# vidify/old-audiosync

Hardware: AMD Instinct MI355X
Metric: cross-correlations/sec (N=1440000 float32 pairs) (higher is better)
Workload: dtype f32; 1 GPU; batched xcorr, N=1440000 frames/sample (source 2N), 124 pairs per GPU per step, 48 kHz mono float32, planted delays, SNR 0 dB; sample_len=1440000, pairs_per_gpu=124, group=124, split=600x2400x16, layout=real-column, parallelism=pairs sharded over 1 GPU(s), one process per GPU, RCCL all_gather of results

## Files before the change

### include/audiosync/xcorr_hip.h

```cpp
#ifndef AUDIOSYNC_XCORR_HIP_H
#define AUDIOSYNC_XCORR_HIP_H

#include <stddef.h>
#include <stdint.h>

#ifdef __cplusplus
extern "C" {
#endif

typedef struct asx_plan asx_plan;


int asx_device_count(void);
int asx_current_device(void);
const char *asx_last_error(void);
int asx_abi_version(void);


asx_plan *asx_plan_create(size_t sample_len, size_t max_batch, int device);
asx_plan *asx_plan_create_ex(size_t sample_len, size_t max_batch, int device, const char *split);
int asx_plan_placement(asx_plan *plan, double ms[2], int *kept);
void asx_plan_destroy(asx_plan *plan);

int asx_plan_peak_overflows(asx_plan *plan, uint64_t *count);
int asx_plan_peak_repairs(asx_plan *plan, uint64_t *count);
int asx_plan_set_exact(asx_plan *plan, int on);
size_t asx_plan_peak_capacity(const asx_plan *plan);

int asx_plan_set_lag_window(asx_plan *plan, int64_t lag_min, int64_t lag_max);
int asx_plan_lag_window(const asx_plan *plan, int64_t *lag_min, int64_t *lag_max);

int asx_plan_set_pearson(asx_plan *plan, int spectral);
int asx_plan_pearson_modes(asx_plan *plan, uint64_t counts[3]);

int asx_plan_set_prune(asx_plan *plan, int on);
int asx_plan_prune_stats(asx_plan *plan, uint64_t *tiles_transformed, uint64_t *tiles_total);

size_t asx_plan_sample_len(const asx_plan *plan);
size_t asx_plan_fft_len(const asx_plan *plan);
int asx_plan_split(const asx_plan *plan, int *m1, int *m2, int *tile_cols);
int asx_plan_layout(const asx_plan *plan);
int asx_plan_threads(const asx_plan *plan, int *threads_cols, int *threads_rows);
size_t asx_plan_group(const asx_plan *plan);
size_t asx_plan_workspace_bytes(const asx_plan *plan);


int asx_xcorr_f64(asx_plan *plan, const double *source, const double *sample, long *lag,
                  double *coefficient);
int asx_plan_narrowed_calls(asx_plan *plan, uint64_t *count);

int asx_xcorr_batch_f32(asx_plan *plan, const float *source, const float *sample, size_t batch,
                        int64_t *lag, double *coef, int32_t *ret);

int asx_xcorr_batch_f32_dev(asx_plan *plan, const float *d_source, const float *d_sample,
                            size_t batch, int64_t *d_lag, double *d_coef, int32_t *d_ret,
                            void *stream);

int asx_xcorr_strided_f32_dev(asx_plan *plan, const float *d_source, size_t source_stride,
                              const float *d_sample, size_t sample_stride, size_t batch,
                              int64_t *d_lag, double *d_coef, int32_t *d_ret, void *stream);

int asx_xcorr_windowed_f32_dev(asx_plan *plan, const float *d_source, size_t source_stride,
                               const float *d_sample, size_t sample_stride,
                               const int64_t *d_windows, size_t window_stride,
                               size_t batch, int64_t *d_lag, double *d_coef, int32_t *d_ret,
                               void *stream);

#define ASX_TOPK_MAX 8
int asx_xcorr_topk_f32_dev(asx_plan *plan, const float *d_source, size_t source_stride,
                           const float *d_sample, size_t sample_stride,
                           const int64_t *d_windows, size_t window_stride,
                           size_t batch, int k, int64_t min_separation,
                           int64_t *d_lag, double *d_coef, int32_t *d_ret, void *stream);

int asx_xcorr_phat_f32_dev(asx_plan *plan, const float *d_source, size_t source_stride,
                           const float *d_sample, size_t sample_stride,
                           const int64_t *d_windows, size_t window_stride, size_t batch,
                           int64_t *d_lag, double *d_coef, double *d_peak, int32_t *d_ret, void *stream);

int asx_xcorr_phat_band_f32_dev(asx_plan *plan, const float *d_source, size_t source_stride,
                                const float *d_sample, size_t sample_stride,
                                const int64_t *d_windows, size_t window_stride, size_t batch,
                                int64_t bin_lo, int64_t bin_hi,
                                int64_t *d_lag, double *d_coef, double *d_peak, int32_t *d_ret, void *stream);

int asx_band_bins(size_t sample_len, double sample_rate, double f_lo_hz, double f_hi_hz,
                  int64_t *bin_lo, int64_t *bin_hi);

int asx_xcorr_pool_f32_dev(asx_plan *plan,
                           const float *d_sources, size_t source_stride, size_t nsources,
                           const float *d_samples, size_t sample_stride, size_t nsamples,
                           const int32_t *d_pairs,
                           const int64_t *d_windows, size_t window_stride,
                           size_t batch, int64_t *d_lag, double *d_coef, int32_t *d_ret, void *stream);

int asx_xcorr_pool_topk_f32_dev(asx_plan *plan,
                                const float *d_sources, size_t source_stride, size_t nsources,
                                const float *d_samples, size_t sample_stride, size_t nsamples,
                                const int32_t *d_pairs,
                                const int64_t *d_windows, size_t window_stride,
                                size_t batch, int k, int64_t min_separation,
                                int64_t *d_lag, double *d_coef, int32_t *d_ret, void *stream);

int asx_xcorr_batch_multi(asx_plan *const *plans, int nplans, const float *source, const float *sample,
                          size_t batch, int64_t *lag, double *coef, int32_t *ret);

typedef struct asx_comm asx_comm;
int asx_shard_range(size_t total, int nshards, int shard, size_t *start, size_t *count);
size_t asx_result_bytes(size_t width);
asx_comm *asx_comm_create(asx_plan *const *plans, int nplans);
void asx_comm_destroy(asx_comm *comm);
int asx_xcorr_batch_multi_dev(asx_comm *comm, const float *const *d_source, const float *const *d_sample,
                              const size_t *counts, size_t width, void *const *d_gathered);

int asx_xcorr_debug_r_dev(asx_plan *plan, const float *d_source, const float *d_sample,
                          float *d_r, int64_t *d_lag, double *d_coef, int32_t *d_ret,
                          void *stream);

int asx_xcorr_phat_debug_r_dev(asx_plan *plan, const float *d_source, const float *d_sample, float *d_r,
                               int64_t *d_lag, double *d_coef, double *d_peak, int32_t *d_ret, void *stream);

int asx_xcorr_phat_band_debug_r_dev(asx_plan *plan, const float *d_source, const float *d_sample,
                                    int64_t bin_lo, int64_t bin_hi, float *d_r,
                                    int64_t *d_lag, double *d_coef, double *d_peak, int32_t *d_ret, void *stream);

int asx_pearson_f64(const double *source_seg, const double *sample_seg, size_t n, int device,
                    double *coefficient);


int asx_results_to_ms_dev(const int64_t *d_lag, const double *d_coef, const int32_t *d_ret,
                          size_t batch, double min_confidence, double sample_rate,
                          int64_t *d_lag_ms, int32_t *d_accept, void *stream);

int asx_topk_best_dev(const int64_t *d_lag, const double *d_coef, const int32_t *d_ret,
                      size_t batch, int k,
                      int64_t *d_best_lag, double *d_best_coef, int32_t *d_best_ret, int32_t *d_best_entry,
                      void *stream);


typedef struct asx_stream asx_stream;

asx_stream *asx_stream_create(size_t max_sample_len, int device);
void asx_stream_destroy(asx_stream *stream);
int asx_stream_append_f64(asx_stream *stream, const double *source_frames, size_t n_source,
                          const double *sample_frames, size_t n_sample);
int asx_stream_lengths(const asx_stream *stream, size_t *n_source, size_t *n_sample);
int asx_stream_reset(asx_stream *stream);
int asx_stream_xcorr(asx_stream *stream, size_t sample_len, long *lag, double *coefficient);
int asx_stream_set_lag_window(asx_stream *stream, int64_t lag_min, int64_t lag_max);


int asx_synth_pairs_dev(uint64_t seed, uint64_t first_pair, size_t count, size_t sample_len,
                        int noise_shift, float *d_source, float *d_sample, int64_t *d_true_lag,
                        void *stream);

int asx_plan_set_profiling(asx_plan *plan, int depth);
int asx_plan_timings_ms(asx_plan *plan, int calls_back, float out[6]);
int asx_plan_last_timings_ms(asx_plan *plan, float out[6]);

void *asx_device_malloc(size_t bytes, int device);
int asx_device_free(void *ptr);
void *asx_host_malloc(size_t bytes);
int asx_host_free(void *ptr);
int asx_memcpy_h2d(void *dst_dev, const void *src_host, size_t bytes);
int asx_memcpy_d2h(void *dst_host, const void *src_dev, size_t bytes);
int asx_stream_sync(asx_plan *plan, void *stream);

#ifdef __cplusplus
}
#endif
#endif
```

### old-audiosync_amd/csrc/asx_api.hip

```cpp
#include "audiosync/xcorr_hip.h"

#include "asx_internal.h"
#include "dev_mem.h"
#include "plan_math.h"
#include "shard_driver.h"
#include "host_narrow.h"

#include <algorithm>
#include <cassert>
#include <cmath>
#include <cstdarg>
#include <cstdio>
#include <cstdlib>
#include <cstring>
#include <dlfcn.h>
#include <mutex>
#include <string>
#include <thread>
#include <type_traits>
#include <vector>

static thread_local std::string g_err;

static int fail(const char *fmt, ...)
{
    char buf[512];
    va_list ap;
    va_start(ap, fmt);
    vsnprintf(buf, sizeof(buf), fmt, ap);
    va_end(ap);
    g_err = buf;
    fprintf(stderr, "audiosync: %s\n", buf);
    return -1;
}

#define HIP_TRY(expr)                                                                         \
    do {                                                                                      \
        hipError_t e_ = (expr);                                                               \
        if (e_ != hipSuccess)                                                                 \
            return fail("%s failed: %s (%s:%d)", #expr, hipGetErrorString(e_), __FILE__, __LINE__); \
    } while (0)

#define HIP_TRY_NULL(expr)                                                                    \
    do {                                                                                      \
        hipError_t e_ = (expr);                                                               \
        if (e_ != hipSuccess) {                                                               \
            fail("%s failed: %s (%s:%d)", #expr, hipGetErrorString(e_), __FILE__, __LINE__);  \
            return nullptr;                                                                   \
        }                                                                                     \
    } while (0)

extern "C" const char *asx_last_error(void) { return g_err.c_str(); }
extern "C" int asx_abi_version(void) { return 2; }

extern "C" int asx_device_count(void)
{
    int n = 0;
    if (hipGetDeviceCount(&n) != hipSuccess) return 0;
    return n;
}

struct EventPair {
    hipEvent_t e0 = nullptr, e1 = nullptr;
    ~EventPair() { for (hipEvent_t e : { e0, e1 }) if (e) (void)hipEventDestroy(e); }
};

struct DevGuard {
    int prev = -1;
    bool ok = false;
    explicit DevGuard(int dev)
    {
        if (hipGetDevice(&prev) == hipSuccess && hipSetDevice(dev) == hipSuccess) ok = true;
    }
    ~DevGuard() { if (prev >= 0) (void)hipSetDevice(prev); }
};

static bool stream_capturing(hipStream_t s)
{
    hipStreamCaptureStatus cap = hipStreamCaptureStatusNone;
    if (hipStreamIsCapturing(s, &cap) != hipSuccess) (void)hipGetLastError();
    return cap != hipStreamCaptureStatusNone;
}

extern "C" int asx_current_device(void)
{
    int d = -1;
    if (hipGetDevice(&d) != hipSuccess) return -1;
    return d;
}

static thread_local hipError_t g_take_err = hipSuccess;
static const AsxMemOps hip_mem = {
    [](void **out, size_t bytes) { return (g_take_err = hipMalloc(out, bytes)) == hipSuccess ? 0 : ((void)hipGetLastError(), -1); },
    [](void *ptr) { (void)hipFree(ptr); }
};

struct asx_plan {
    int device = 0;
    AsxHostPlan host;
    AsxDev dev{};
    size_t group = 1;
    size_t stamp_blocks = 0;
    hipStream_t stream = nullptr;
    std::mutex lock;

    AsxMemSet mem{ hip_mem }, cxy0{ hip_mem };
    struct Lane {
        hipStream_t stream = nullptr;
        hipEvent_t done = nullptr;
        float2 *zxa = nullptr, *zya = nullptr, *ga = nullptr;
        AsxPeakWs pk{};
        AsxSeg *seg = nullptr;
        double *psums = nullptr;
        AsxSpecWs spec{};
        AsxTopkWs tk{};
        AsxPrune prune{};
        AsxPoolPair *pool = nullptr;
    } lanes[2];
    int nlanes = 1;
    hipEvent_t fork = nullptr;
    struct BigPeak {
        AsxCand *cand = nullptr;
        uint32_t *refine_idx = nullptr, *cand_n = nullptr, *refine_n = nullptr;
        double *refine_val = nullptr;
        unsigned long long *overflows = nullptr;
        float *src_dc = nullptr;
        double *stats = nullptr;
        size_t cap = 0;
    } big;
    AsxSpectra bslot{};
    struct Bank {
        AsxSpectra c{};
        AsxMemSet mem{ hip_mem };
        size_t nsrc = 0, nsmp = 0;
        unsigned long long fills = 0;
    } bank;
    uint32_t *over_list = nullptr, *over_n = nullptr;
    volatile uint32_t *h_over_n = nullptr;
    size_t over_cap = 0;
    std::vector<uint32_t> h_over;
    unsigned long long repaired = 0;
    bool exact = true;
    int64_t win_lo = 0, win_hi = 0;
    bool spectral = false;
    unsigned long long *mode_count = nullptr;
    bool prunable = false;
    bool prune = false;
    unsigned long long *prune_stats = nullptr;
    bool tune_placement = false, placement_done = false;
    double placement_ms[2] = { 0.0, 0.0 };
    int placement_kept = -1;
    struct Staging {
        float *src = nullptr, *smp = nullptr;
        int64_t *lag = nullptr; double *coef = nullptr; int32_t *ret = nullptr;
    } st;
    struct Staging64 { double *src = nullptr, *smp = nullptr; } st64;
    float *pin32 = nullptr;
    unsigned long long narrowed = 0;

    bool profiling = false;
    size_t prof_depth = 1, prof_calls = 0, prof_ring = 0;
    std::vector<std::vector<hipEvent_t>> evr;
    std::vector<size_t> prof_groups;
    size_t ev_groups = 0;
};

struct PlanCall {
    std::unique_lock<std::mutex> guard;
    DevGuard dg;
    hipStream_t s;
    explicit PlanCall(asx_plan *p, void *stream = nullptr, bool lock = true)
        : guard(lock ? std::unique_lock<std::mutex>(p->lock) : std::unique_lock<std::mutex>()), dg(p->device),
          s(stream ? (hipStream_t)stream : p->stream) {}
};

template <typename T> static int dev_alloc(AsxMemSet &m, T **out, size_t count)
{
    return m.take(out, count) ? fail("hipMalloc(&ptr, bytes) failed: %s (%s:%d)", hipGetErrorString(g_take_err), __FILE__, __LINE__) : 0;
}

template <typename T> static int dev_upload(AsxMemSet &m, const T **out, const std::vector<T> &v)
{
    T *d = nullptr;
    if (dev_alloc(m, &d, v.size()) != 0) return -1;
    HIP_TRY(hipMemcpy(d, v.data(), v.size() * sizeof(T), hipMemcpyHostToDevice));
    *out = d;
    return 0;
}

static int take_spectra(const AsxDev &P, AsxMemSet &m, AsxSpectra &c, size_t nsrc, size_t nsmp)
{
    const size_t pitch = asx_spectrum_len(P), na = std::max(nsrc, nsmp), nt = P.ntiles, nb = nt * (size_t)P.nbands;
    return m.take(&c.cx, nsrc * pitch) || m.take(&c.cy, nsmp * pitch) || m.take(&c.nrm, na * 2 * nt) || (nb && m.take(&c.band, na * 2 * nb)) ? -1 : 0;
}

static int plan_init(asx_plan *p, size_t N, size_t max_batch, const char *split)
{
    std::string err = asx_host_plan_build(N, split, &p->host);
    if (!err.empty()) return fail("plan for sample_len=%zu: %s", N, err.c_str());
    const AsxHostPlan &h = p->host;
    AsxDev &d = p->dev;
    AsxMemSet &m = p->mem;
    d.N = (uint32_t)N;
    d.F = h.F; d.M = h.M; d.M1 = h.M1; d.M2 = h.M2; d.T = h.T; d.logT = h.logT; d.ntiles = h.ntiles;
    d.src_valid = h.src_valid;
    d.src_period = (uint32_t)(2 * N);
    d.nout = (uint32_t)(2 * N);
    d.bound_scale = 2.0f * ASX_BOUND_C * 5.9604645e-8f * log2f((float)h.F) * (float)h.F;
    d.st1 = h.st1; d.st2 = h.st2;
    const AsxKernelChoice &k = h.kernels;
    if (k.rlayout && (k.cols < 0 || k.rows < 0 || !h.rlayout)) return fail("internal: a real-column plan without its kernels");
    d.threads_cols = k.threads_cols; d.threads_rows = k.threads_rows;
    d.rlayout = k.rlayout ? 1 : 0;
    d.kcols = k.cols; d.krows = k.rows;
    d.band_rows = k.band_rows;
    d.nbands = k.band_rows ? 2 * h.M1 / k.band_rows : 0;
    p->prunable = k.prunable;
    if (dev_upload(m, &d.tw1, h.tw1) || dev_upload(m, &d.tw2, h.tw2) || dev_upload(m, &d.tw2s, h.tw2s) || dev_upload(m, &d.tw_lo, h.tw_lo) ||
        dev_upload(m, &d.tw_hi, h.tw_hi) ||
        dev_upload(m, &d.k1_of_pos1, h.k1_of_pos1) || dev_upload(m, &d.pos1_of_k1, h.pos1_of_k1) ||
        dev_upload(m, &d.pos2_of_k2, h.pos2_of_k2) || dev_upload(m, &d.row_tasks, h.row_tasks))
        return -1;

    d.col_pairs = nullptr;
    d.col_tw = nullptr;
    if (k.rlayout && (dev_upload(m, &d.col_pairs, h.col_pairs) || dev_upload(m, &d.col_tw, h.col_tw))) return -1;
    size_t ws_mb = 4096;
    if (const char *e = getenv("ASX_WS_MB")) ws_mb = (size_t)atol(e) > 0 ? (size_t)atol(e) : ws_mb;
    size_t per_pair = (size_t)3 * h.M * sizeof(float2);
    size_t g = (ws_mb << 20) / per_pair / (getenv("ASX_LANES") && atoi(getenv("ASX_LANES")) == 2 ? 2 : 1);
    if (g < 1) g = 1;
    if (g > 65535) g = 65535;
    if (max_batch < 1) max_batch = 1;
    if (g > max_batch) g = max_batch;
    p->group = g;
    if (const char *e = getenv("ASX_LANES")) p->nlanes = atoi(e) == 2 ? 2 : 1;
    size_t cap = std::min<size_t>(std::max<size_t>(N / 64, ASX_CAND_MIN), ASX_CAND_MAX);
    cap = std::min<size_t>(cap, 2 * N);
    for (int l = 0; l < p->nlanes; l++) {
        asx_plan::Lane &ln = p->lanes[l];
        ln.pk.cap = (uint32_t)cap;
        const size_t mz = asx_spectrum_len(d);
        AsxMemSet &cxy = l == 0 ? p->cxy0 : m;
        if (dev_alloc(cxy, &ln.zxa, g * mz) || dev_alloc(cxy, &ln.zya, g * mz) || dev_alloc(m, &ln.ga, g * mz) ||
            dev_alloc(m, &ln.pk.nrm_part, g * 2 * (size_t)h.ntiles) || dev_alloc(m, &ln.pk.bound2, g) ||
            dev_alloc(m, &ln.pk.pairmax, g) || dev_alloc(m, &ln.pk.cand_n, g) ||
            dev_alloc(m, &ln.pk.cand, g * cap) || dev_alloc(m, &ln.pk.refine_n, g) ||
            dev_alloc(m, &ln.pk.refine_idx, g * cap) || dev_alloc(m, &ln.pk.refine_val, g * cap) ||
            dev_alloc(m, &ln.pk.overflows, 1) ||
            dev_alloc(m, &ln.seg, g) || dev_alloc(m, &ln.psums, g * (size_t)asx_pearson_blocks((uint32_t)N) * 6) ||
            dev_alloc(m, &ln.tk.pairs, g) || dev_alloc(m, &ln.tk.lag, g) || dev_alloc(m, &ln.tk.coef, g) || dev_alloc(m, &ln.tk.ret, g) ||
            dev_alloc(m, &ln.tk.sink, 1) || dev_alloc(m, &ln.pool, g))
            return -1;
        HIP_TRY(hipMemset(ln.pk.overflows, 0, sizeof(unsigned long long)));
        ln.pk.band = nullptr; ln.pk.tile_peak = nullptr;
        if (d.rlayout) {
            const size_t nbands = (size_t)d.nbands;
            if (!p->mode_count) {
                if (dev_alloc(m, &p->mode_count, ASX_PM_NMODES)) return -1;
                HIP_TRY(hipMemset(p->mode_count, 0, ASX_PM_NMODES * sizeof(unsigned long long)));
            }
            if (dev_alloc(m, &ln.pk.band, g * 2 * nbands * (size_t)h.ntiles) || dev_alloc(m, &ln.pk.tile_peak, g * (size_t)(h.M2 / h.T)) ||
                dev_alloc(m, &ln.spec.part, g * ASX_PREP_BLOCKS_MAX * 4) || dev_alloc(m, &ln.spec.hdr, g * ASX_SPEC_HDR))
                return -1;
            ln.spec.mode_count = p->mode_count;
            ln.spec.tol = 1e-5;
        }
        if (p->prunable) {
            if (!p->prune_stats) {
                if (dev_alloc(m, &p->prune_stats, 2)) return -1;
                HIP_TRY(hipMemset(p->prune_stats, 0, 2 * sizeof(unsigned long long)));
            }
            if (dev_alloc(m, &ln.prune.eng, g * ((size_t)h.M1 + 1) * (size_t)h.ntiles) || dev_alloc(m, &ln.prune.ub, g * (size_t)h.ntiles) ||
                dev_alloc(m, &ln.prune.best, g) || dev_alloc(m, &ln.prune.skip, g * (size_t)h.ntiles) ||
                dev_alloc(m, &ln.prune.part, g * 1024) || dev_alloc(m, &ln.prune.ticket, g))
                return -1;
            HIP_TRY(hipMemset(ln.prune.part, 0, g * 1024 * sizeof(double)));
            HIP_TRY(hipMemset(ln.prune.ticket, 0, g * sizeof(unsigned)));
            ln.prune.stats = p->prune_stats;
        }
        HIP_TRY(hipStreamCreateWithFlags(&ln.stream, hipStreamNonBlocking));
        HIP_TRY(hipEventCreateWithFlags(&ln.done, hipEventDisableTiming));
    }
    p->over_cap = std::max<size_t>(g * (size_t)p->nlanes, 1024);
    if (dev_alloc(m, &p->over_list, p->over_cap) || dev_alloc(m, &p->over_n, 1)) return -1;
    HIP_TRY(hipMemset(p->over_n, 0, sizeof(uint32_t)));
    uint32_t *d_over_host = nullptr;
    {
        void *h = nullptr, *dptr = nullptr;
        HIP_TRY(hipHostMalloc(&h, sizeof(uint32_t), hipHostMallocMapped));
        p->h_over_n = (volatile uint32_t *)h;
        *p->h_over_n = 0;
        HIP_TRY(hipHostGetDevicePointer(&dptr, h, 0));
        d_over_host = (uint32_t *)dptr;
    }
    for (int l = 0; l < p->nlanes; l++) {
        p->lanes[l].pk.over_list = p->over_list;
        p->lanes[l].pk.over_n = p->over_n;
        p->lanes[l].pk.over_host = d_over_host;
        p->lanes[l].pk.over_cap = (uint32_t)p->over_cap;
    }
    p->spectral = d.rlayout != 0;
    if (const char *e = getenv("ASX_PEARSON")) p->spectral = p->spectral && strcmp(e, "direct") != 0;
    p->prune = p->prunable;
    if (const char *e = getenv("ASX_PRUNE")) p->prune = p->prune && atoi(e) != 0;
    if (const char *e = getenv("ASX_EXACT")) p->exact = atoi(e) != 0;
    p->win_lo = -(int64_t)p->host.N;
    p->win_hi = (int64_t)p->host.N - 1;
    HIP_TRY(hipEventCreateWithFlags(&p->fork, hipEventDisableTiming));
    d.stamps = nullptr;
    d.stamp_kernel = 0;
    if (const char *e = getenv("ASX_STAMPS")) {
        unsigned long long *st = nullptr;
        p->stamp_blocks = g * (size_t)std::max(h.M1 + 1, 2 * h.ntiles);
        if (dev_alloc(m, &st, p->stamp_blocks * 8)) return -1;
        HIP_TRY(hipMemset(st, 0, p->stamp_blocks * 8 * sizeof(unsigned long long)));
        d.stamps = st;
        d.stamp_kernel = !strcmp(e, "fwd") ? 1 : !strcmp(e, "inv") ? 2 : 0;
    }
    {
        AsxDev *dcopy = nullptr;
        if (dev_alloc(m, &dcopy, 1)) return -1;
        d.self_dev = dcopy;
        HIP_TRY(hipMemcpy(dcopy, &d, sizeof(AsxDev), hipMemcpyHostToDevice));
    }
    HIP_TRY(hipStreamCreate(&p->stream));
    HIP_TRY(hipDeviceSynchronize());
    return 0;
}

static std::string measure_best_split(size_t N, size_t max_batch, int device)
{
    std::vector<std::string> cands = asx_host_plan_candidates(N, 16);
    {
        AsxHostPlan h;
        if (asx_host_plan_build(N, "", &h).empty()) {
            char buf[64];
            snprintf(buf, sizeof buf, "%dx%dx%d", h.M1, h.M2, h.T);
            if (std::find(cands.begin(), cands.end(), std::string(buf)) == cands.end()) cands.insert(cands.begin(), buf);
        }
    }
    if (cands.empty()) return "";
    size_t probe = ((size_t)512 << 20) / (12 * N);
    probe = std::max<size_t>(probe, 4);
    probe = std::min<size_t>(probe, 1024);
    probe = std::max<size_t>(1, std::min(probe, max_batch));
    AsxMemSet m(hip_mem);
    asx_plan::Staging d;
    std::string best;
    float best_ms = 0.f;
    EventPair ev;
    if (!m.take(&d.src, probe * 2 * N) && !m.take(&d.smp, probe * N) && !m.take(&d.lag, probe) && !m.take(&d.coef, probe) &&
        !m.take(&d.ret, probe) && hipEventCreate(&ev.e0) == hipSuccess && hipEventCreate(&ev.e1) == hipSuccess &&
        asx_synth_pairs_dev(12345, 0, probe, N, 1, d.src, d.smp, nullptr, nullptr) == 0 && hipDeviceSynchronize() == hipSuccess) {
        for (const std::string &c : cands) {
            asx_plan *p = asx_plan_create_ex(N, probe, device, c.c_str());
            if (!p) continue;
            bool ok = asx_xcorr_batch_f32_dev(p, d.src, d.smp, probe, d.lag, d.coef, d.ret, nullptr) == 0;
            float ms = 0.f;
            if (ok) {
                ok = hipEventRecord(ev.e0, p->stream) == hipSuccess;
                for (int r = 0; r < 2 && ok; r++) ok = asx_xcorr_batch_f32_dev(p, d.src, d.smp, probe, d.lag, d.coef, d.ret, nullptr) == 0;
                ok = ok && hipEventRecord(ev.e1, p->stream) == hipSuccess && hipEventSynchronize(ev.e1) == hipSuccess &&
                     hipEventElapsedTime(&ms, ev.e0, ev.e1) == hipSuccess;
            }
            asx_plan_destroy(p);
            if (ok && (best.empty() || ms < best_ms)) { best = c; best_ms = ms; }
        }
    }
    (void)hipGetLastError();
    return best;
}

extern "C" asx_plan *asx_plan_create_ex(size_t sample_len, size_t max_batch, int device, const char *split)
{
    if (!split || !*split) split = getenv("ASX_SPLIT");
    if (split && !strcmp(split, "measure")) {
        int prev = 0, ndev0 = 0;
        if (hipGetDeviceCount(&ndev0) != hipSuccess || ndev0 == 0) {
            fail("no usable HIP device; this library has no CPU fallback");
            return nullptr;
        }
        HIP_TRY_NULL(hipGetDevice(&prev));
        const int dev = device < 0 ? prev : device;
        if (dev >= ndev0) { fail("device %d out of range (%d devices)", dev, ndev0); return nullptr; }
        HIP_TRY_NULL(hipSetDevice(dev));
        const std::string best = measure_best_split(sample_len, max_batch ? max_batch : 1, dev);
        (void)hipSetDevice(prev);
        asx_plan *mp = asx_plan_create_ex(sample_len, max_batch, device, best.empty() ? "auto" : best.c_str());
        if (mp) mp->tune_placement = true;
        return mp;
    }
    if (split && !strcmp(split, "auto")) split = "";
    int ndev = 0;
    hipError_t e = hipGetDeviceCount(&ndev);
    if (e != hipSuccess || ndev == 0) {
        fail("no usable HIP device (%s); this library has no CPU fallback",
             e == hipSuccess ? "device count is 0" : hipGetErrorString(e));
        return nullptr;
    }
    if (device < 0) HIP_TRY_NULL(hipGetDevice(&device));
    if (device >= ndev) {
        fail("device %d out of range (%d devices)", device, ndev);
        return nullptr;
    }
    int prev = 0;
    HIP_TRY_NULL(hipGetDevice(&prev));
    HIP_TRY_NULL(hipSetDevice(device));
    asx_plan *p = new asx_plan();
    p->device = device;
    int rc = plan_init(p, sample_len, max_batch, split);
    (void)hipSetDevice(prev);
    if (rc != 0) {
        asx_plan_destroy(p);
        return nullptr;
    }
    return p;
}

extern "C" asx_plan *asx_plan_create(size_t sample_len, size_t max_batch, int device)
{
    return asx_plan_create_ex(sample_len, max_batch, device, nullptr);
}

extern "C" void asx_plan_destroy(asx_plan *p)
{
    if (!p) return;
    DevGuard dg(p->device);
    if (p->stream) { (void)hipStreamSynchronize(p->stream); (void)hipStreamDestroy(p->stream); }
    for (auto &ln : p->lanes) {
        if (ln.stream) { (void)hipStreamSynchronize(ln.stream); (void)hipStreamDestroy(ln.stream); }
        if (ln.done) (void)hipEventDestroy(ln.done);
    }
    if (p->fork) (void)hipEventDestroy(p->fork);
    for (auto &ring : p->evr)
        for (hipEvent_t ev : ring) (void)hipEventDestroy(ev);
    if (p->pin32) (void)hipHostFree(p->pin32);
    if (p->h_over_n) (void)hipHostFree((void *)p->h_over_n);
    delete p;
}

extern "C" size_t asx_plan_sample_len(const asx_plan *p) { return p ? p->host.N : 0; }
extern "C" size_t asx_plan_fft_len(const asx_plan *p) { return p ? p->host.F : 0; }
extern "C" size_t asx_plan_group(const asx_plan *p) { return p ? p->group : 0; }
extern "C" size_t asx_plan_workspace_bytes(const asx_plan *p) { return p ? p->mem.bytes() + p->cxy0.bytes() : 0; }
extern "C" long asx_plan_debug_stamps(asx_plan *p, unsigned long long *out, size_t cap)
{
    if (!p || !p->dev.stamps) return -1;
    size_t n = p->stamp_blocks * 8;
    if (n > cap) n = cap;
    if (hipMemcpy(out, p->dev.stamps, n * sizeof(unsigned long long), hipMemcpyDeviceToHost) != hipSuccess) return -1;
    return (long)n;
}

extern "C" int asx_plan_peak_overflows(asx_plan *p, uint64_t *count)
{
    if (!p || !count) return fail("asx_plan_peak_overflows: null argument");
    PlanCall c(p);
    if (!c.dg.ok) return fail("cannot select device %d", p->device);
    unsigned long long total = 0;
    for (int l = 0; l < p->nlanes; l++) {
        unsigned long long v = 0;
        HIP_TRY(hipStreamSynchronize(p->lanes[l].stream));
        HIP_TRY(hipStreamSynchronize(p->stream));
        HIP_TRY(hipMemcpy(&v, p->lanes[l].pk.overflows, sizeof(v), hipMemcpyDeviceToHost));
        total += v;
    }
    *count = total;
    return 0;
}

extern "C" int asx_plan_set_exact(asx_plan *p, int on)
{
    if (!p) return fail("asx_plan_set_exact: null argument");
    PlanCall c(p);
    if (!c.dg.ok) return fail("cannot select device %d", p->device);
    HIP_TRY(hipDeviceSynchronize());
    HIP_TRY(hipMemset(p->over_n, 0, sizeof(uint32_t)));
    *p->h_over_n = 0;
    p->exact = on != 0;
    return 0;
}

extern "C" int asx_plan_set_pearson(asx_plan *p, int spectral)
{
    if (!p) return fail("asx_plan_set_pearson: null argument");
    std::lock_guard<std::mutex> guard(p->lock);
    if (spectral && !p->dev.rlayout) return fail("asx_plan_set_pearson: the spectral form needs a real-column plan (the reference's six lengths)");
    p->spectral = spectral != 0;
    return 0;
}

extern "C" int asx_plan_pearson_modes(asx_plan *p, uint64_t counts[3])
{
    if (!p || !counts) return fail("asx_plan_pearson_modes: null argument");
    PlanCall c(p);
    if (!c.dg.ok) return fail("cannot select device %d", p->device);
    counts[0] = counts[1] = counts[2] = 0;
    if (!p->mode_count) return 0;
    HIP_TRY(hipDeviceSynchronize());
    unsigned long long v[ASX_PM_NMODES];
    HIP_TRY(hipMemcpy(v, p->mode_count, sizeof v, hipMemcpyDeviceToHost));
    for (int i = 0; i < 3; i++) counts[i] = v[i];
    return 0;
}

extern "C" int asx_plan_set_prune(asx_plan *p, int on)
{
    if (!p) return fail("asx_plan_set_prune: null argument");
    std::lock_guard<std::mutex> guard(p->lock);
    if (on && !p->prunable)
        return fail("asx_plan_set_prune: the pruned inverse pass needs a real-column plan (the reference's six lengths)");
    p->prune = on != 0;
    return 0;
}

extern "C" int asx_plan_prune_stats(asx_plan *p, uint64_t *tiles_transformed, uint64_t *tiles_total)
{
    if (!p || !tiles_transformed || !tiles_total) return fail("asx_plan_prune_stats: null argument");
    PlanCall c(p);
    if (!c.dg.ok) return fail("cannot select device %d", p->device);
    *tiles_transformed = *tiles_total = 0;
    if (!p->prune_stats) return 0;
    HIP_TRY(hipDeviceSynchronize());
    unsigned long long v[2];
    HIP_TRY(hipMemcpy(v, p->prune_stats, sizeof v, hipMemcpyDeviceToHost));
    *tiles_transformed = v[0];
    *tiles_total = v[1];
    return 0;
}

extern "C" int asx_plan_peak_repairs(asx_plan *p, uint64_t *count)
{
    if (!p || !count) return fail("asx_plan_peak_repairs: null argument");
    std::lock_guard<std::mutex> guard(p->lock);
    *count = p->repaired;
    return 0;
}

extern "C" int asx_plan_debug_peak(asx_plan *p, size_t pair, float *bound2, uint32_t *cand_n, uint32_t *refine_n,
                                   unsigned long long *pairmax, double *vals, uint32_t *idxs, size_t cap)
{
    if (!p || pair >= p->group) return -1;
    PlanCall c(p, nullptr, false);
    const AsxPeakWs &W = p->lanes[0].pk;
    (void)hipDeviceSynchronize();
    if (hipMemcpy(bound2, W.bound2 + pair, 4, hipMemcpyDeviceToHost) != hipSuccess) return -1;
    if (hipMemcpy(cand_n, W.cand_n + pair, 4, hipMemcpyDeviceToHost) != hipSuccess) return -1;
    if (hipMemcpy(refine_n, W.refine_n + pair, 4, hipMemcpyDeviceToHost) != hipSuccess) return -1;
    if (hipMemcpy(pairmax, W.pairmax + pair, 8, hipMemcpyDeviceToHost) != hipSuccess) return -1;
    size_t n = std::min<size_t>(cap, W.cap);
    if (vals && hipMemcpy(vals, W.refine_val + pair * (size_t)W.cap, n * 8, hipMemcpyDeviceToHost) != hipSuccess) return -1;
    if (idxs && hipMemcpy(idxs, W.refine_idx + pair * (size_t)W.cap, n * 4, hipMemcpyDeviceToHost) != hipSuccess) return -1;
    return 0;
}

extern "C" int asx_plan_debug_spectral(asx_plan *p, size_t pair, int *dims, float *band, size_t band_cap, double *hdr,
                                       long long *seg, double *pick)
{
    if (!p || pair >= p->group || !dims || !hdr || !seg || !pick) return -1;
    const asx_plan::Lane &W = p->lanes[0];
    if (!p->dev.rlayout || !W.pk.band || !W.spec.hdr) return -1;
    PlanCall c(p, nullptr, false);
    if (!c.dg.ok || hipDeviceSynchronize() != hipSuccess) return -1;
    const AsxDev &P = p->dev;
    const size_t cells = (size_t)P.ntiles * (size_t)P.nbands;
    if (band) {
        if (band_cap < 4 * cells) return -1;
        if (hipMemcpy(band, W.pk.band + pair * 2 * cells, 2 * cells * sizeof(float2), hipMemcpyDeviceToHost) != hipSuccess) return -1;
    }
    AsxSeg sg;
    if (hipMemcpy(hdr, W.spec.hdr + pair * ASX_SPEC_HDR, ASX_SPEC_HDR * sizeof(double), hipMemcpyDeviceToHost) != hipSuccess ||
        hipMemcpy(&sg, W.seg + pair, sizeof sg, hipMemcpyDeviceToHost) != hipSuccess)
        return -1;
    seg[0] = sg.lag; seg[1] = sg.src_off; seg[2] = sg.smp_off; seg[3] = sg.len; seg[4] = sg.peak; seg[5] = sg.flags;
    AsxMemSet tmp(hip_mem);
    double *d_pick = nullptr;
    if (tmp.take(&d_pick, 8)) return -1;
    const int nb = asx_launch_debug_spec_pick(P, W.spec, W.seg, pair, d_pick, p->stream);
    if (hipGetLastError() != hipSuccess || hipStreamSynchronize(p->stream) != hipSuccess ||
        hipMemcpy(pick, d_pick, 8 * sizeof(double), hipMemcpyDeviceToHost) != hipSuccess)
        return -1;
    dims[0] = P.ntiles; dims[1] = P.nbands; dims[2] = P.band_rows; dims[3] = nb;
    return 0;
}

extern "C" int asx_plan_debug_prune(asx_plan *p, size_t pair, float *ub, int *best, size_t n)
{
    if (!p || pair >= p->group || !p->lanes[0].prune.ub || n > (size_t)p->host.ntiles) return -1;
    PlanCall c(p, nullptr, false);
    if (!c.dg.ok || hipDeviceSynchronize() != hipSuccess) return -1;
    const AsxPrune &U = p->lanes[0].prune;
    if (ub && hipMemcpy(ub, U.ub + pair * (size_t)p->host.ntiles, n * sizeof(float), hipMemcpyDeviceToHost) != hipSuccess) return -1;
    if (best && hipMemcpy(best, U.best + pair, sizeof(int), hipMemcpyDeviceToHost) != hipSuccess) return -1;
    return 0;
}

extern "C" int asx_plan_debug_over_list(asx_plan *p, uint32_t *dev_n, uint32_t *host_n)
{
    if (!p || !dev_n || !host_n) return -1;
    PlanCall c(p, nullptr, false);
    if (!c.dg.ok || hipDeviceSynchronize() != hipSuccess) return -1;
    if (hipMemcpy(dev_n, p->over_n, sizeof(uint32_t), hipMemcpyDeviceToHost) != hipSuccess) return -1;
    *host_n = *p->h_over_n;
    return 0;
}

extern "C" size_t asx_plan_peak_capacity(const asx_plan *p) { return p ? p->lanes[0].pk.cap : 0; }

extern "C" int asx_plan_set_lag_window(asx_plan *p, int64_t lag_min, int64_t lag_max)
{
    if (!p) return fail("asx_plan_set_lag_window: null plan");
    const int64_t N = (int64_t)p->host.N;
    if (lag_min < -N || lag_max > N - 1 || lag_min > lag_max)
        return fail("asx_plan_set_lag_window: [%lld, %lld] is not a window inside [%lld, %lld] with lag_min <= lag_max",
                    (long long)lag_min, (long long)lag_max, (long long)-N, (long long)(N - 1));
    std::lock_guard<std::mutex> guard(p->lock);
    p->win_lo = lag_min;
    p->win_hi = lag_max;
    return 0;
}

extern "C" int asx_plan_lag_window(const asx_plan *p, int64_t *lag_min, int64_t *lag_max)
{
    if (!p || !lag_min || !lag_max) return fail("asx_plan_lag_window: null argument");
    std::lock_guard<std::mutex> guard(const_cast<asx_plan *>(p)->lock);
    *lag_min = p->win_lo;
    *lag_max = p->win_hi;
    return 0;
}

extern "C" int asx_plan_threads(const asx_plan *p, int *cols, int *rows)
{
    if (!p) return -1;
    if (cols) *cols = p->dev.threads_cols;
    if (rows) *rows = p->dev.threads_rows;
    return 0;
}

extern "C" int asx_plan_layout(const asx_plan *p) { return p ? p->dev.rlayout : -1; }

extern "C" int asx_plan_narrowed_calls(asx_plan *p, uint64_t *count)
{
    if (!p || !count) return fail("asx_plan_narrowed_calls: null argument");
    std::lock_guard<std::mutex> guard(p->lock);
    *count = p->narrowed;
    return 0;
}

extern "C" int asx_plan_split(const asx_plan *p, int *m1, int *m2, int *tile_cols)
{
    if (!p) return -1;
    if (m1) *m1 = p->host.M1;
    if (m2) *m2 = p->host.M2;
    if (tile_cols) *tile_cols = p->host.T;
    return 0;
}

static void prof_begin_call(asx_plan *p)
{
    p->ev_groups = 0;
    if (!p->profiling) return;
    p->prof_ring = p->prof_calls % p->prof_depth;
    if (p->prof_groups.size() < p->prof_depth) p->prof_groups.resize(p->prof_depth, 0);
    if (p->evr.size() < p->prof_depth) p->evr.resize(p->prof_depth);
    p->prof_groups[p->prof_ring] = 0;
}
static void prof_end_call(asx_plan *p, size_t groups)
{
    if (!p->profiling) return;
    p->ev_groups = groups;
    p->prof_groups[p->prof_ring] = groups;
    p->prof_calls++;
}

static int prof_mark(asx_plan *p, hipStream_t s, size_t slot)
{
    if (!p->profiling) return 0;
    std::vector<hipEvent_t> &ev = p->evr[p->prof_ring];
    while (ev.size() <= slot) {
        hipEvent_t e;
        HIP_TRY(hipEventCreate(&e));
        ev.push_back(e);
    }
    HIP_TRY(hipEventRecord(ev[slot], s));
    return 0;
}

struct PoolCall {
    const int32_t *rows;
    size_t nsrc, nsmp;
};
template <typename TIn> struct Pairs {
    const float *src, *smp;
    const TIn *tsrc, *tsmp;
    size_t src_step, smp_step;
    int bc;
    const int64_t *win = nullptr;
    size_t win_step = 0;
    const PoolCall *pool = nullptr;
    size_t first = 0;
    static Pairs staged(const float *src, const float *smp, const TIn *tsrc, const TIn *tsmp, size_t N, const int64_t *win = nullptr,
                        size_t win_step = 0)
    {
        return { .src = src, .smp = smp, .tsrc = tsrc, .tsmp = tsmp, .src_step = 2 * N, .smp_step = N, .bc = 0, .win = win, .win_step = win_step };
    }
    static Pairs contiguous(const float *src, const float *smp, size_t N) { return staged(src, smp, src, smp, N); }
    static Pairs strided(const float *src, size_t src_step, const float *smp, size_t smp_step, int bc, const int64_t *win, size_t win_step)
    {
        return { .src = src, .smp = smp, .tsrc = src, .tsmp = smp, .src_step = src_step, .smp_step = smp_step, .bc = bc, .win = win, .win_step = win_step };
    }
    static Pairs pooled(const PoolCall *pool, const float *srcs, size_t src_stride, const float *smps, size_t smp_stride, const int64_t *win,
                        size_t win_step)
    {
        Pairs x = strided(srcs, src_stride, smps, smp_stride, 0, win, win_step);
        x.pool = pool;
        return x;
    }
    Pairs pool_pair(size_t a, size_t b, size_t N) const
    {
        return staged(src + a * src_step, smp + b * smp_step, tsrc + a * src_step, tsmp + b * smp_step, N, win, win_step);
    }
    Pairs at(size_t k) const
    {
        Pairs x = *this;
        if (win) x.win += 2 * k * win_step;
        if (pool) { x.first += k; return x; }
        x.src += k * src_step; x.smp += k * smp_step; x.tsrc += k * src_step; x.tsmp += k * smp_step;
        return x;
    }
    AsxInputs<TIn> inputs(const AsxPoolPair *pl) const { return { tsrc, tsmp, src_step, smp_step, pl }; }
};

struct Results {
    int64_t *lag;
    double *coef;
    int32_t *ret;
    size_t step = 1;
    double *peak = nullptr;
    Results at(size_t k) const
    {
        return { lag ? lag + k * step : nullptr, coef + k * step, ret ? ret + k * step : nullptr, step, peak ? peak + k : nullptr };
    }
};

struct Topk {
    int k = 1;
    int64_t sep = 0;
};

struct GroupOpts {
    static constexpr size_t no_marks = SIZE_MAX;
    size_t prof_group = 0;
    int lane = 0;
    uint32_t pair_base = 0;
    bool listed = true;
    bool spectral = true;
    float *r_out = nullptr;
    int dot_blocks = 0;
    const AsxPeakWs *pk = nullptr;
    Topk topk{};
    AsxWeight weight = ASX_W_NONE;
    AsxBand fband{};
};

template <typename TIn>
static int run_group(asx_plan *p, const Pairs<TIn> &x, size_t g, const Results &y, hipStream_t s, const GroupOpts &o = {})
{
    const AsxDev &P = p->dev;
    asx_plan::Lane &W = p->lanes[o.lane];
    const AsxPeakWs &pk = o.pk ? *o.pk : W.pk;
    auto mark = [&](size_t k) { return o.prof_group != GroupOpts::no_marks && prof_mark(p, s, o.prof_group * 6 + k); };
    AsxPeakWs fin = pk;
    const bool phat = o.weight != ASX_W_NONE;
    if (!o.listed || phat) { fin.over_list = nullptr; fin.over_n = nullptr; fin.over_host = nullptr; fin.over_cap = 0; }
    const bool spectral = std::is_same<TIn, float>::value && p->spectral && o.spectral && pk.band && !phat;
    AsxPeakWs tk = pk;
    if (!spectral) { tk.band = nullptr; tk.tile_peak = nullptr; }
    const bool f32_entry = std::is_same<TIn, float>::value && o.spectral;
    const AsxSearch call = AsxSearch::of(p->win_lo, p->win_hi, P.N, x.win, x.win_step, W.tk, 0);
    const bool prune = p->prune && !phat && f32_entry && !x.pool && x.bc == 0 && !o.r_out && !o.pk && o.topk.k == 1 && call.kind == AsxSearch::ALL;
    const AsxPoolPair *pl = x.pool ? W.pool : nullptr;
    const AsxSpectra &from = pl ? p->bank.c : p->bslot;
    const AsxSpectra C{ (pl || (x.bc & 1)) ? from.cx : W.zxa, (pl || (x.bc & 2)) ? from.cy : W.zya, pk.nrm_part, tk.band, x.bc, pl,
                        prune ? &W.prune : nullptr, o.weight, o.fband };
    if (mark(0)) return -1;
    if (pl) {
        const AsxPoolArgs A{ x.pool->rows, (uint64_t)x.first, (uint64_t)x.pool->nsrc, (uint64_t)x.pool->nsmp, (uint64_t)x.src_step,
                             (uint64_t)x.smp_step, from.nrm, from.band };
        asx_launch_pool_resolve(P, A, W.pool, C.nrm, C.band, (int)g, s);
    } else if (P.rlayout) {
        asx_launch_fwd_cols_r(P, (x.bc & 1) ? nullptr : x.src, x.src_step, (x.bc & 2) ? nullptr : x.smp, x.smp_step, 0, (int)g, C, false, s);
        for (unsigned which = 0; which < 2; which++)
            if (x.bc & (1 << which)) asx_launch_bcast_aux(P, from.nrm, from.band, C.nrm, C.band, (int)g, which, s);
    } else if (x.src_step == 2 * (size_t)P.N && x.smp_step == P.N) {
        asx_launch_fwd_cols(P, x.src, x.smp, W.zxa, W.zya, tk, (int)g, s);
    } else {
        for (size_t k = 0; k < g; k++) {
            AsxPeakWs one = tk;
            one.nrm_part = pk.nrm_part + k * 2 * (size_t)P.ntiles;
            asx_launch_fwd_cols(P, x.at(k).src, x.at(k).smp, W.zxa + k * (size_t)P.M, W.zya + k * (size_t)P.M, one, 1, s);
        }
    }
    if (mark(1)) return -1;
    float2 *q = W.ga;
    if (!P.rlayout) asx_launch_rows(P, W.zxa, W.zya, q, tk, (int)g, s);
    else asx_launch_rows_r(P, C, q, tk, (int)g, s);
    if (mark(2)) return -1;
    const int K = o.topk.k;
    const Results out = K > 1 ? Results{ W.tk.lag, W.tk.coef, W.tk.ret } : y;
    const AsxInputs<TIn> in = x.inputs(pl);
    const int dot_blocks = o.dot_blocks ? o.dot_blocks : (int)std::min<size_t>(ASX_DOT_BLOCKS, std::max<size_t>(8, 16384 / g));
    auto search = [&](int j) { return AsxSearch::of(p->win_lo, p->win_hi, P.N, x.win, x.win_step, W.tk, j); };
    auto pass = [&](const AsxSearch &find, bool first) -> int {
        float *const r_out = first ? o.r_out : nullptr;
        if (!P.rlayout) asx_launch_inv_cols(P, q, tk, r_out, (int)g, s, find);
        else asx_launch_inv_cols_r(P, q, tk, r_out, (int)g, s, find, C.prune);
        if (first && mark(3)) return -1;
        if (phat) {
            asx_launch_phat_finalize(P, fin, W.seg, y.peak, o.weight == ASX_W_PHAT_BAND ? o.fband.votes(P.N) : (double)P.F, (int)g, s, find);
            if (first && mark(4)) return -1;
            asx_launch_pearson(in, P.N, W.seg, W.psums, out.lag, out.coef, out.ret, (int)g, s);
            return 0;
        }
        asx_launch_finalize(P, fin, W.seg, (int)g, s, o.pair_base, find);
        asx_launch_refine(P, in, pk, W.seg, (int)g, s, dot_blocks, !spectral, find);
        if (first && mark(4)) return -1;
        if (!spectral)
            asx_launch_pearson(in, P.N, W.seg, W.psums, out.lag, out.coef, out.ret, (int)g, s);
        else if constexpr (std::is_same<TIn, float>::value)
            asx_launch_pearson_spectral_f32(P, in, find, tk, W.spec, W.seg, W.psums, out.lag, out.coef, out.ret, (int)g, s);
        return 0;
    };
    if (pass(call, true)) return -1;
    if (call.kind == AsxSearch::ROWS && K == 1) asx_launch_invalid_rows(call.rows, P.N, y.lag, y.coef, y.ret, (int)g, s);
    if (pl && K == 1) asx_launch_invalid_pairs(pl, y.lag, y.coef, y.ret, (int)g, s);
    for (int j = 0; K > 1 && j < K; j++) {
        if (j > 0 && pass(search(j), false)) return -1;
        asx_launch_topk_step(W.tk, W.seg, pk, call, P.N, (int)g, j, K, o.topk.sep, y.lag, y.coef, y.ret, s);
    }
    if (pl && K > 1) asx_launch_invalid_pairs_k(pl, K, y.lag, y.coef, y.ret, (int)g, s);
    if (mark(5)) return -1;
    HIP_TRY(hipGetLastError());
    return 0;
}

template <typename TIn>
static int second_look(asx_plan *p, const Pairs<TIn> &xi, const Results &yi, hipStream_t s, const Topk &topk)
{
    const AsxDev &P = p->dev;
    const size_t N = p->host.N;
    asx_plan::BigPeak &B = p->big;
    if (!B.cand && asx_mem_whole(p->mem, B, [&](AsxMemSet &m, asx_plan::BigPeak &T) {
            T.cap = 2 * N;
            if (dev_alloc(m, &T.cand, T.cap) || dev_alloc(m, &T.refine_idx, T.cap) || dev_alloc(m, &T.refine_val, T.cap) ||
                dev_alloc(m, &T.cand_n, 1) || dev_alloc(m, &T.refine_n, 1) || dev_alloc(m, &T.overflows, 1) ||
                dev_alloc(m, &T.src_dc, 2 * N) || dev_alloc(m, &T.stats, ASX_DC_STATS_DOUBLES))
                return -1;
            HIP_TRY(hipMemsetAsync(T.overflows, 0, sizeof(unsigned long long), s));
            return 0;
        }))
        return -1;
    AsxPeakWs K = p->lanes[0].pk;
    K.cand_n = B.cand_n; K.cand = B.cand;
    K.refine_n = B.refine_n; K.refine_idx = B.refine_idx; K.refine_val = B.refine_val;
    K.overflows = B.overflows;
    K.over_list = nullptr; K.over_n = nullptr; K.over_host = nullptr; K.over_cap = 0;
    K.band = nullptr; K.tile_peak = nullptr;
    K.cap = (uint32_t)B.cap;
    HIP_TRY(hipMemsetAsync(B.cand_n, 0, sizeof(uint32_t), s));
    asx_launch_dc_remove(xi.tsrc, xi.tsmp, P.N, (double)P.F, B.stats, B.src_dc, s);
    K.shift = B.stats + 2;
    if (run_group(p, Pairs<TIn>::staged(B.src_dc, xi.smp, xi.tsrc, xi.tsmp, N, xi.win, xi.win_step), 1, yi, s,
                  { .prof_group = GroupOpts::no_marks, .listed = false, .spectral = false, .dot_blocks = 2048, .pk = &K, .topk = topk }))
        return -1;
    p->repaired++;
    return 0;
}

template <typename TIn>
static int resolve_overflows(asx_plan *p, const Pairs<TIn> &x, const Results &y, hipStream_t s, const Topk &topk = {})
{
    HIP_TRY(hipStreamSynchronize(s));
    if (p->lanes[0].pk.cap >= 2 * p->host.N) return 0;
    const uint32_t n = *p->h_over_n;
    if (n == 0) return 0;
    if (n > p->over_cap) {
        (void)hipMemsetAsync(p->over_n, 0, sizeof(uint32_t), s);
        (void)hipStreamSynchronize(s);
        *p->h_over_n = 0;
        return fail("internal: %u overflowed pairs in a window of %zu", n, p->over_cap);
    }
    p->h_over.resize(n);
    HIP_TRY(hipMemcpyAsync(p->h_over.data(), p->over_list, n * sizeof(uint32_t), hipMemcpyDeviceToHost, s));
    HIP_TRY(hipMemsetAsync(p->over_n, 0, sizeof(uint32_t), s));
    std::vector<int32_t> ab;
    if (x.pool) {
        ab.resize(2 * (size_t)n);
        for (uint32_t k = 0; k < n; k++) {
            const size_t pi = x.first + p->h_over[k];
            if (x.pool->rows)
                HIP_TRY(hipMemcpyAsync(&ab[2 * k], x.pool->rows + 2 * pi, 2 * sizeof(int32_t), hipMemcpyDeviceToHost, s));
            else { ab[2 * k] = (int32_t)(pi / x.pool->nsmp); ab[2 * k + 1] = (int32_t)(pi % x.pool->nsmp); }
        }
    }
    HIP_TRY(hipStreamSynchronize(s));
    *p->h_over_n = 0;
    for (uint32_t k = 0; k < n; k++) {
        const uint32_t i = p->h_over[k];
        Pairs<TIn> xi = x.at(i);
        if (x.pool) {
            const int64_t a = ab[2 * k], b = ab[2 * k + 1];
            if (a < 0 || (size_t)a >= x.pool->nsrc || b < 0 || (size_t)b >= x.pool->nsmp) continue;
            xi = xi.pool_pair((size_t)a, (size_t)b, p->host.N);
        }
        if (second_look(p, xi, y.at(i), s, topk)) return -1;
    }
    return (int)n;
}

template <typename TIn>
static int fetch_results(asx_plan *p, const Pairs<TIn> &x, size_t g, const Results &d, const Results &h, hipStream_t s)
{
    for (int pass = 0; pass < 2; pass++) {
        HIP_TRY(hipMemcpyAsync(h.lag, d.lag, g * sizeof(int64_t), hipMemcpyDeviceToHost, s));
        HIP_TRY(hipMemcpyAsync(h.coef, d.coef, g * sizeof(double), hipMemcpyDeviceToHost, s));
        HIP_TRY(hipMemcpyAsync(h.ret, d.ret, g * sizeof(int32_t), hipMemcpyDeviceToHost, s));
        if (pass == 1) { HIP_TRY(hipStreamSynchronize(s)); break; }
        const int looked = resolve_overflows(p, x, d, s);
        if (looked < 0) return -1;
        if (looked == 0) break;
    }
    return 0;
}

static int tune_placement(asx_plan *p, const float *d_src, const float *d_smp, size_t g, hipStream_t s)
{
    if (stream_capturing(s)) return 0;
    p->placement_done = true;
    const AsxDev &P = p->dev;
    asx_plan::Lane &W = p->lanes[0];
    const size_t mz = asx_spectrum_len(P) * p->group;
    AsxMemSet second(hip_mem);
    float2 *set[2][2] = { { W.zxa, W.zya }, { nullptr, nullptr } };
    if (second.take(&set[1][0], mz) || second.take(&set[1][1], mz)) return 0;
    EventPair ev;
    HIP_TRY(hipEventCreate(&ev.e0));
    HIP_TRY(hipEventCreate(&ev.e1));
    AsxPeakWs tk = W.pk;
    tk.band = nullptr; tk.tile_peak = nullptr;
    for (int k = 0; k < 2; k++) {
        float best = 0.f;
        for (int r = 0; r < 4; r++) {
            HIP_TRY(hipEventRecord(ev.e0, s));
            if (P.rlayout) asx_launch_fwd_cols_r(P, d_src, 2 * (size_t)P.N, d_smp, P.N, 0, (int)g, { set[k][0], set[k][1], tk.nrm_part, tk.band }, false, s);
            else asx_launch_fwd_cols(P, d_src, d_smp, set[k][0], set[k][1], tk, (int)g, s);
            HIP_TRY(hipEventRecord(ev.e1, s));
            HIP_TRY(hipEventSynchronize(ev.e1));
            float ms = 0.f;
            HIP_TRY(hipEventElapsedTime(&ms, ev.e0, ev.e1));
            if (r >= 1 && (best == 0.f || ms < best)) best = ms;
        }
        p->placement_ms[k] = best;
    }
    const int keep = p->placement_ms[1] < 0.995 * p->placement_ms[0] ? 1 : 0;
    p->placement_kept = keep;
    if (keep == 1) p->cxy0.swap(second);
    W.zxa = set[keep][0];
    W.zya = set[keep][1];
    return 0;
}

extern "C" int asx_plan_placement(asx_plan *p, double ms[2], int *kept)
{
    if (!p || !ms || !kept) return fail("asx_plan_placement: null argument");
    std::lock_guard<std::mutex> guard(p->lock);
    ms[0] = p->placement_ms[0]; ms[1] = p->placement_ms[1];
    *kept = p->placement_kept;
    return 0;
}

static int run_batch(asx_plan *p, const Pairs<float> &x, size_t batch, const Results &y, hipStream_t s, const Topk &topk = {},
                     AsxWeight weight = ASX_W_NONE, const AsxBand &band = {})
{
    prof_begin_call(p);
    const bool exact = p->exact && weight == ASX_W_NONE;
    const bool overlap = (p->nlanes == 2) && !p->profiling && batch >= 8;
    size_t chunk = p->group;
    if (overlap && batch < 2 * chunk) chunk = (batch + 1) / 2;
    const size_t window = exact ? std::max<size_t>(chunk, p->over_cap / chunk * chunk) : batch;
    size_t gi = 0;
    for (size_t w0 = 0; w0 < batch; w0 += window) {
        const size_t wn = std::min(window, batch - w0);
        if (overlap) {
            HIP_TRY(hipEventRecord(p->fork, s));
            for (int l = 0; l < 2; l++) HIP_TRY(hipStreamWaitEvent(p->lanes[l].stream, p->fork, 0));
        }
        for (size_t done = w0; done < w0 + wn; done += chunk, gi++) {
            const size_t g = std::min(chunk, w0 + wn - done);
            const int lane = overlap ? (int)(gi & 1) : 0;
            hipStream_t ls = overlap ? p->lanes[lane].stream : s;
            if (run_group(p, x.at(done), g, y.at(done), ls,
                          { .prof_group = gi, .lane = lane, .pair_base = (uint32_t)(done - w0), .listed = exact, .topk = topk,
                            .weight = weight, .fband = band }))
                return -1;
        }
        if (overlap) {
            for (int l = 0; l < 2; l++) {
                HIP_TRY(hipEventRecord(p->lanes[l].done, p->lanes[l].stream));
                HIP_TRY(hipStreamWaitEvent(s, p->lanes[l].done, 0));
            }
        }
        if (exact && resolve_overflows(p, x.at(w0), y.at(w0), s, topk) < 0) return -1;
    }
    prof_end_call(p, gi);
    return 0;
}

extern "C" int asx_xcorr_batch_f32_dev(asx_plan *p, const float *d_source, const float *d_sample,
                                       size_t batch, int64_t *d_lag, double *d_coef, int32_t *d_ret,
                                       void *stream)
{
    if (!p || !d_source || !d_sample || !d_coef) return fail("asx_xcorr_batch_f32_dev: null argument");
    PlanCall c(p, stream);
    if (!c.dg.ok) return fail("cannot select device %d", p->device);
    const size_t N = p->host.N;
    if (p->tune_placement && !p->placement_done && batch >= std::min<size_t>(p->group, 8) &&
        tune_placement(p, d_source, d_sample, std::min(batch, p->group), c.s))
        return -1;
    return run_batch(p, Pairs<float>::contiguous(d_source, d_sample, N), batch, { d_lag, d_coef, d_ret }, c.s);
}

static int strided_batch(asx_plan *p, const char *fn, const float *d_source, size_t source_stride, const float *d_sample,
                         size_t sample_stride, const int64_t *d_windows, size_t window_stride, size_t batch, const Results &y, void *stream,
                         const Topk &topk = {}, AsxWeight weight = ASX_W_NONE, const AsxBand &band = {})
{
    PlanCall c(p, stream);
    if (!c.dg.ok) return fail("cannot select device %d", p->device);
    hipStream_t s = c.s;
    const AsxDev &P = p->dev;
    if (weight != ASX_W_NONE && P.rlayout != 1) return fail("%s: PHAT calls need a real-column plan (asx_plan_layout() == 1)", fn);
    if (P.rlayout) {
        if (((uintptr_t)d_source & 15u) || ((uintptr_t)d_sample & 15u))
            return fail("%s: real-column plans need 16-byte aligned inputs (source %p, sample %p)",
                        fn, (const void *)d_source, (const void *)d_sample);
        if ((source_stride & 3u) || (sample_stride & 3u))
            return fail("%s: real-column plans need strides that are multiples of 4 floats "
                        "(source_stride %zu, sample_stride %zu)", fn, source_stride, sample_stride);
    }
    if (batch == 0) return 0;
    const int bc = P.rlayout ? (source_stride == 0 ? 1 : 0) | (sample_stride == 0 ? 2 : 0) : 0;
    if (bc) {
        AsxSpectra &B = p->bslot;
        if (!B.cx) {
            if (stream_capturing(s))
                return fail("%s: the plan's broadcast workspace does not exist yet and cannot be allocated "
                            "during a stream capture; make one call with a stride of 0 outside the capture first", fn);
            if (asx_mem_whole(p->mem, B, [&](AsxMemSet &m, AsxSpectra &T) { return take_spectra(P, m, T, 1, 1); }))
                return fail("hipMalloc(&ptr, bytes) failed: %s (%s:%d)", hipGetErrorString(g_take_err), __FILE__, __LINE__);
        }
        asx_launch_fwd_cols_r(P, (bc & 1) ? d_source : nullptr, 0, (bc & 2) ? d_sample : nullptr, 0, 0, 1, B, true, s);
    }
    return run_batch(p, Pairs<float>::strided(d_source, source_stride, d_sample, sample_stride, bc, d_windows, window_stride), batch, y, s,
                     topk, weight, band);
}

extern "C" int asx_xcorr_strided_f32_dev(asx_plan *p, const float *d_source, size_t source_stride, const float *d_sample,
                                         size_t sample_stride, size_t batch, int64_t *d_lag, double *d_coef, int32_t *d_ret,
                                         void *stream)
{
    if (!p || !d_source || !d_sample || !d_coef) return fail("asx_xcorr_strided_f32_dev: null argument");
// ... 924 lines not shown
```

### old-audiosync_amd/csrc/asx_internal.h

```cpp
#pragma once

#include <hip/hip_runtime.h>
#include <stdint.h>
#include <type_traits>

#define ASX_MAX_STAGES 12
#define ASX_TW_LOG 11
#define ASX_TW_LO (1u << ASX_TW_LOG)
#define ASX_THREADS 256
#define ASX_FFT_THREADS_MAX 512
#define ASX_COL_LOADS 10
#define ASX_ROW_STEPS 5
#define ASX_PEARSON_BLOCKS_MAX 512
#define ASX_DC_STATS_DOUBLES (4 + 2 * 128)
#define ASX_BOUND_C 4.0f
#define ASX_PRUNE_DELTA 6.103515625e-5f
#define ASX_PRUNE_FLOOR_PER_TERM 3.944304526105059e-31
#define ASX_PRUNE_T 16
#define ASX_CAND_MAX 16384
#define ASX_CAND_MIN 2048
#define ASX_DOT_BLOCKS 128

struct AsxStages {
    int n;
    int nstages;
    int radix[ASX_MAX_STAGES];
    int ns[ASX_MAX_STAGES];
    int q[ASX_MAX_STAGES];
    int nbf[ASX_MAX_STAGES];
    int twmul[ASX_MAX_STAGES];
    float inv_q[ASX_MAX_STAGES];
    float inv_nbf[ASX_MAX_STAGES];
};

struct AsxDev;
struct AsxDev {
    uint32_t N;
    uint32_t F, M;
    int M1, M2;
    int T, logT;
    int ntiles;
    int threads_cols, threads_rows;
    uint32_t src_valid;
    uint32_t src_period;
    uint32_t nout;
    float bound_scale;
    AsxStages st1, st2;
    const float2 *tw1;
    const float2 *tw2;
    const float2 *tw2s;
    const float2 *tw_lo;
    const float2 *tw_hi;
    const int *k1_of_pos1;
    const int *pos1_of_k1;
    const int *pos2_of_k2;
    const int4 *row_tasks;
    int band_rows, nbands;
    int rlayout;
    const int4 *col_pairs;
    const float2 *col_tw;
    const AsxDev *self_dev;
    unsigned long long *stamps;
    int stamp_kernel;
    int kcols, krows;
};

typedef unsigned long long asx_peak_t;

struct AsxSeg {
    long long lag;
    uint32_t src_off;
    uint32_t smp_off;
    uint32_t len;
    uint32_t peak;
    uint32_t flags;
};
#define ASX_SEG_INEXACT 1u

struct AsxWin {
    uint32_t a, w, seed, n;
    static constexpr bool masks = true;
    __device__ __forceinline__ AsxWin window_of(size_t, uint32_t) const { return *this; }
};
__host__ __device__ inline bool asx_win_has(const AsxWin &z, uint32_t idx)
{
    if (idx >= z.n) return false;
    const uint32_t d = idx >= z.a ? idx - z.a : idx + (z.n - z.a);
    return d <= z.w;
}
__host__ __device__ inline AsxWin asx_win_of(int64_t lo, int64_t hi, uint32_t N)
{
    AsxWin z;
    z.n = 2u * N;
    z.a = (uint32_t)(lo >= 0 ? lo : (int64_t)z.n + lo);
    z.w = (uint32_t)(hi - lo);
    z.seed = (lo < 0 && hi >= 0) ? 0u : z.a;
    return z;
}

struct AsxWinRows;
__device__ inline bool asx_win_row(const AsxWinRows &R, size_t pair, uint32_t N, AsxWin &z);
struct AsxWinRows {
    const int64_t *rows;
    size_t step;
    static constexpr bool masks = true;
    __device__ __forceinline__ AsxWin window_of(size_t pair, uint32_t N) const
    {
        AsxWin z;
        (void)asx_win_row(*this, pair, N, z);
        return z;
    }
    __device__ __forceinline__ uint32_t seed_of(size_t pair, uint32_t N) const { return window_of(pair, N).seed; }
};
__device__ inline bool asx_win_row(const AsxWinRows &R, size_t pair, uint32_t N, AsxWin &z)
{
    const int64_t *row = R.rows + 2 * pair * R.step;
    const int64_t lo = row[0], hi = row[1], n = (int64_t)N;
    const bool ok = -n <= lo && lo <= hi && hi <= n - 1;
    if (ok) z = asx_win_of(lo, hi, N);
    else z.a = z.w = z.seed = z.n = 0u;
    return ok;
}

#define ASX_TOPK_MAX 8
#define ASX_TK_EMPTY 1u
#define ASX_TK_INVALID 2u
#define ASX_TK_INEXACT 4u
struct AsxTopkPair {
    AsxWin z;
    int32_t lo[ASX_TOPK_MAX - 1];
    uint32_t wd[ASX_TOPK_MAX - 1];
    uint32_t nz;
    uint32_t flags;
    int32_t wlo, whi;
};
template <int ZC> struct AsxWinX {
    uint32_t a, w, seed, n;
    uint32_t zo[ZC];
    uint32_t wd[ZC];
};
template <int ZC> __host__ __device__ inline bool asx_win_has(const AsxWinX<ZC> &z, uint32_t idx)
{
    if (idx >= z.n) return false;
    const uint32_t d = idx >= z.a ? idx - z.a : idx + (z.n - z.a);
    bool in = d <= z.w;
#pragma unroll
    for (int i = 0; i < ZC; i++) in = in && d - z.zo[i] > z.wd[i];
    return in;
}
template <int ZC> __host__ __device__ inline AsxWinX<ZC> asx_win_x(const AsxTopkPair *X, size_t pair)
{
    const AsxTopkPair &t = X[pair];
    AsxWinX<ZC> z;
    z.a = t.z.a; z.w = t.z.w; z.seed = t.z.seed; z.n = t.z.n;
#pragma unroll
    for (int i = 0; i < ZC; i++) {
        const bool used = (uint32_t)i < t.nz;
        z.zo[i] = used ? (uint32_t)(t.lo[i] - t.wlo) : ~0u;
        z.wd[i] = used ? t.wd[i] : 0u;
    }
    return z;
}
struct AsxTopkWs {
    AsxTopkPair *pairs;
    int64_t *lag;
    double *coef;
    int32_t *ret;
    unsigned long long *sink;
};

struct AsxSearch {
    enum Kind { ALL, WINDOW, ROWS, TOPK } kind;
    int64_t lo, hi;
    AsxWin win;
    AsxWinRows rows;
    const AsxTopkPair *tk;
    int tk_zones;
    unsigned long long *tk_sink;
    uint32_t seed() const { return kind == WINDOW ? win.seed : 0u; }
    static AsxSearch of(int64_t lo, int64_t hi, uint32_t N, const int64_t *rows, size_t rows_step, const AsxTopkWs &T, int pass)
    {
        AsxSearch q{ ALL, lo, hi, asx_win_of(lo, hi, N), { rows, rows_step }, nullptr, 0, nullptr };
        if (pass > 0) { q.kind = TOPK; q.tk = T.pairs; q.tk_zones = pass; q.tk_sink = T.sink; }
        else if (rows) q.kind = ROWS;
        else if (lo != -(int64_t)N || hi != (int64_t)N - 1) q.kind = WINDOW;
        return q;
    }
};

#define ASX_POOL_INVALID 1u
struct AsxPoolPair {
    uint32_t sx, sy;
    uint32_t flags, pad;
    uint64_t src_off;
    uint64_t smp_off;
};
struct AsxPoolArgs {
    const int32_t *rows;
    uint64_t first;
    uint64_t nsrc, nsmp, src_stride, smp_stride;
    const float *nrm;
    const float2 *band;
};

template <typename TIn> struct AsxInputs {
    const TIn *src, *smp;
    size_t src_pitch, smp_pitch;
    const AsxPoolPair *pl;
};
struct AsxAtPitch {
    size_t src_pitch, smp_pitch;
    __device__ __forceinline__ size_t src_off(size_t pair) const { return pair * src_pitch; }
    __device__ __forceinline__ size_t smp_off(size_t pair) const { return pair * smp_pitch; }
};
struct AsxAtList {
    const AsxPoolPair *__restrict__ pl;
    __device__ __forceinline__ size_t src_off(size_t pair) const { return pl[pair].src_off; }
    __device__ __forceinline__ size_t smp_off(size_t pair) const { return pl[pair].smp_off; }
};
template <typename TIn, class F> void asx_with_inputs(const AsxInputs<TIn> &in, F go)
{
    if constexpr (std::is_same<TIn, float>::value) {
        if (in.pl) return go(AsxAtList{ in.pl });
    }
    go(AsxAtPitch{ in.src_pitch, in.smp_pitch });
}

struct AsxCand {
    uint32_t idx;
    float key;
};

struct AsxPeakWs {
    float *nrm_part;
    float *bound2;
    asx_peak_t *pairmax;
    uint32_t *cand_n;
    AsxCand *cand;
    uint32_t *refine_n;
    uint32_t *refine_idx;
    double *refine_val;
    unsigned long long *overflows;
    uint32_t *over_list;
    uint32_t *over_n;
    uint32_t *over_host;
    uint32_t over_cap;
    const double *shift;
    uint32_t cap;
    float2 *band;
    float *tile_peak;
};

struct AsxPrune {
    float *eng;
    float *ub;
    int *best;
    double *part;
    unsigned *ticket;
    unsigned char *skip;
    unsigned long long *stats;
};

struct AsxSelAll {
    static constexpr bool masks = false;
    __device__ __forceinline__ AsxWin window_of(size_t, uint32_t) const { return AsxWin{}; }
};
template <int ZC> struct AsxSelTopk {
    const AsxTopkPair *__restrict__ X;
    static constexpr bool masks = true;
    __device__ __forceinline__ AsxWinX<ZC> window_of(size_t pair, uint32_t) const { return asx_win_x<ZC>(X, pair); }
};
struct AsxSelSeed {
    uint32_t seed;
    __device__ __forceinline__ uint32_t seed_of(size_t, uint32_t) const { return seed; }
};
struct AsxSelTopkSeed {
    const AsxTopkPair *__restrict__ X;
    __device__ __forceinline__ uint32_t seed_of(size_t pair, uint32_t) const { return X[pair].z.seed; }
};
template <bool FIRST> struct AsxSelPrune {
    const int *__restrict__ best;
    const unsigned char *__restrict__ skip;
    static constexpr bool masks = false;
    __device__ __forceinline__ AsxWin window_of(size_t, uint32_t) const { return AsxWin{}; }
};
template <class Sel> __device__ __forceinline__ bool asx_sel_takes(const Sel &, int, int, int) { return true; }
template <class Sel> __device__ __forceinline__ int asx_sel_tile(const Sel &, int grid_tile) { return grid_tile; }
template <bool FIRST> __device__ __forceinline__ bool asx_sel_takes(const AsxSelPrune<FIRST> &q, int grid_tile, int M2, int T)
{
    if constexpr (FIRST) {
        const int bt = q.best[blockIdx.x];
        return blockIdx.y == 0 || bt != 0;
    } else {
        return grid_tile * T < M2 && !q.skip[(size_t)blockIdx.x * (size_t)(M2 / T) + grid_tile];
    }
}
template <bool FIRST> __device__ __forceinline__ int asx_sel_tile(const AsxSelPrune<FIRST> &q, int grid_tile)
{
    if constexpr (FIRST) return blockIdx.y == 0 ? q.best[blockIdx.x] : 0;
    else return grid_tile;
}
template <int... ZC, class F> void asx_with_selection(const AsxSearch &q, F go)
{
    if constexpr (sizeof...(ZC) == 0) {
        if (q.kind == AsxSearch::TOPK) go(AsxSelTopkSeed{ q.tk });
        else if (q.kind == AsxSearch::ROWS) go(q.rows);
        else go(AsxSelSeed{ q.seed() });
    } else {
        if (q.kind == AsxSearch::TOPK) (void)((q.tk_zones <= ZC && (go(AsxSelTopk<ZC>{ q.tk }), true)) || ...);
        else if (q.kind == AsxSearch::ROWS) go(q.rows);
        else if (q.kind == AsxSearch::WINDOW) go(q.win);
        else go(AsxSelAll{});
    }
}

enum AsxWeight { ASX_W_NONE = 0, ASX_W_PHAT = 1, ASX_W_PHAT_BAND = 2 };
struct AsxBand {
    uint32_t lo = 0, span = 0;
    double votes(uint32_t N) const { return 2.0 * ((double)span + 1.0) - (lo == 0) - (lo + span == N); }
};
struct AsxSpectra {
    float2 *cx, *cy;
    float *nrm;
    float2 *band;
    int bc = 0;
    const AsxPoolPair *pl = nullptr;
    const AsxPrune *prune = nullptr;
    AsxWeight weight = ASX_W_NONE;
    AsxBand fband{};
};
inline size_t asx_spectrum_len(const AsxDev &P) { return ((size_t)P.M1 + 1) * (size_t)P.M2; }

#define ASX_PM_FAST 0
#define ASX_PM_CORR 1
#define ASX_PM_DIRECT 2
#define ASX_PM_NMODES 3
#ifndef ASX_PREP_BLOCKS
#define ASX_PREP_BLOCKS 4
#endif
#define ASX_PREP_BLOCKS_MAX 16
#define ASX_SPEC_HDR 4
struct AsxSpecWs {
    double *part;
    double *hdr;
    unsigned long long *mode_count;
    double tol;
    int nb;
    uint32_t N;
};

void asx_launch_fwd_cols(const AsxDev &P, const float *src, const float *smp, float2 *zxa,
                         float2 *zya, const AsxPeakWs &W, int npairs, hipStream_t s);
void asx_launch_rows(const AsxDev &P, float2 *zxa, float2 *zya, float2 *ga,
                     const AsxPeakWs &W, int npairs, hipStream_t s);
void asx_launch_inv_cols(const AsxDev &P, const float2 *ga, const AsxPeakWs &W, float *r_out, int npairs, hipStream_t s,
                         const AsxSearch &q);
void asx_launch_fwd_cols_r(const AsxDev &P, const float *src, size_t src_stride, const float *smp, size_t smp_stride, size_t first,
                           int count, const AsxSpectra &dst, bool temporal, hipStream_t s);
void asx_launch_rows_r(const AsxDev &P, const AsxSpectra &C, float2 *q, const AsxPeakWs &W, int npairs, hipStream_t s);
void asx_launch_inv_cols_r(const AsxDev &P, const float2 *q, const AsxPeakWs &W, float *r_out, int npairs, hipStream_t s,
                           const AsxSearch &search, const AsxPrune *U);
void asx_launch_phat_finalize(const AsxDev &P, const AsxPeakWs &W, AsxSeg *seg, double *peak, double f, int npairs, hipStream_t s,
                              const AsxSearch &q);
void asx_launch_bcast_aux(const AsxDev &P, const float *snrm, const float2 *sband, float *nrm, float2 *band, int npairs,
                          unsigned which, hipStream_t s);
void asx_launch_pool_resolve(const AsxDev &P, const AsxPoolArgs &A, AsxPoolPair *out, float *nrm, float2 *band, int npairs,
                             hipStream_t s);
void asx_launch_invalid_pairs(const AsxPoolPair *pl, int64_t *lag, double *coef, int32_t *ret, int npairs, hipStream_t s);
void asx_launch_invalid_pairs_k(const AsxPoolPair *pl, int k, int64_t *lag, double *coef, int32_t *ret, int npairs, hipStream_t s);
void asx_launch_finalize(const AsxDev &P, const AsxPeakWs &W, AsxSeg *seg, int npairs, hipStream_t s, uint32_t pair_base,
                         const AsxSearch &q);
void asx_launch_topk_step(AsxTopkWs T, const AsxSeg *seg, const AsxPeakWs &W, const AsxSearch &call, uint32_t N, int npairs, int j,
                          int k, int64_t sep, int64_t *lag, double *coef, int32_t *ret, hipStream_t s);
void asx_launch_invalid_rows(const AsxWinRows &rows, uint32_t N, int64_t *lag, double *coef, int32_t *ret, int npairs, hipStream_t s);
template <typename TIn>
void asx_launch_refine(const AsxDev &P, const AsxInputs<TIn> &in, const AsxPeakWs &W, AsxSeg *seg, int npairs, hipStream_t s,
                       int dot_blocks, bool pick, const AsxSearch &q);
template <typename TIn>
void asx_launch_pearson(const AsxInputs<TIn> &in, uint32_t basis_len, const AsxSeg *seg, double *psums, int64_t *lag, double *coef,
                        int32_t *ret, int npairs, hipStream_t s);
void asx_launch_pearson_partial_spec_f32(const AsxInputs<float> &in, uint32_t basis_len, const AsxSeg *seg, const AsxSpecWs &S,
                                         double *psums, int npairs, hipStream_t s);
void asx_launch_pearson_spectral_f32(const AsxDev &P, const AsxInputs<float> &in, const AsxSearch &q, const AsxPeakWs &W,
                                     const AsxSpecWs &S, AsxSeg *seg, double *psums, int64_t *lag, double *coef, int32_t *ret,
                                     int npairs, hipStream_t s);
int asx_launch_debug_spec_pick(const AsxDev &P, const AsxSpecWs &S, const AsxSeg *seg, size_t pair, double *out, hipStream_t s);
void asx_launch_results_to_ms(const int64_t *lag, const double *coef, const int32_t *ret, size_t batch,
                              double min_confidence, double sample_rate, int64_t *lag_ms, int32_t *accept,
                              hipStream_t s);
void asx_launch_topk_best(const int64_t *lag, const double *coef, const int32_t *ret, size_t batch, int k, int64_t *best_lag,
                          double *best_coef, int32_t *best_ret, int32_t *best_entry, hipStream_t s);
void asx_launch_cvt_f64_f32(const double *in, float *out, size_t n, hipStream_t s);
unsigned asx_pearson_blocks(uint32_t basis_len);
template <typename TIn>
void asx_launch_dc_remove(const TIn *src, const TIn *smp, uint32_t N, double scale, double *stats, float *out, hipStream_t s);
void asx_launch_synth(uint64_t seed, uint64_t first_pair, size_t count, uint32_t N,
                      int noise_shift, float *src, float *smp, int64_t *true_lag, hipStream_t s);
```

### old-audiosync_amd/csrc/rlayout.hip

```cpp
#include "asx_internal.h"
#include "lds_fft.h"
#include "xcorr_dev.h"
#include "kernel_table.h"

#include <algorithm>
#include <map>
#include <mutex>
#include <utility>
#include <stdlib.h>

extern __shared__ __attribute__((aligned(16))) float2 asx_lds_r[];

#ifdef ASX_STAMPS
#define RSTAMP(kernel, block, slot)                                                                  \
    do {                                                                                             \
        if (P.stamps && P.stamp_kernel == (kernel) && threadIdx.x == 0)                              \
            P.stamps[(size_t)(block) * 8 + (slot)] = clock64();                                      \
    } while (0)
#else
#define RSTAMP(kernel, block, slot) do {} while (0)
#endif

struct RArgs {
    const float2 *tw1, *tw2, *tw_lo, *tw_hi;
    uint32_t N, nout;
    int M1, M2, ntiles;
    float bound_scale;
    unsigned long long *stamps;
    int stamp_kernel;
};
static RArgs rargs_of(const AsxDev &P)
{
    RArgs a;
    a.tw1 = P.tw1; a.tw2 = P.tw2; a.tw_lo = P.tw_lo; a.tw_hi = P.tw_hi;
    a.N = P.N; a.nout = P.nout; a.M1 = P.M1; a.M2 = P.M2; a.ntiles = P.ntiles; a.bound_scale = P.bound_scale;
    a.stamps = P.stamps; a.stamp_kernel = P.stamp_kernel;
    return a;
}
__device__ __forceinline__ float2 tw_F(const RArgs &P, uint32_t p)
{
    const float2 lo = P.tw_lo[p & (ASX_TW_LO - 1u)];
    const float2 hi = P.tw_hi[p >> ASX_TW_LOG];
    return cmul(lo, hi);
}

__device__ __forceinline__ Cx1 lds_get1(const float4 *p)
{
    const float2 x = *reinterpret_cast<const float2 *>(p);
    return Cx1{ x.x, x.y };
}
__device__ __forceinline__ void lds_put1(float4 *p, Cx1 v) { *reinterpret_cast<float2 *>(p) = make_float2(v.re, v.im); }

__device__ __forceinline__ void wave_lds_sync()
{
    asm volatile("s_waitcnt lgkmcnt(0)" ::: "memory");
    __builtin_amdgcn_fence(__ATOMIC_RELEASE, "wavefront");
    __builtin_amdgcn_wave_barrier();
    __builtin_amdgcn_fence(__ATOMIC_ACQUIRE, "wavefront");
}

__device__ __forceinline__ float quad_sum(float v)
{
    v += __int_as_float(__builtin_amdgcn_mov_dpp(__float_as_int(v), 0xB1, 0xF, 0xF, true));
    v += __int_as_float(__builtin_amdgcn_mov_dpp(__float_as_int(v), 0x4E, 0xF, 0xF, true));
    return v;
}
__device__ __forceinline__ float row16_sum(float v)
{
    v = quad_sum(v);
    v += __int_as_float(__builtin_amdgcn_mov_dpp(__float_as_int(v), 0x141, 0xF, 0xF, true));
    v += __int_as_float(__builtin_amdgcn_mov_dpp(__float_as_int(v), 0x140, 0xF, 0xF, true));
    return v;
}
template <int N> __device__ __forceinline__ float tree_sum(const float (&p)[N])
{
    if constexpr (N == 1) return p[0];
    else {
        float q[(N + 1) / 2];
        static_for<0, N / 2>([&](auto I) __attribute__((always_inline)) { q[I] = p[2 * decltype(I)::value] + p[2 * decltype(I)::value + 1]; });
        if constexpr (N & 1) q[N / 2] = p[N - 1];
        return tree_sum<(N + 1) / 2>(q);
    }
}

#ifdef ASX_EXP_PAIRMOD
#define RWS_PAIR(pair) ((pair) % (ASX_EXP_PAIRMOD))
#else
#define RWS_PAIR(pair) (pair)
#endif
#ifndef ASX_RNT
#define ASX_RNT 15
#endif
typedef float asx_f4v __attribute__((ext_vector_type(4)));
__device__ __forceinline__ float4 ld_f4(const void *p, bool nt)
{
    if (nt) { const asx_f4v v = __builtin_nontemporal_load(reinterpret_cast<const asx_f4v *>(p)); return make_float4(v.x, v.y, v.z, v.w); }
    return *reinterpret_cast<const float4 *>(p);
}
__device__ __forceinline__ void st_f4(void *p, float4 v, bool nt)
{
    if (nt) { asx_f4v w; w.x = v.x; w.y = v.y; w.z = v.z; w.w = v.w; __builtin_nontemporal_store(w, reinterpret_cast<asx_f4v *>(p)); }
    else *reinterpret_cast<float4 *>(p) = v;
}
typedef float asx_f2v __attribute__((ext_vector_type(2)));
__device__ __forceinline__ void st_f2(float2 *p, float2 v, bool nt)
{
    if (nt) { asx_f2v w; w.x = v.x; w.y = v.y; __builtin_nontemporal_store(w, reinterpret_cast<asx_f2v *>(p)); }
    else *p = v;
}

#ifndef ASX_ROWS_EARLY
#define ASX_ROWS_EARLY 14
#endif
#ifndef ASX_ROWSR_WAVES
#define ASX_ROWSR_WAVES 4
#endif

__device__ __forceinline__ Cx1 phat_unit(Cx1 q)
{
    const float m = fmaxf(fabsf(q.re), fabsf(q.im));
    const int e = __builtin_amdgcn_frexp_expf(m);
    const float a = ldexpf(q.re, -e), b = ldexpf(q.im, -e);
    const float n2 = fmaf(a, a, b * b);
    float y = __builtin_amdgcn_rsqf(n2);
    y = fmaf(y, fmaf(-0.5f * n2 * y, y, 0.5f), y);
    return m == 0.f ? Cx1{ 0.f, 0.f } : Cx1{ a * y, b * y };
}

template <class S, int NT, bool TWO, int BC, bool ENG = false, bool PHAT = false, bool BAND = false>
__device__ __forceinline__ void rows_r_body(const RArgs P, const float2 *__restrict__ cx, const float2 *__restrict__ cy,
                                            float2 *__restrict__ qo, int nrows, size_t pitch_x, size_t pitch_y, size_t pitch_q,
                                            AsxPeakWs W, const AsxPoolPair *__restrict__ L = nullptr, float *__restrict__ eng = nullptr,
                                            const AsxBand band = {})
{
    static_assert(S::nstages == 3, "three-stage row schedules only");
    static_assert(!BAND || PHAT, "a band is a band of the phase transform");
    constexpr int NS = S::n;
    constexpr int M2 = TWO ? 2 * NS : NS;
    constexpr int TWS = TWO ? 2 : 1;
    constexpr int NTB = TWO ? 2 * NT : NT;
    constexpr StageK K0 = S::stage(0), K1 = S::stage(1), K2 = S::stage(2);
    constexpr int R0 = K0.R, R1 = K1.R, R2 = K2.R;
    constexpr int Q0 = K0.q;
    constexpr int UN = K1.ns;
    static_assert(UN == R1 * R2 && Q0 == UN && K2.q == 1, "unit = R1 x R2");
    static_assert((NS & 1) == 0, "rows move as 16 bytes per lane");
    constexpr int HALF = NS / 2, WSTEPS = (HALF + NTB - 1) / NTB;
    constexpr int LPU = R1 > R2 ? R1 : R2, UPW = 64 / LPU, NW = NT / 64;
    static_assert(NT % 64 == 0 && UPW >= 1, "whole waves");
    constexpr bool XNT = (BC & 1) == 0, YNT = (BC & 2) == 0;

#ifdef ASX_STAMPS
    const long long t_entry = clock64(), w_entry = wall_clock64();
#endif
    const int task = blockIdx.x, tid = threadIdx.x;
    const int half = TWO ? tid / NT : 0, lt = tid - half * NT;
    float4 *A4 = reinterpret_cast<float4 *>(asx_lds_r) + half * NS;
    __shared__ float2 tw_step[WSTEPS];
    __shared__ float2 leg[R0];

    const int pair = task / nrows;
    const uint32_t k1 = (uint32_t)(task - pair * nrows);
    const size_t row = (size_t)RWS_PAIR(pair) * pitch_q + (size_t)k1 * M2;
    size_t rowx, rowy;
    if constexpr ((BC & 4) != 0) {
        rowx = (size_t)L[pair].sx * pitch_x + (size_t)k1 * M2;
        rowy = (size_t)L[pair].sy * pitch_y + (size_t)k1 * M2;
    } else {
        rowx = (size_t)RWS_PAIR(pair) * pitch_x + (size_t)k1 * M2;
        rowy = (size_t)RWS_PAIR(pair) * pitch_y + (size_t)k1 * M2;
    }
    if (k1 == 0 && tid < 64) {
        const float *np = W.nrm_part + (size_t)pair * 2 * P.ntiles;
        float sx = 0.f, sy = 0.f;
        for (int t = tid; t < P.ntiles; t += 64) { sx += np[t]; sy += np[P.ntiles + t]; }
        sx = wave_sum_f32(sx); sy = wave_sum_f32(sy);
        if (tid == 0) {
            if constexpr (PHAT) W.bound2[pair] = (sx != 0.f && sy != 0.f) ? 1.17549435e-38f : 0.f;
            else W.bound2[pair] = P.bound_scale * sqrtf(sx) * sqrtf(sy);
            W.pairmax[pair] = 0;
            W.cand_n[pair] = 0;
        }
    }
    constexpr bool LOOKUPS_FIRST = (ASX_ROWS_EARLY & 8) != 0 && (TWO || NS != 1200);
    const bool is_step = tid < WSTEPS, is_leg = tid >= NTB - R0;
    static_assert(WSTEPS <= NTB - R0, "the threads that fill tw_step and leg are different threads");
    float2 pre_lo = make_float2(1.f, 0.f), pre_hi = pre_lo;
    if ((LOOKUPS_FIRST || (ASX_ROWS_EARLY & 1)) && (is_step || is_leg)) {
        const uint32_t p = is_step ? k1 * (uint32_t)(2 * NTB * tid) : k1 * (uint32_t)(Q0 * (tid - (NTB - R0)));
        pre_lo = P.tw_lo[p & (ASX_TW_LO - 1u)];
        pre_hi = P.tw_hi[p >> ASX_TW_LOG];
    }
    float2 tail_w2 = make_float2(1.f, 0.f), tail_lo = tail_w2, tail_hi = tail_w2;
    if (TWO && (ASX_ROWS_EARLY & 2) && tid < Q0) {
        const uint32_t p = k1 * (uint32_t)tid;
        tail_w2 = P.tw2[tid];
        tail_lo = P.tw_lo[p & (ASX_TW_LO - 1u)];
        tail_hi = P.tw_hi[p >> ASX_TW_LOG];
    }
    float4 w2pre[TWO ? WSTEPS : 1];
    if constexpr (TWO && (ASX_ROWS_EARLY & 4) != 0) {
        static_for<0, WSTEPS>([&](auto I) __attribute__((always_inline)) {
            constexpr int i = decltype(I)::value;
            const int q = tid + i * NTB;
            w2pre[I] = make_float4(1.f, 0.f, 1.f, 0.f);
            if ((i + 1) * NTB <= HALF || q < HALF) w2pre[I] = *reinterpret_cast<const float4 *>(P.tw2 + 2 * q);
        });
    }
    float4 lx[WSTEPS], ly[WSTEPS], lx2[TWO ? WSTEPS : 1], ly2[TWO ? WSTEPS : 1];
    auto issue_row_loads = [&]() __attribute__((always_inline)) {
        const float2 *gx = cx + rowx, *gy = cy + rowy;
        static_for<0, WSTEPS>([&](auto I) __attribute__((always_inline)) {
            const int q = tid + decltype(I)::value * NTB;
            if (((ASX_ROWS_EARLY & 4) && (decltype(I)::value + 1) * NTB <= HALF) || q < HALF) {
                lx[I] = ld_f4(gx + 2 * q, XNT && (ASX_RNT & 4));
                ly[I] = ld_f4(gy + 2 * q, YNT && (ASX_RNT & 4));
                if constexpr (TWO) {
                    lx2[I] = ld_f4(gx + NS + 2 * q, XNT && (ASX_RNT & 4));
                    ly2[I] = ld_f4(gy + NS + 2 * q, YNT && (ASX_RNT & 4));
                }
            }
        });
    };
    if constexpr (!LOOKUPS_FIRST) issue_row_loads();
    auto publish_step_and_leg = [&]() __attribute__((always_inline)) {
        if (is_step) {
            const float2 t = (LOOKUPS_FIRST || (ASX_ROWS_EARLY & 1)) ? cmul(pre_lo, pre_hi) : tw_F(P, k1 * (uint32_t)(2 * NTB * tid));
            tw_step[tid] = make_float2(0.5f * t.x, 0.5f * t.y);
        }
        if (is_leg) { const int t = tid - (NTB - R0); leg[t] = (LOOKUPS_FIRST || (ASX_ROWS_EARLY & 1)) ? cmul(pre_lo, pre_hi) : tw_F(P, k1 * (uint32_t)(Q0 * t)); }
    };
    if constexpr (!LOOKUPS_FIRST) publish_step_and_leg();
    const float2 twa = tw_F(P, k1 * (uint32_t)(2 * tid < NS ? 2 * tid : 0));
    const float2 wk1 = tw_F(P, k1);
    const float2 wh = TWO ? tw_F(P, k1 * (uint32_t)NS) : make_float2(1.f, 0.f);
    const int j0 = lt < Q0 ? lt : 0;
    const float2 s0w1 = P.tw2[TWS * j0], s0w4 = P.tw2[TWS * 4 * j0];
    const float2 tw0base = TWO ? make_float2(1.f, 0.f) : tw_F(P, k1 * (uint32_t)j0);
    const int lane = tid & 63, wave = lt >> 6;
    const int ul = lane / LPU, jl = lane - ul * LPU;
    const int j1c = jl < R2 ? jl : 0;
    const float2 s1w1 = P.tw2[TWS * K1.twmul * j1c], s1w4 = P.tw2[TWS * (R1 > 4 ? 4 : 1) * K1.twmul * j1c];
    if constexpr (LOOKUPS_FIRST) { issue_row_loads(); publish_step_and_leg(); }
    RSTAMP(0, task, 0);
#ifdef ASX_STAMPS
    if (P.stamps && P.stamp_kernel == 0 && threadIdx.x == 0) { P.stamps[(size_t)task * 8 + 6] = t_entry; P.stamps[(size_t)task * 8 + 7] = w_entry; }
#endif
    __syncthreads();
    static_for<0, WSTEPS>([&](auto I) __attribute__((always_inline)) {
        constexpr int i = decltype(I)::value;
        const int q = tid + i * NTB;
        if (((ASX_ROWS_EARLY & 4) && (i + 1) * NTB <= HALF) || q < HALF) {
            const float2 wa0 = cmul(twa, tw_step[i]), wa1 = cmul(wa0, wk1);
            const Cx2 c0 = mulw(Cx2{ v2f{ lx[I].x, ly[I].x }, v2f{ lx[I].y, ly[I].y } }, wa0);
            const Cx2 c1 = mulw(Cx2{ v2f{ lx[I].z, ly[I].z }, v2f{ lx[I].w, ly[I].w } }, wa1);
            if constexpr (!TWO) {
                lds_put(A4 + 2 * q, c0);
                lds_put(A4 + 2 * q + 1, c1);
            } else {
                float4 *base = reinterpret_cast<float4 *>(asx_lds_r);
                const float2 wb0 = cmul(wa0, wh), wb1 = cmul(wa1, wh);
                const Cx2 d0 = mulw(Cx2{ v2f{ lx2[I].x, ly2[I].x }, v2f{ lx2[I].y, ly2[I].y } }, wb0);
                const Cx2 d1 = mulw(Cx2{ v2f{ lx2[I].z, ly2[I].z }, v2f{ lx2[I].w, ly2[I].w } }, wb1);
                const float4 w2 = (ASX_ROWS_EARLY & 4) ? w2pre[I] : *reinterpret_cast<const float4 *>(P.tw2 + 2 * q);
                lds_put(base + 2 * q, c0 + d0);
                lds_put(base + 2 * q + 1, c1 + d1);
                lds_put(base + NS + 2 * q, mulw(c0 - d0, make_float2(w2.x, w2.y)));
                lds_put(base + NS + 2 * q + 1, mulw(c1 - d1, make_float2(w2.z, w2.w)));
            }
        }
    });
    __syncthreads();
    RSTAMP(0, task, 1);

    for (int j = lt; j < Q0; j += NT) {
        float4 *p = A4 + j;
        Cx2 v[R0];
        static_for<0, R0>([&](auto T) __attribute__((always_inline)) { v[T] = lds_get(p + decltype(T)::value * Q0); });
        float2 w1 = s0w1, w4 = s0w4;
        if (j != lt) { w1 = P.tw2[TWS * j]; w4 = P.tw2[TWS * 4 * j]; }
        float2 tww[R0];
        stage_twiddles_from<R0>(w1, w4, tww);
        Bfly<R0, false>::run(v);
        static_for<1, R0>([&](auto U) __attribute__((always_inline)) { v[U] = mulw(v[U], tww[U]); });
        static_for<0, R0>([&](auto T) __attribute__((always_inline)) { lds_put(p + decltype(T)::value * Q0, v[T]); });
    }
    __syncthreads();
    RSTAMP(0, task, 2);

    for (int u0 = wave * UPW; u0 < R0; u0 += NW * UPW) {
        const int unit = u0 + ul;
        const bool on = (ul < UPW) && (unit < R0);
        float4 *base = A4 + (on ? unit : 0) * UN;
        float2 tw1[R1];
        stage_twiddles_from<R1>(s1w1, s1w4, tw1);
        if (on && jl < R2) {
            float4 *p = base + jl;
            Cx2 v[R1];
            static_for<0, R1>([&](auto T) __attribute__((always_inline)) { v[T] = lds_get(p + decltype(T)::value * R2); });
            Bfly<R1, false>::run(v);
            static_for<1, R1>([&](auto U) __attribute__((always_inline)) { v[U] = mulw(v[U], tw1[U]); });
            static_for<0, R1>([&](auto T) __attribute__((always_inline)) { lds_put(p + decltype(T)::value * R2, v[T]); });
        }
        wave_lds_sync();
        if (on && jl < R1) {
            float4 *p = base + jl * R2;
            Cx2 v[R2];
            static_for<0, R2>([&](auto T) __attribute__((always_inline)) { v[T] = lds_get(p + decltype(T)::value); });
            Bfly<R2, false>::run(v);
            Cx1 pr[R2];
            static_for<0, R2>([&](auto T) __attribute__((always_inline)) {
                pr[T] = Cx1{ v[T].re.x * v[T].re.y + v[T].im.x * v[T].im.y, v[T].im.x * v[T].re.y - v[T].re.x * v[T].im.y };
            });
            if constexpr (PHAT) static_for<0, R2>([&](auto T) __attribute__((always_inline)) { pr[T] = phat_unit(pr[T]); });
            if constexpr (BAND) {
                constexpr uint32_t HS = TWO ? 2u : 1u;
                const uint32_t F = 2u * P.N, m2 = 2u * (uint32_t)P.M1;
                const uint32_t k0 = k1 + m2 * (HS * (uint32_t)(unit + R0 * jl) + (uint32_t)half), kstep = m2 * (HS * R0 * R1);
                static_for<0, R2>([&](auto T) __attribute__((always_inline)) {
                    const uint32_t k = k0 + (uint32_t) decltype(T)::value * kstep;
                    const bool in = (k - band.lo <= band.span) || (F - k - band.lo <= band.span);
                    pr[T] = in ? pr[T] : Cx1{ 0.f, 0.f };
                });
            }
            Bfly<R2, true>::run(pr);
            static_for<0, R2>([&](auto T) __attribute__((always_inline)) { lds_put1(p + decltype(T)::value, pr[T]); });
        }
        wave_lds_sync();
        if (on && jl < R2) {
            float4 *p = base + jl;
            Cx1 v[R1];
            static_for<0, R1>([&](auto T) __attribute__((always_inline)) { v[T] = lds_get1(p + decltype(T)::value * R2); });
            static_for<1, R1>([&](auto U) __attribute__((always_inline)) { v[U] = mulwc(v[U], tw1[U]); });
            Bfly<R1, true>::run(v);
            static_for<0, R1>([&](auto T) __attribute__((always_inline)) { lds_put1(p + decltype(T)::value * R2, v[T]); });
        }
    }
    __syncthreads();
    RSTAMP(0, task, 3);

    float2 *go = qo + row;
    static_assert(!ENG || (ASX_PRUNE_T == 16 && M2 % ASX_PRUNE_T == 0 && NTB % ASX_PRUNE_T == 0 && 16 * M2 < 65536),
                  "tile energies: tiles of sixteen columns, a tile per row of sixteen lanes");
    auto eng_base = [](int j) __attribute__((always_inline)) { return reinterpret_cast<float *>(asx_lds_r) + 4 * j + 2; };
    auto eng_put = [](float *ej, int c0, Cx1 y) __attribute__((always_inline)) { ej[4 * c0] = fmaf(y.re, y.re, y.im * y.im); };
    if constexpr (!TWO) {
        for (int j = lt; j < Q0; j += NT) {
            [[maybe_unused]] float *const ej = eng_base(j);
            const float4 *p = A4 + j;
            Cx1 v[R0];
            static_for<0, R0>([&](auto T) __attribute__((always_inline)) { v[T] = lds_get1(p + decltype(T)::value * Q0); });
            float2 w1 = s0w1, w4 = s0w4, fb = tw0base;
            if (j != lt) { w1 = P.tw2[j]; w4 = P.tw2[4 * j]; fb = tw_F(P, k1 * (uint32_t)j); }
            float2 tww[R0];
            stage_twiddles_from<R0>(w1, w4, tww);
            static_for<1, R0>([&](auto U) __attribute__((always_inline)) { v[U] = mulwc(v[U], tww[U]); });
            Bfly<R0, true>::run(v);
            static_for<0, R0>([&](auto T) __attribute__((always_inline)) {
                constexpr int t = decltype(T)::value;
                const Cx1 y = mulwc(v[t], t == 0 ? fb : cmul(fb, leg[t]));
                st_f2(go + j + t * Q0, make_float2(y.re, y.im), ASX_RNT & 8);
                if constexpr (ENG) eng_put(ej, t * Q0, y);
            });
        }
    } else {
        const float4 *base = reinterpret_cast<const float4 *>(asx_lds_r);
        static_assert(Q0 <= NT, "one butterfly per thread of the first half");
        for (int j = tid; j < Q0; j += NTB) {
            [[maybe_unused]] float *const ej = eng_base(j);
            Cx2 v[R0];
            static_for<0, R0>([&](auto T) __attribute__((always_inline)) {
                const Cx1 a = lds_get1(base + j + decltype(T)::value * Q0), b = lds_get1(base + NS + j + decltype(T)::value * Q0);
                v[T] = Cx2{ v2f{ a.re, b.re }, v2f{ a.im, b.im } };
            });
            float2 tww[R0];
            if constexpr (ASX_ROWS_EARLY & 2) stage_twiddles_from<R0>(s0w1, s0w4, tww);
            else stage_twiddles_from<R0>(P.tw2[TWS * j], P.tw2[TWS * 4 * j], tww);
            static_for<1, R0>([&](auto U) __attribute__((always_inline)) { v[U] = mulwc(v[U], tww[U]); });
            Bfly<R0, true>::run(v);
            const float2 w2 = (ASX_ROWS_EARLY & 2) ? tail_w2 : P.tw2[j];
            const float2 fa = (ASX_ROWS_EARLY & 2) ? cmul(tail_lo, tail_hi) : tw_F(P, k1 * (uint32_t)j);
            const float2 fbh = cmul(fa, wh);
            static_for<0, R0>([&](auto T) __attribute__((always_inline)) {
                constexpr int t = decltype(T)::value;
                const Cx1 A = Cx1{ v[t].re.x, v[t].im.x };
                const Cx1 Bw = mul_root<2 * R0, t, true>(mulwc(Cx1{ v[t].re.y, v[t].im.y }, w2));
                const float2 lg = leg[t];
                const Cx1 y = mulwc(A + Bw, t == 0 ? fa : cmul(fa, lg));
                const Cx1 z = mulwc(A - Bw, t == 0 ? fbh : cmul(fbh, lg));
                st_f2(go + j + t * Q0, make_float2(y.re, y.im), ASX_RNT & 8);
                st_f2(go + NS + j + t * Q0, make_float2(z.re, z.im), ASX_RNT & 8);
                if constexpr (ENG) { eng_put(ej, t * Q0, y); eng_put(ej, NS + t * Q0, z); }
            });
        }
    }
    if constexpr (ENG) {
        __syncthreads();
        constexpr int NTILE = M2 / ASX_PRUNE_T, ESTEPS = (M2 + NTB - 1) / NTB;
        const float *er = eng_base(tid);
        float *eo = eng + ((size_t)pair * nrows + k1) * NTILE + (tid >> 4);
        float v[ESTEPS];
        static_for<0, ESTEPS>([&](auto I) __attribute__((always_inline)) {
            constexpr int i = decltype(I)::value;
            v[I] = ((i + 1) * NTB <= M2 || tid + i * NTB < M2) ? er[4 * NTB * i] : 0.f;
        });
        static_for<0, ESTEPS>([&](auto I) __attribute__((always_inline)) { v[I] = row16_sum(v[I]); });
        if ((tid & 15) == 0)
            static_for<0, ESTEPS>([&](auto I) __attribute__((always_inline)) {
                constexpr int i = decltype(I)::value;
                if ((i + 1) * NTB <= M2 || tid + i * NTB < M2) eo[(NTB / 16) * i] = v[I];
            });
    }
    RSTAMP(0, task, 4);
#ifdef ASX_STAMPS
    if (P.stamps && P.stamp_kernel == 0 && threadIdx.x == 0) P.stamps[(size_t)task * 8 + 5] = wall_clock64();
#endif
}

template <class S, int NT, bool TWO, int BC>
__global__ __launch_bounds__(TWO ? 2 * NT : NT, ASX_ROWSR_WAVES) void k_rows_r(const RArgs P, const float2 *__restrict__ cx,
                                                                                const float2 *__restrict__ cy, float2 *__restrict__ qo,
                                                                                int nrows, size_t pair_pitch, AsxPeakWs W)
{
    rows_r_body<S, NT, TWO, BC>(P, cx, cy, qo, nrows, (BC & 1) ? 0 : pair_pitch, (BC & 2) ? 0 : pair_pitch, pair_pitch, W);
}

template <class S, int NT, bool TWO>
__global__ __launch_bounds__(TWO ? 2 * NT : NT, ASX_ROWSR_WAVES) void k_rows_re(const RArgs P, const float2 *__restrict__ cx,
                                                                                 const float2 *__restrict__ cy, float2 *__restrict__ qo,
                                                                                 int nrows, size_t pair_pitch, AsxPeakWs W,
                                                                                 float *__restrict__ eng)
{
    rows_r_body<S, NT, TWO, 0, true>(P, cx, cy, qo, nrows, pair_pitch, pair_pitch, pair_pitch, W, nullptr, eng);
}

template <class S, int NT, bool TWO, int BC>
__global__ __launch_bounds__(TWO ? 2 * NT : NT, ASX_ROWSR_WAVES) void k_rows_rp(const RArgs P, const float2 *__restrict__ cx,
                                                                                 const float2 *__restrict__ cy, float2 *__restrict__ qo,
                                                                                 int nrows, size_t pair_pitch, AsxPeakWs W)
{
    rows_r_body<S, NT, TWO, BC, false, true>(P, cx, cy, qo, nrows, (BC & 1) ? 0 : pair_pitch, (BC & 2) ? 0 : pair_pitch, pair_pitch, W);
}

template <class S, int NT, bool TWO, int BC>
__global__ __launch_bounds__(TWO ? 2 * NT : NT, ASX_ROWSR_WAVES) void k_rows_rb(const RArgs P, const float2 *__restrict__ cx,
                                                                                 const float2 *__restrict__ cy, float2 *__restrict__ qo,
                                                                                 int nrows, size_t pair_pitch, AsxPeakWs W,
                                                                                 const AsxBand band)
{
    rows_r_body<S, NT, TWO, BC, false, true, true>(P, cx, cy, qo, nrows, (BC & 1) ? 0 : pair_pitch, (BC & 2) ? 0 : pair_pitch, pair_pitch, W,
                                                   nullptr, nullptr, band);
}

template <class S, int NT, bool TWO>
__global__ __launch_bounds__(TWO ? 2 * NT : NT, ASX_ROWSR_WAVES) void k_rows_rl(const RArgs P, const float2 *__restrict__ cx,
                                                                                 const float2 *__restrict__ cy, float2 *__restrict__ qo,
                                                                                 int nrows, size_t pair_pitch, AsxPeakWs W,
                                                                                 const AsxPoolPair *__restrict__ L)
{
    const int pair = blockIdx.x / nrows;
    if (L[pair].flags & ASX_POOL_INVALID) {
        constexpr int M2 = TWO ? 2 * S::n : S::n, NTB = TWO ? 2 * NT : NT;
        const int k1 = blockIdx.x - pair * nrows;
        float2 *go = qo + (size_t)pair * pair_pitch + (size_t)k1 * M2;
        for (int j = threadIdx.x; j < M2; j += NTB) go[j] = make_float2(NAN, NAN);
        if (k1 == 0 && threadIdx.x == 0) {
            W.bound2[pair] = 0.f;
            W.pairmax[pair] = 0;
            W.cand_n[pair] = 0;
        }
        return;
    }
    rows_r_body<S, NT, TWO, 7>(P, cx, cy, qo, nrows, pair_pitch, pair_pitch, pair_pitch, W, L);
}

__device__ __host__ constexpr int rcol_line_log(int logT) { return logT >= 5 ? 0 : 5 - logT; }
__device__ __forceinline__ int rcol_tile_of_block(int b, int logT)
{
    const int ll = rcol_line_log(logT);
    const int grp = 8 << ll;
    return (b & ~(grp - 1)) + ((b & 7) << ll) + ((b >> 3) & ((1 << ll) - 1));
}
static inline unsigned rcol_grid_x(int ntiles, int logT)
{
    const unsigned grp = 8u << rcol_line_log(logT);
    return ((unsigned)ntiles + grp - 1) / grp * grp;
}

#ifndef ASX_SPECIAL_LAST
#define ASX_SPECIAL_LAST 1
#endif
template <int NITEMS, int H, int NT> __device__ __forceinline__ int rcol_item_of_thread(int t)
{
    constexpr bool own_wave = NITEMS - H <= NT - 64;
    if (!ASX_SPECIAL_LAST || !own_wave) return t < NITEMS ? t : -1;
    return t < NITEMS - H ? t + H : t >= NT - H ? t - (NT - H) : -1;
}
#ifndef ASX_INV_WU
#define ASX_INV_WU 1
#endif
#ifndef ASX_RCOL_LOADS
#define ASX_RCOL_LOADS 5
#endif

template <class S1, int TC, int NT, bool NTS>
__global__ __launch_bounds__(NT, 4) void k_fwd_cols_r(const RArgs P, const float *__restrict__ src, const float *__restrict__ smp,
                                                       size_t src_stride, size_t smp_stride, float2 *__restrict__ cx,
                                                       float2 *__restrict__ cy, float *__restrict__ nrm_part, size_t pair_pitch,
                                                       float2 *__restrict__ band, unsigned op0)
{
    constexpr int M1 = S1::n, T = TC, logT = asx_ilog2(TC), H = T / 2, logH = logT - 1, Q4 = T / 4, logQ4 = logT - 2;
    static_assert(T >= 4 && (M1 & 1) == 0, "four real columns per 16-byte load, an even number of packed rows");
    __shared__ float nrm_red[NT / 64];
    const unsigned which = op0 + blockIdx.y;
    const bool is_smp = which != 0;
    const size_t pair = blockIdx.z;
    const int tile = rcol_tile_of_block(blockIdx.x, logT);
    if (tile >= P.ntiles) return;
    const int M2 = P.M2, c0 = tile * T;
    const float *in = is_smp ? smp + pair * smp_stride : src + pair * src_stride;
    const int data_m = is_smp ? M1 / 2 : M1;
    float2 *out = (is_smp ? cy : cx) + RWS_PAIR(pair) * pair_pitch;
    float4 *lds4 = reinterpret_cast<float4 *>(asx_lds_r);
    const LdsLayout Lc = col_layout(T, logT, NT);
    const TwPre pre = tw_prefetch_first<S1, false, true>(Lc, P.tw1);

    constexpr int QN = NT / Q4, RPQ = rcol_rows_per_group(M1, NT, T);
    static_assert(Q4 == 4, "sixteen real columns: four lanes per row pair (the quad reductions below)");
    static_assert(M1 % RPQ == 0 && (M1 / 2) % RPQ == 0 && RPQ <= ASX_RCOL_LOADS && RPQ * QN >= M1, "whole bands in both tracks");
    const int grp = threadIdx.x >> logQ4, h = threadIdx.x & (Q4 - 1), m0 = grp * RPQ;
    float ss = 0.f, q1 = 0.f;
    {
        float4 a[RPQ], b[RPQ];
        float sq[RPQ];
        static_for<0, RPQ>([&](auto I) __attribute__((always_inline)) {
            const int m = m0 + decltype(I)::value;
            a[I] = b[I] = make_float4(0.f, 0.f, 0.f, 0.f);
            if (m < data_m) {
                const float *p = in + (size_t)(2 * m) * M2 + c0 + 4 * h;
                a[I] = *reinterpret_cast<const float4 *>(p);
                b[I] = *reinterpret_cast<const float4 *>(p + M2);
            }
        });
        static_for<0, RPQ>([&](auto I) __attribute__((always_inline)) {
            const int m = m0 + decltype(I)::value;
            if (m < M1) {
                float4 *o = lds4 + (m << logH) + 2 * h;
                o[0] = make_float4(a[I].x, b[I].x, a[I].y, b[I].y);
                o[1] = make_float4(a[I].z, b[I].z, a[I].w, b[I].w);
            }
            sq[I] = fmaf(a[I].x, a[I].x, fmaf(a[I].y, a[I].y, fmaf(a[I].z, a[I].z, a[I].w * a[I].w)));
            sq[I] = fmaf(b[I].x, b[I].x, fmaf(b[I].y, b[I].y, fmaf(b[I].z, b[I].z, fmaf(b[I].w, b[I].w, sq[I]))));
            if (band) q1 += ((a[I].x + a[I].y) + (a[I].z + a[I].w)) + ((b[I].x + b[I].y) + (b[I].z + b[I].w));
        });
        ss = tree_sum<RPQ>(sq);
    }
    if (band) {
        const float r1 = quad_sum(q1), r2 = quad_sum(ss);
        if (h == 0 && m0 < data_m)
            band[(((size_t)pair * 2 + which) * (size_t)P.ntiles + tile) * (size_t)(M1 / RPQ) + grp] = make_float2(r1, r2);
    }
    ss = wave_sum_f32(ss);
    if ((threadIdx.x & 63) == 0) nrm_red[threadIdx.x >> 6] = ss;
    __syncthreads();
    (void)lds_fft_static_head<S1, false, true>(lds4, Lc, P.tw1, pre);
    if (threadIdx.x == NT - H - 1) {
        float t = nrm_red[0];
        for (int w = 1; w < NT / 64; w++) t += nrm_red[w];
        nrm_part[(pair * 2 + which) * (size_t)P.ntiles + tile] = t;
    }
    static_assert(S1::nstages == 3, "three-stage column schedules");
    constexpr int RL = S1::stage(2).R, R0c = S1::stage(0).R, R1c = S1::stage(1).R, MB = M1 / RL;
    static_assert(S1::stage(2).q == 1 && MB == R0c * R1c && MB % 2 == 0, "innermost stage of consecutive slots");
    constexpr int NBPAIRS = (MB / 2) * H;
    static_assert(NBPAIRS <= NT - 1, "one work item per thread at most, none for thread NT - H - 1 (the block's norm)");
    if (const int e = rcol_item_of_thread<NBPAIRS, H, NT>(threadIdx.x); e >= 0) {
        const int g = e & (H - 1), v = e >> logH;
        const int ub = v, ubp = v == 0 ? MB / 2 : MB - v;
        const int d1 = ub / R0c, d0 = ub - d1 * R0c, e1 = ubp / R0c, e0 = ubp - e1 * R0c;
        const float4 *pa = lds4 + (((d0 * R1c + d1) * RL) << logH) + g, *pb = lds4 + (((e0 * R1c + e1) * RL) << logH) + g;
        Cx2 za[RL], zb[RL];
        static_for<0, RL>([&](auto TT) __attribute__((always_inline)) {
            za[TT] = lds_get(pa + (decltype(TT)::value << logH));
            zb[TT] = lds_get(pb + (decltype(TT)::value << logH));
        });
        Bfly<RL, false>::run(za);
// ... 214 lines not shown
        float best_m = -INFINITY;
        last_stage([&](auto RC, auto &v, int g, int pos0, int q) __attribute__((always_inline)) {
            static_for<0, decltype(RC)::value>([&](auto TT) __attribute__((always_inline)) {
                constexpr int t = decltype(TT)::value;
                if constexpr (WIN) {
                    const uint32_t i0 = (uint32_t)(2 * (pos0 + t * q)) * uM2 + (uint32_t)(c0 + 2 * g);
                    const float a0 = inw(i0) ? fabsf(v[t].re.x) : NAN, a1 = inw(i0 + uM2) ? fabsf(v[t].im.x) : NAN;
                    const float a2 = inw(i0 + 1) ? fabsf(v[t].re.y) : NAN, a3 = inw(i0 + uM2 + 1) ? fabsf(v[t].im.y) : NAN;
                    best_m = fmaxf(fmaxf(best_m, fmaxf(a0, a1)), fmaxf(a2, a3));
                } else {
                    best_m = fmaxf(fmaxf(best_m, fmaxf(fabsf(v[t].re.x), fabsf(v[t].im.x))), fmaxf(fabsf(v[t].re.y), fabsf(v[t].im.y)));
                }
            });
        });
        RSTAMP(2, sblock, 4);
        const float wmax = wave_max_nonneg(fmaxf(best_m, 0.f));
        float *redf = reinterpret_cast<float *>(red);
        if ((threadIdx.x & 63) == 0) redf[threadIdx.x >> 6] = wmax;
        __syncthreads();
        float bm = redf[0];
        for (int w = 1; w < NT / 64; w++) bm = fmaxf(bm, redf[w]);
        if (bm < near_max_threshold(peak_key(run0), b2)) return;
        RSTAMP(2, sblock, 5);
        const float thr = near_max_threshold(fmaxf(bm, peak_key(run0)), b2);
        uint32_t my_idx = 0xFFFFFFFFu;
        float my_val = 0.f;
        if (best_m >= thr || best_m == bm) {
            last_stage([&](auto RC, auto &v, int g, int pos0, int q) __attribute__((always_inline)) {
                static_for<0, decltype(RC)::value>([&](auto TT) __attribute__((always_inline)) {
                    constexpr int t = decltype(TT)::value;
                    const float val[4] = { v[t].re.x, v[t].re.y, v[t].im.x, v[t].im.y };
                    const uint32_t i0 = (uint32_t)(2 * (pos0 + t * q)) * uM2 + (uint32_t)(c0 + 2 * g);
#pragma unroll
                    for (int h = 0; h < 4; h++) {
                        const uint32_t idx = i0 + (uint32_t)(h >> 1) * uM2 + (uint32_t)(h & 1);
                        const float a = inw(idx) ? fabsf(val[h]) : NAN;
                        if (a == bm && idx < my_idx) { my_idx = idx; my_val = val[h]; }
                        if (a >= thr) cand_append(W, pair, idx, a);
                    }
                });
            });
        }
        __syncthreads();
        const asx_peak_t mine = my_idx == 0xFFFFFFFFu ? 0 : peak_pack_key(bm, my_idx);
        const asx_peak_t tb = block_peak_max(mine, red);
        if (threadIdx.x == 0) { atomicMax(&W.pairmax[pair], tb); red[0] = tb; }
        __syncthreads();
        if (W.tile_peak && mine != 0 && mine == red[0]) W.tile_peak[pair * (size_t)(P.M2 / T) + tile] = my_val;
    } else {
        float best_key = -INFINITY, best_val = 0.f;
        uint32_t best_idx = 0xFFFFFFFFu;
        last_stage([&](auto RC, auto &v, int g, int pos0, int q) __attribute__((always_inline)) {
            static_for<0, decltype(RC)::value>([&](auto TT) __attribute__((always_inline)) {
                constexpr int t = decltype(TT)::value;
                const float val[4] = { v[t].re.x, v[t].im.x, v[t].re.y, v[t].im.y };
                const uint32_t i0 = (uint32_t)(2 * (pos0 + t * q)) * uM2 + (uint32_t)(c0 + 2 * g);
#pragma unroll
                for (int h = 0; h < 4; h++) {
                    const uint32_t idx = i0 + (uint32_t)(h & 1) * uM2 + (uint32_t)(h >> 1);
                    const float key = shift == 0.0 ? peak_key_of(val[h], idx, seed) : peak_key_shifted(val[h], idx, shift, seed);
                    if (inw(idx) && (key > best_key || (key == best_key && idx < best_idx) || best_idx == 0xFFFFFFFFu)) { best_key = key; best_idx = idx; best_val = val[h]; }
                    if (r_out) r_out[pair * (size_t)P.nout + idx] = val[h];
                }
            });
        });
        const asx_peak_t mine = best_idx == 0xFFFFFFFFu ? 0 : peak_pack_key(best_key, best_idx);
        asx_peak_t best = block_peak_max(mine, red);
        if (threadIdx.x == 0) { atomicMax(&W.pairmax[pair], best); red[0] = best; }
        __syncthreads();
        if (W.tile_peak && mine != 0 && mine == red[0]) W.tile_peak[pair * (size_t)(P.M2 / T) + tile] = best_val;
        const float thr = near_max_threshold(peak_key(peak_max(red[0], run0)), b2);
        again = best_key >= thr;
        thr_again = thr;
    }
    if (again) examine_again(thr_again);
    RSTAMP(2, sblock, 3);
}

#if defined(HIP_VERSION_MAJOR) && HIP_VERSION_MAJOR == 7 && HIP_VERSION_MINOR == 2
constexpr int BOUNDS_TICKET_ORDER = __ATOMIC_RELAXED;
#else
constexpr int BOUNDS_TICKET_ORDER = __ATOMIC_RELEASE;
#endif
constexpr int BOUNDS_ROWS_IN_FLIGHT = 16, BOUNDS_SLICES_IN_FLIGHT = 8;

template <int DEPTH, class Load>
__device__ __forceinline__ double sum_in_order(int n, Load load)
{
    double sum = 0.0;
    for (int i0 = 0; i0 < n; i0 += DEPTH) {
        double v[DEPTH];
#pragma unroll
        for (int i = 0; i < DEPTH; i++) v[i] = load(i0 + i < n ? i0 + i : n - 1);
#pragma unroll
        for (int i = 0; i < DEPTH; i++) sum += i0 + i < n ? v[i] : 0.0;
    }
    return sum;
}

__global__ __launch_bounds__(1024) void k_tile_bounds(const float *__restrict__ eng, float *__restrict__ ub, int *__restrict__ best,
                                                       double *part, unsigned *__restrict__ ticket, int nrows, int ntiles,
                                                       double scale, double floor)
{
    __shared__ unsigned long long tops[16];
    __shared__ int last;
    const size_t pair = blockIdx.x;
    const int tile = threadIdx.x, tp = (ntiles + 31) & ~31, sl = blockIdx.y, nsl = gridDim.y;
    unsigned long long *pp = reinterpret_cast<unsigned long long *>(part + pair * 1024);
    if (tile < ntiles) {
        const float *e = eng + pair * (size_t)nrows * ntiles + (size_t)sl * ntiles + tile;
        const size_t step = (size_t)nsl * ntiles;
        const double sum = sum_in_order<BOUNDS_ROWS_IN_FLIGHT>((nrows - sl + nsl - 1) / nsl,
                                                               [=](int i) { return (double)e[(size_t)i * step]; });
        __hip_atomic_store(pp + sl * tp + tile, (unsigned long long)__double_as_longlong(sum), __ATOMIC_RELAXED,
                           __HIP_MEMORY_SCOPE_AGENT);
    }
    asm volatile("s_waitcnt vmcnt(0)" ::: "memory");
    __syncthreads();
    if (threadIdx.x == 0) {
        const unsigned drawn = __hip_atomic_fetch_add(ticket + pair, 1u, BOUNDS_TICKET_ORDER, __HIP_MEMORY_SCOPE_AGENT);
        last = drawn == (unsigned)nsl - 1u;
        if (last) {
            __hip_atomic_store(ticket + pair, 0u, __ATOMIC_RELAXED, __HIP_MEMORY_SCOPE_AGENT);
            __builtin_amdgcn_fence(__ATOMIC_ACQUIRE, "agent");
            asm volatile("s_waitcnt vmcnt(0)" ::: "memory");
        }
    }
    __syncthreads();
    if (!last) return;
    unsigned long long top = 0;
    if (tile < ntiles) {
        const double s = sum_in_order<BOUNDS_SLICES_IN_FLIGHT>(nsl, [=](int i) {
            return __longlong_as_double((long long)__hip_atomic_load(pp + i * tp + tile, __ATOMIC_RELAXED, __HIP_MEMORY_SCOPE_AGENT));
        });
        const float b = s < floor ? INFINITY : __double2float_ru(sqrt(scale * s) * (1.0 + (double)ASX_PRUNE_DELTA));
        ub[pair * ntiles + tile] = b;
        top = b == b ? ((unsigned long long)__float_as_uint(b) << 32) | (0xFFFFFFFFu - (unsigned)tile) : 0ull;
    }
#pragma unroll
    for (int off = 32; off > 0; off >>= 1) {
        const unsigned hi = __shfl_xor((unsigned)(top >> 32), off, 64), lo = __shfl_xor((unsigned)top, off, 64);
        const unsigned long long o = ((unsigned long long)hi << 32) | lo;
        top = o > top ? o : top;
    }
    if ((threadIdx.x & 63) == 0) tops[threadIdx.x >> 6] = top;
    __syncthreads();
    if (threadIdx.x != 0) return;
    for (int w = 1; w < (int)blockDim.x / 64; w++) top = tops[w] > top ? tops[w] : top;
    best[pair] = top ? (int)(0xFFFFFFFFu - (unsigned)top) : 0;
}

__global__ __launch_bounds__(256) void k_prune_select(const float *__restrict__ ub, const int *__restrict__ best,
                                                       unsigned char *__restrict__ skip, AsxPeakWs W, int ntiles,
                                                       unsigned long long *__restrict__ stats)
{
    __shared__ unsigned kept;
    const size_t pair = blockIdx.x;
    if (threadIdx.x == 0) kept = 0;
    __syncthreads();
    const asx_peak_t pm = W.pairmax[pair];
    const float thr = near_max_threshold(peak_key(pm), W.bound2[pair]);
    const int bt = best[pair];
    unsigned n = 0;
    for (int t = threadIdx.x; t < ntiles; t += 256) {
        const bool sk = t == bt || t == 0 || (pm != 0 && ub[pair * ntiles + t] < thr);
        skip[pair * ntiles + t] = sk ? 1 : 0;
        n += sk ? 0u : 1u;
    }
    if (n) atomicAdd(&kept, n);
    __syncthreads();
    if (threadIdx.x == 0) {
        atomicAdd(&stats[0], (unsigned long long)(kept + (bt == 0 ? 1u : 2u)));
        atomicAdd(&stats[1], (unsigned long long)ntiles);
    }
}

template <class Sel>
__global__ __launch_bounds__(256) void k_phat_finalize(AsxPeakWs W, AsxSeg *__restrict__ seg, double *__restrict__ peak, uint32_t N,
                                                        double f, int npairs, Sel sel)
{
    const int pair = blockIdx.x * 256 + threadIdx.x;
    if (pair >= npairs) return;
    const asx_peak_t best = W.pairmax[pair];
    seg[pair] = make_seg(best ? peak_index(best) : sel.seed_of((size_t)pair, N), N);
    W.refine_n[pair] = 0u;
    if (!peak) return;
    const float key = best ? peak_key(best) : 0.f;
    double v = key == -INFINITY ? (double)NAN : fabs((double)key) / f;
    if constexpr (std::is_same<Sel, AsxWinRows>::value) {
        AsxWin z;
        if (!asx_win_row(sel, (size_t)pair, N, z)) v = (double)NAN;
    }
    peak[pair] = v;
}

template <class K, class... X>
static void launch_rows_r(K kernel, const AsxDev &P, int nt, const AsxSpectra &C, float2 *q, const AsxPeakWs &W, int npairs,
                          hipStream_t s, X... extra)
{
    const int nrows = P.M1 + 1;
    hipLaunchKernelGGL(kernel, dim3((unsigned)nrows * (unsigned)npairs), dim3(nt), (size_t)P.M2 * sizeof(float4), s, rargs_of(P),
                       (const float2 *)C.cx, (const float2 *)C.cy, q, nrows, (size_t)nrows * (size_t)P.M2, W, extra...);
}

void asx_launch_rows_r(const AsxDev &P, const AsxSpectra &C, float2 *q, const AsxPeakWs &W, int npairs, hipStream_t s)
{
    asx_with_entry(AsxRRows{}, P.krows, [&](auto e) {
        using S = typename decltype(e)::sched;
        constexpr int NT = e.nt, nt = e.two ? 2 * NT : NT;
        constexpr bool TWO = e.two;
        if (C.weight == ASX_W_PHAT_BAND)
            switch (C.bc) {
            case 0: launch_rows_r(k_rows_rb<S, NT, TWO, 0>, P, nt, C, q, W, npairs, s, C.fband); break;
            case 1: launch_rows_r(k_rows_rb<S, NT, TWO, 1>, P, nt, C, q, W, npairs, s, C.fband); break;
            case 2: launch_rows_r(k_rows_rb<S, NT, TWO, 2>, P, nt, C, q, W, npairs, s, C.fband); break;
            default: launch_rows_r(k_rows_rb<S, NT, TWO, 3>, P, nt, C, q, W, npairs, s, C.fband); break;
            }
        else if (C.weight == ASX_W_PHAT)
            switch (C.bc) {
            case 0: launch_rows_r(k_rows_rp<S, NT, TWO, 0>, P, nt, C, q, W, npairs, s); break;
            case 1: launch_rows_r(k_rows_rp<S, NT, TWO, 1>, P, nt, C, q, W, npairs, s); break;
            case 2: launch_rows_r(k_rows_rp<S, NT, TWO, 2>, P, nt, C, q, W, npairs, s); break;
            default: launch_rows_r(k_rows_rp<S, NT, TWO, 3>, P, nt, C, q, W, npairs, s); break;
            }
        else if (C.prune) launch_rows_r(k_rows_re<S, NT, TWO>, P, nt, C, q, W, npairs, s, C.prune->eng);
        else if (C.pl) launch_rows_r(k_rows_rl<S, NT, TWO>, P, nt, C, q, W, npairs, s, C.pl);
        else
            switch (C.bc) {
            case 0: launch_rows_r(k_rows_r<S, NT, TWO, 0>, P, nt, C, q, W, npairs, s); break;
            case 1: launch_rows_r(k_rows_r<S, NT, TWO, 1>, P, nt, C, q, W, npairs, s); break;
            case 2: launch_rows_r(k_rows_r<S, NT, TWO, 2>, P, nt, C, q, W, npairs, s); break;
            default: launch_rows_r(k_rows_r<S, NT, TWO, 3>, P, nt, C, q, W, npairs, s); break;
            }
    });
}

void asx_launch_phat_finalize(const AsxDev &P, const AsxPeakWs &W, AsxSeg *seg, double *peak, double f, int npairs, hipStream_t s,
                              const AsxSearch &q)
{
    asx_with_selection(q, [&](auto sel) {
        if constexpr (!std::is_same<decltype(sel), AsxSelTopkSeed>::value)
            hipLaunchKernelGGL(k_phat_finalize<decltype(sel)>, dim3((unsigned)(npairs + 255) / 256), dim3(256), 0, s, W, seg, peak, P.N,
                               f, npairs, sel);
    });
}

static unsigned resident_blocks(const void *fn, int nthreads, size_t lds)
{
    static std::mutex mu;
    static std::map<std::pair<const void *, int>, unsigned> known;
    int dev = 0;
    (void)hipGetDevice(&dev);
    std::lock_guard<std::mutex> lock(mu);
    auto it = known.find({ fn, dev });
    if (it != known.end()) return it->second;
    int per_cu = 0, cus = 0;
    unsigned n = 512;
    if (hipDeviceGetAttribute(&cus, hipDeviceAttributeMultiprocessorCount, dev) == hipSuccess &&
        hipOccupancyMaxActiveBlocksPerMultiprocessor(&per_cu, fn, nthreads, lds) == hipSuccess && per_cu > 0 && cus > 0)
        n = (unsigned)per_cu * (unsigned)cus;
    known[{ fn, dev }] = n;
    return n;
}

void asx_launch_fwd_cols_r(const AsxDev &P, const float *src, size_t src_stride, const float *smp, size_t smp_stride, size_t first,
                           int count, const AsxSpectra &dst, bool temporal, hipStream_t s)
{
    const unsigned op0 = src ? 0 : 1, nops = (src ? 1 : 0) + (smp ? 1 : 0);
    if (nops == 0) return;
    const size_t pitch = asx_spectrum_len(P), lds = (size_t)P.M1 * P.T * sizeof(float2);
    const size_t per = 2 * (size_t)P.ntiles;
    if (src) src += first * src_stride;
    if (smp) smp += first * smp_stride;
    float2 *cx = dst.cx + first * pitch, *cy = dst.cy + first * pitch;
    float2 *band = dst.band ? dst.band + first * per * (size_t)P.nbands : nullptr;
    float *nrm = dst.nrm + first * per;
    const dim3 grid(rcol_grid_x(P.ntiles, P.logT), nops, count);
    auto launch = [&](auto kernel, int nt) {
        allow_big_lds((const void *)kernel, lds);
        hipLaunchKernelGGL(kernel, grid, dim3(nt), lds, s, rargs_of(P), src, smp, src_stride, smp_stride, cx, cy, nrm, pitch, band, op0);
    };
    asx_with_entry(AsxRCols{}, P.kcols, [&](auto e) {
        using S = typename decltype(e)::sched;
        if (temporal) launch(k_fwd_cols_r<S, e.t, e.nt, false>, e.nt);
        else launch(k_fwd_cols_r<S, e.t, e.nt, true>, e.nt);
    });
}

void asx_launch_pool_resolve(const AsxDev &P, const AsxPoolArgs &A, AsxPoolPair *out, float *nrm, float2 *band, int npairs,
                             hipStream_t s)
{
    const int per = std::max(P.ntiles, band ? P.ntiles * P.nbands : 0);
    hipLaunchKernelGGL(k_pool_resolve, dim3((unsigned)(per + 255) / 256, (unsigned)npairs), dim3(256), 0, s, A, out, nrm, band, P.ntiles,
                       P.nbands);
}

void asx_launch_bcast_aux(const AsxDev &P, const float *snrm, const float2 *sband, float *nrm, float2 *band, int npairs,
                          unsigned which, hipStream_t s)
{
    const int per = std::max(P.ntiles, band ? P.ntiles * P.nbands : 0);
    hipLaunchKernelGGL(k_bcast_aux, dim3((unsigned)(per + 255) / 256, (unsigned)npairs), dim3(256), 0, s, snrm, sband, nrm, band,
                       P.ntiles, P.nbands, which);
}

template <class K, class Sel>
static void launch_inv_r(K kernel, const AsxDev &P, dim3 grid, int nt, size_t lds, hipStream_t s, const float2 *q, const AsxPeakWs &W,
                         float *r_out, Sel sel)
{
    const void *fn = (const void *)kernel;
    allow_big_lds(fn, lds);
    hipLaunchKernelGGL(kernel, grid, dim3(nt), lds, s, rargs_of(P), q, asx_spectrum_len(P), W, r_out,
                       resident_blocks(fn, nt, lds), sel);
}

template <class S1, int TC, int NT>
static void launch_inv_rq(const AsxDev &P, const float2 *q, const AsxPeakWs &W, const AsxPrune &U, int npairs, hipStream_t s)
{
    const size_t pitch = asx_spectrum_len(P), lds = (size_t)S1::n * TC * sizeof(float2);
    auto k1 = k_inv_cols_r<S1, TC, NT, AsxSelPrune<true>>;
    auto k2 = k_inv_cols_r<S1, TC, NT, AsxSelPrune<false>>;
    allow_big_lds((const void *)k1, lds);
    allow_big_lds((const void *)k2, lds);
    const int tp = (P.ntiles + 31) & ~31;
    hipLaunchKernelGGL(k_tile_bounds, dim3(npairs, 1024 / tp), dim3((tp + 63) & ~63), 0, s, U.eng, U.ub, U.best, U.part, U.ticket, P.M1 + 1, P.ntiles,
                       4.0 * (double)P.M1, ASX_PRUNE_FLOOR_PER_TERM * (double)ASX_PRUNE_T * (double)(P.M1 + 1));
    hipLaunchKernelGGL(k1, dim3(npairs, 2), dim3(NT), lds, s, rargs_of(P), q, pitch, W, resident_blocks((const void *)k1, NT, lds),
                       AsxSelPrune<true>{ U.best, U.skip });
    hipLaunchKernelGGL(k_prune_select, dim3(npairs), dim3(256), 0, s, U.ub, U.best, U.skip, W, P.ntiles, U.stats);
    hipLaunchKernelGGL(k2, dim3(npairs, rcol_grid_x(P.ntiles, asx_ilog2(TC))), dim3(NT), lds, s, rargs_of(P), q, pitch, W,
                       resident_blocks((const void *)k2, NT, lds), AsxSelPrune<false>{ U.best, U.skip });
}

void asx_launch_inv_cols_r(const AsxDev &P, const float2 *q, const AsxPeakWs &W, float *r_out, int npairs, hipStream_t s,
                           const AsxSearch &search, const AsxPrune *U)
{
    asx_with_entry(AsxRCols{}, P.kcols, [&](auto e) {
        using S = typename decltype(e)::sched;
        constexpr int T = e.t, NT = e.nt;
        const size_t lds = (size_t)S::n * T * sizeof(float2);
        const dim3 grid(npairs, rcol_grid_x(P.M2 / T, asx_ilog2(T)));
        if (U)
            launch_inv_rq<S, T, NT>(P, q, W, *U, npairs, s);
        else
            asx_with_selection<1, 3, ASX_TOPK_MAX - 1>(search, [&](auto sel) {
                launch_inv_r(k_inv_cols_r<S, T, NT, decltype(sel), float>, P, grid, NT, lds, s, q, W, r_out, sel);
            });
    });
}
```

### old-audiosync_amd/hipxcorr.py

```python
import ctypes
import os
import sys

import numpy as np

_HERE = os.path.dirname(os.path.abspath(__file__))
LIB_PATH = os.path.join(_HERE, "libaudiosync_hip.so")
_lib = None

c_f32p = ctypes.POINTER(ctypes.c_float)
c_f64p = ctypes.POINTER(ctypes.c_double)
c_i64p = ctypes.POINTER(ctypes.c_int64)
c_i32p = ctypes.POINTER(ctypes.c_int32)
c_intp = ctypes.POINTER(ctypes.c_int)

_vp, _sz, _int, _i64, _u64, _dbl, _str = (ctypes.c_void_p, ctypes.c_size_t, ctypes.c_int, ctypes.c_int64, ctypes.c_uint64,
                                          ctypes.c_double, ctypes.c_char_p)
_vpp, _szp, _longp = ctypes.POINTER(_vp), ctypes.POINTER(_sz), ctypes.POINTER(ctypes.c_long)
_u32p, _u64p = ctypes.POINTER(ctypes.c_uint32), ctypes.POINTER(ctypes.c_uint64)

_HEADER_SIGNATURES = {
    "asx_device_count": (_int, []),
    "asx_current_device": (_int, []),
    "asx_last_error": (_str, []),
    "asx_abi_version": (_int, []),
    "asx_plan_create": (_vp, [_sz, _sz, _int]),
    "asx_plan_create_ex": (_vp, [_sz, _sz, _int, _str]),
    "asx_plan_destroy": (None, [_vp]),
    "asx_plan_sample_len": (_sz, [_vp]),
    "asx_plan_fft_len": (_sz, [_vp]),
    "asx_plan_group": (_sz, [_vp]),
    "asx_plan_workspace_bytes": (_sz, [_vp]),
    "asx_plan_peak_capacity": (_sz, [_vp]),
    "asx_plan_threads": (_int, [_vp, c_intp, c_intp]),
    "asx_plan_split": (_int, [_vp, c_intp, c_intp, c_intp]),
    "asx_plan_layout": (_int, [_vp]),
    "asx_plan_peak_overflows": (_int, [_vp, _u64p]),
    "asx_plan_peak_repairs": (_int, [_vp, _u64p]),
    "asx_plan_narrowed_calls": (_int, [_vp, _u64p]),
    "asx_plan_set_exact": (_int, [_vp, _int]),
    "asx_plan_set_lag_window": (_int, [_vp, _i64, _i64]),
    "asx_plan_lag_window": (_int, [_vp, c_i64p, c_i64p]),
    "asx_stream_set_lag_window": (_int, [_vp, _i64, _i64]),
    "asx_plan_placement": (_int, [_vp, c_f64p, c_intp]),
    "asx_plan_set_pearson": (_int, [_vp, _int]),
    "asx_plan_pearson_modes": (_int, [_vp, _u64p]),
    "asx_plan_set_prune": (_int, [_vp, _int]),
    "asx_plan_prune_stats": (_int, [_vp, _u64p, _u64p]),
    "asx_plan_set_profiling": (_int, [_vp, _int]),
    "asx_plan_last_timings_ms": (_int, [_vp, c_f32p]),
    "asx_plan_timings_ms": (_int, [_vp, _int, c_f32p]),
    "asx_xcorr_f64": (_int, [_vp, c_f64p, c_f64p, _longp, c_f64p]),
    "asx_xcorr_batch_f32": (_int, [_vp, c_f32p, c_f32p, _sz, c_i64p, c_f64p, c_i32p]),
    "asx_xcorr_batch_multi": (_int, [_vpp, _int, c_f32p, c_f32p, _sz, c_i64p, c_f64p, c_i32p]),
    "asx_xcorr_batch_f32_dev": (_int, [_vp, _vp, _vp, _sz, _vp, _vp, _vp, _vp]),
    "asx_xcorr_strided_f32_dev": (_int, [_vp, _vp, _sz, _vp, _sz, _sz, _vp, _vp, _vp, _vp]),
    "asx_xcorr_windowed_f32_dev": (_int, [_vp, _vp, _sz, _vp, _sz, _vp, _sz, _sz, _vp, _vp, _vp, _vp]),
    "asx_xcorr_topk_f32_dev": (_int, [_vp, _vp, _sz, _vp, _sz, _vp, _sz, _sz, _int, _i64, _vp, _vp, _vp, _vp]),
    "asx_xcorr_phat_f32_dev": (_int, [_vp, _vp, _sz, _vp, _sz, _vp, _sz, _sz, _vp, _vp, _vp, _vp, _vp]),
    "asx_xcorr_phat_band_f32_dev": (_int, [_vp, _vp, _sz, _vp, _sz, _vp, _sz, _sz, _i64, _i64, _vp, _vp, _vp, _vp, _vp]),
    "asx_xcorr_pool_f32_dev": (_int, [_vp, _vp, _sz, _sz, _vp, _sz, _sz, _vp, _vp, _sz, _sz, _vp, _vp, _vp, _vp]),
    "asx_xcorr_pool_topk_f32_dev": (_int, [_vp, _vp, _sz, _sz, _vp, _sz, _sz, _vp, _vp, _sz, _sz, _int, _i64, _vp, _vp, _vp, _vp]),
    "asx_xcorr_debug_r_dev": (_int, [_vp, _vp, _vp, _vp, _vp, _vp, _vp, _vp]),
    "asx_xcorr_phat_debug_r_dev": (_int, [_vp, _vp, _vp, _vp, _vp, _vp, _vp, _vp, _vp]),
    "asx_xcorr_phat_band_debug_r_dev": (_int, [_vp, _vp, _vp, _i64, _i64, _vp, _vp, _vp, _vp, _vp, _vp]),
    "asx_band_bins": (_int, [_sz, _dbl, _dbl, _dbl, c_i64p, c_i64p]),
    "asx_pearson_f64": (_int, [c_f64p, c_f64p, _sz, _int, c_f64p]),
    "asx_results_to_ms_dev": (_int, [_vp, _vp, _vp, _sz, _dbl, _dbl, _vp, _vp, _vp]),
    "asx_topk_best_dev": (_int, [_vp, _vp, _vp, _sz, _int, _vp, _vp, _vp, _vp, _vp]),
    "asx_synth_pairs_dev": (_int, [_u64, _u64, _sz, _sz, _int, _vp, _vp, _vp, _vp]),
    "asx_shard_range": (_int, [_sz, _int, _int, _szp, _szp]),
    "asx_result_bytes": (_sz, [_sz]),
    "asx_comm_create": (_vp, [_vpp, _int]),
    "asx_comm_destroy": (None, [_vp]),
    "asx_xcorr_batch_multi_dev": (_int, [_vp, _vpp, _vpp, _szp, _sz, _vpp]),
    "asx_stream_create": (_vp, [_sz, _int]),
    "asx_stream_destroy": (None, [_vp]),
    "asx_stream_append_f64": (_int, [_vp, c_f64p, _sz, c_f64p, _sz]),
    "asx_stream_lengths": (_int, [_vp, _szp, _szp]),
    "asx_stream_reset": (_int, [_vp]),
    "asx_stream_xcorr": (_int, [_vp, _sz, _longp, c_f64p]),
    "asx_device_malloc": (_vp, [_sz, _int]),
    "asx_device_free": (_int, [_vp]),
    "asx_host_malloc": (_vp, [_sz]),
    "asx_host_free": (_int, [_vp]),
    "asx_memcpy_h2d": (_int, [_vp, _vp, _sz]),
    "asx_memcpy_d2h": (_int, [_vp, _vp, _sz]),
    "asx_stream_sync": (_int, [_vp, _vp]),
}

_DIAGNOSTIC_SIGNATURES = {
    "asx_planmath_describe": (_int, [_sz, _str, _u32p, _u32p, c_intp, c_intp, c_intp, c_intp, c_intp, c_intp, c_intp]),
    "asx_planmath_table": (_int, [_sz, _str, _int, c_intp, _sz]),
    "asx_planmath_twiddles": (_int, [_sz, _str, _int, c_f32p, _sz]),
    "asx_planmath_candidates": (_int, [_sz, _sz, _str, _sz]),
    "asx_planmath_kernels": (_int, [_sz, _str, c_intp, c_intp, c_intp]),
    "asx_planmath_kernel_table": (_int, [_int, _int, c_intp]),
    "asx_plan_debug_kernels": (_int, [_vp, c_intp, c_intp, c_intp]),
    "asx_plan_debug_bank": (_int, [_vp, _u64p, _u64p, _u64p]),
    "asx_plan_debug_prune": (_int, [_vp, _sz, c_f32p, c_intp, _sz]),
    "asx_plan_debug_peak": (_int, [_vp, _sz, c_f32p, _u32p, _u32p, _u64p, _vp, _vp, _sz]),
    "asx_plan_debug_spectral": (_int, [_vp, _sz, c_intp, _vp, _sz, c_f64p, ctypes.POINTER(ctypes.c_longlong), c_f64p]),
    "asx_plan_debug_over_list": (_int, [_vp, _u32p, _u32p]),
    "asx_plan_debug_stamps": (ctypes.c_long, [_vp, _vp, _sz]),
}

SIGNATURES = {**_HEADER_SIGNATURES, **_DIAGNOSTIC_SIGNATURES}

ABI_SYMBOLS = list(_HEADER_SIGNATURES)

TOPK_MAX = 8


class AsxError(RuntimeError):
    pass


def _one_hip_runtime():
    if os.environ.get("ASX_NO_TORCH") == "1" or "torch" in sys.modules:
        return
    try:
        import torch
    except ImportError:
        pass


def lib():
    global _lib
    if _lib is not None:
        return _lib
    if not os.path.exists(LIB_PATH):
        raise AsxError(LIB_PATH + " is missing: run `python -c 'import __graft_entry__ as g; g.build()'` "
                       "(hipcc --offload-arch=gfx950); there is no CPU fallback")
    _one_hip_runtime()
    L = ctypes.CDLL(LIB_PATH)
    for name, (restype, argtypes) in SIGNATURES.items():
        f = getattr(L, name)
        f.restype, f.argtypes = restype, argtypes
    _lib = L
    return L


def _err():
    return lib().asx_last_error().decode("utf-8", "replace")


def _check(rc, message=None):
    if rc != 0:
        raise AsxError(message or _err())


def _handle(ptr):
    if not ptr:
        raise AsxError(_err())
    return ptr


def _counters(fn, handle, count, message=None):
    c = [ctypes.c_uint64(0) for _ in range(count)]
    _check(fn(handle, *c), message)
    return tuple(v.value for v in c)


def abi_version():
    return lib().asx_abi_version()


def device_count():
    return lib().asx_device_count()


def _split_arg(split):
    return split.encode() if split else None


def planmath_describe(sample_len, split=None):
    F, valid = ctypes.c_uint32(), ctypes.c_uint32()
    m1, m2, t, n1, n2 = (ctypes.c_int() for _ in range(5))
    r1 = (ctypes.c_int * 16)()
    r2 = (ctypes.c_int * 16)()
    _check(lib().asx_planmath_describe(sample_len, _split_arg(split), F, valid, m1, m2, t, n1, r1, n2, r2))
    return {"F": F.value, "src_valid": valid.value, "M1": m1.value, "M2": m2.value, "T": t.value,
            "radix1": list(r1[: n1.value]), "radix2": list(r2[: n2.value])}


KERNEL_ENTRY_CAP = 32


def _kernel_entry(v, nhead, flag=None):
    if v[0] < 0:
        return None
    v = list(v)
    head = [bool(x) if i == flag else x for i, x in enumerate(v[:nhead])]
    return (*head, tuple(v[nhead:v.index(0, nhead)]))


def planmath_kernel_table():
    f = lib().asx_planmath_kernel_table
    table = {}
    for which, (name, nhead, flag) in enumerate((("real-column cols", 3, None), ("real-column rows", 3, 1),
                                                 ("packed cols", 4, None), ("packed rows", 3, None))):
# ... 232 lines not shown
            lib().asx_comm_destroy(self._h)
            self._h = None

    def __enter__(self):
        return self

    def __exit__(self, *a):
        self.close()


class Stream:

    def __init__(self, max_sample_len, device=-1):
        self._h = _handle(lib().asx_stream_create(int(max_sample_len), int(device)))
        self._destroy = lib().asx_stream_destroy

    def close(self):
        if getattr(self, "_h", None):
            self._destroy(self._h)
            self._h = None

    __del__ = close

    def append(self, source_frames, sample_frames):
        s = np.ascontiguousarray(source_frames, dtype=np.float64)
        t = np.ascontiguousarray(sample_frames, dtype=np.float64)
        _check(lib().asx_stream_append_f64(self._h, s.ctypes.data_as(c_f64p), s.size, t.ctypes.data_as(c_f64p), t.size))

    def lengths(self):
        a, b = ctypes.c_size_t(), ctypes.c_size_t()
        lib().asx_stream_lengths(self._h, a, b)
        return a.value, b.value

    def reset(self):
        lib().asx_stream_reset(self._h)

    def set_lag_window(self, lo, hi):
        _check(lib().asx_stream_set_lag_window(self._h, int(lo), int(hi)))

    def xcorr(self, sample_len):
        lag = ctypes.c_long(0)
        coef = ctypes.c_double(0.0)
        ret = lib().asx_stream_xcorr(self._h, int(sample_len), ctypes.byref(lag), ctypes.byref(coef))
        return ret, lag.value, coef.value


class _Staging:

    def __init__(self, plan):
        self._plan, self._lib, self._ptrs, self._outs = plan, lib(), [], []

    def __enter__(self):
        return self

    def __exit__(self, *a):
        while self._ptrs:
            self._lib.asx_device_free(self._ptrs.pop())

    def alloc(self, nbytes):
        self._ptrs.append(_handle(self._lib.asx_device_malloc(max(int(nbytes), 16), self._plan.device)))
        return self._ptrs[-1]

    def upload(self, host):
        if host is None:
            return 0
        ptr = self.alloc(host.nbytes)
        _check(self._lib.asx_memcpy_h2d(ptr, host.ctypes.data, host.nbytes))
        return ptr

    def output(self, shape, dtype):
        host = np.zeros(shape, dtype=dtype)
        self._outs.append((host, self.alloc(host.nbytes)))
        return self._outs[-1][1]

    def fetch(self):
        self._plan.sync()
        for host, ptr in self._outs:
            _check(self._lib.asx_memcpy_d2h(host.ctypes.data, ptr, host.nbytes))
        return tuple(host for host, _ in self._outs)


_RESULTS = (np.int64, np.float64, np.int32)
_PHAT_RESULTS = (np.int64, np.float64, np.float64, np.int32)


class Plan:

    def __init__(self, sample_len, max_batch=1, device=-1, split=None):
        self._h = _handle(lib().asx_plan_create_ex(int(sample_len), int(max_batch), int(device), _split_arg(split)))
        self._destroy = lib().asx_plan_destroy
        self.sample_len = int(sample_len)
        self.device = int(device)

    def close(self):
        if getattr(self, "_h", None):
            self._destroy(self._h)
            self._h = None

    __del__ = close

    def __enter__(self):
        return self

    def __exit__(self, *a):
        self.close()

    @property
    def fft_len(self):
        return lib().asx_plan_fft_len(self._h)

    @property
    def group(self):
        return lib().asx_plan_group(self._h)

    @property
    def peak_capacity(self):
        return lib().asx_plan_peak_capacity(self._h)

    def peak_overflows(self):
        return _counters(lib().asx_plan_peak_overflows, self._h, 1)[0]

    def set_lag_window(self, lo, hi):
        _check(lib().asx_plan_set_lag_window(self._h, int(lo), int(hi)))

    @property
    def lag_window(self):
        lo, hi = ctypes.c_int64(0), ctypes.c_int64(0)
        _check(lib().asx_plan_lag_window(self._h, ctypes.byref(lo), ctypes.byref(hi)))
        return lo.value, hi.value

    def set_exact(self, on=True):
        _check(lib().asx_plan_set_exact(self._h, 1 if on else 0))

    def placement(self):
        ms = (ctypes.c_double * 2)()
        kept = ctypes.c_int(-1)
        _check(lib().asx_plan_placement(self._h, ms, ctypes.byref(kept)))
        return (float(ms[0]), float(ms[1])), int(kept.value)

    def set_pearson(self, spectral=True):
        _check(lib().asx_plan_set_pearson(self._h, 1 if spectral else 0))

    def pearson_modes(self):
        c = (ctypes.c_uint64 * 3)()
        _check(lib().asx_plan_pearson_modes(self._h, c))
        return tuple(int(v) for v in c)

    def set_prune(self, on=True):
        _check(lib().asx_plan_set_prune(self._h, 1 if on else 0))

    def prune_stats(self):
        return _counters(lib().asx_plan_prune_stats, self._h, 2)

    def narrowed_calls(self):
        return _counters(lib().asx_plan_narrowed_calls, self._h, 1)[0]

    def peak_repairs(self):
        return _counters(lib().asx_plan_peak_repairs, self._h, 1)[0]

    @property
    def workspace_bytes(self):
        return lib().asx_plan_workspace_bytes(self._h)

    @property
    def split(self):
        a, b, c = ctypes.c_int(), ctypes.c_int(), ctypes.c_int()
        lib().asx_plan_split(self._h, a, b, c)
        return a.value, b.value, c.value

    @property
    def layout(self):
        return "real-column" if lib().asx_plan_layout(self._h) == 1 else "packed"

    @property
    def threads(self):
        a, b = ctypes.c_int(), ctypes.c_int()
        lib().asx_plan_threads(self._h, a, b)
        return a.value, b.value

    def xcorr_f64(self, source, sample):
        s = np.ascontiguousarray(source, dtype=np.float64)
        t = np.ascontiguousarray(sample, dtype=np.float64)
        assert t.size == self.sample_len and s.size == 2 * self.sample_len
        lag = ctypes.c_long(0)
        coef = ctypes.c_double(0.0)
        ret = lib().asx_xcorr_f64(self._h, s.ctypes.data_as(c_f64p), t.ctypes.data_as(c_f64p),
                                  ctypes.byref(lag), ctypes.byref(coef))
        return ret, lag.value, coef.value

    def xcorr_batch_f32(self, source, sample):
        s = np.ascontiguousarray(source, dtype=np.float32)
        t = np.ascontiguousarray(sample, dtype=np.float32)
        n = self.sample_len
        batch = t.size // n
        assert t.size == batch * n and s.size == 2 * n * batch
        lag = np.zeros(batch, dtype=np.int64)
        coef = np.zeros(batch, dtype=np.float64)
        ret = np.zeros(batch, dtype=np.int32)
        _check(lib().asx_xcorr_batch_f32(self._h, s.ctypes.data_as(c_f32p), t.ctypes.data_as(c_f32p), batch,
                                         lag.ctypes.data_as(c_i64p), coef.ctypes.data_as(c_f64p), ret.ctypes.data_as(c_i32p)))
        return lag, coef, ret

    def xcorr_batch_dev(self, d_src, d_smp, batch, d_lag, d_coef, d_ret, stream=0):
        _check(lib().asx_xcorr_batch_f32_dev(self._h, d_src, d_smp, batch, d_lag or None, d_coef, d_ret or None, stream or None))

    def xcorr_strided_dev(self, d_src, src_stride, d_smp, smp_stride, batch, d_lag, d_coef, d_ret, stream=0):
        _check(lib().asx_xcorr_strided_f32_dev(self._h, d_src, int(src_stride), d_smp, int(smp_stride), int(batch), d_lag or None,
                                               d_coef, d_ret or None, stream or None))

    def xcorr_windowed_dev(self, d_src, src_stride, d_smp, smp_stride, d_windows, window_stride, batch, d_lag, d_coef, d_ret,
                           stream=0):
        _check(lib().asx_xcorr_windowed_f32_dev(self._h, d_src, int(src_stride), d_smp, int(smp_stride), d_windows, int(window_stride),
                                                int(batch), d_lag or None, d_coef, d_ret, stream or None))

    def xcorr_phat_dev(self, d_src, src_stride, d_smp, smp_stride, d_windows, window_stride, batch, d_lag, d_coef, d_peak, d_ret,
                       stream=0):
        _check(lib().asx_xcorr_phat_f32_dev(self._h, d_src or None, int(src_stride), d_smp or None, int(smp_stride), d_windows or None,
                                            int(window_stride), int(batch), d_lag or None, d_coef or None, d_peak or None,
                                            d_ret or None, stream or None))

    def phat_debug_r_dev(self, d_src, d_smp, d_r, d_lag, d_coef, d_peak, d_ret, stream=0):
        _check(lib().asx_xcorr_phat_debug_r_dev(self._h, d_src or None, d_smp or None, d_r or None, d_lag or None, d_coef or None,
                                                d_peak or None, d_ret or None, stream or None))

    def xcorr_phat_band_dev(self, d_src, src_stride, d_smp, smp_stride, d_windows, window_stride, batch, bin_lo, bin_hi, d_lag, d_coef,
                            d_peak, d_ret, stream=0):
        _check(lib().asx_xcorr_phat_band_f32_dev(self._h, d_src or None, int(src_stride), d_smp or None, int(smp_stride),
                                                 d_windows or None, int(window_stride), int(batch), int(bin_lo), int(bin_hi),
                                                 d_lag or None, d_coef or None, d_peak or None, d_ret or None, stream or None))

    def phat_band_debug_r_dev(self, d_src, d_smp, bin_lo, bin_hi, d_r, d_lag, d_coef, d_peak, d_ret, stream=0):
        _check(lib().asx_xcorr_phat_band_debug_r_dev(self._h, d_src or None, d_smp or None, int(bin_lo), int(bin_hi), d_r or None,
                                                     d_lag or None, d_coef or None, d_peak or None, d_ret or None, stream or None))

    def xcorr_topk_dev(self, d_src, src_stride, d_smp, smp_stride, d_windows, window_stride, batch, k, min_separation, d_lag, d_coef,
                       d_ret, stream=0):
        _check(lib().asx_xcorr_topk_f32_dev(self._h, d_src, int(src_stride), d_smp, int(smp_stride), d_windows or None,
                                            int(window_stride), int(batch), int(k), int(min_separation), d_lag or None, d_coef,
                                            d_ret or None, stream or None))

    def xcorr_pool_dev(self, d_sources, source_stride, nsources, d_samples, sample_stride, nsamples, d_pairs, d_windows, window_stride,
                       batch, d_lag, d_coef, d_ret, stream=0):
        _check(lib().asx_xcorr_pool_f32_dev(self._h, d_sources, int(source_stride), int(nsources), d_samples, int(sample_stride),
                                            int(nsamples), d_pairs or None, d_windows or None, int(window_stride), int(batch),
                                            d_lag or None, d_coef, d_ret, stream or None))

    def xcorr_pool_topk_dev(self, d_sources, source_stride, nsources, d_samples, sample_stride, nsamples, d_pairs, d_windows,
                            window_stride, batch, k, min_separation, d_lag, d_coef, d_ret, stream=0):
        _check(lib().asx_xcorr_pool_topk_f32_dev(self._h, d_sources, int(source_stride), int(nsources), d_samples, int(sample_stride),
                                                 int(nsamples), d_pairs or None, d_windows or None, int(window_stride), int(batch),
                                                 int(k), int(min_separation), d_lag or None, d_coef, d_ret, stream or None))

    def debug_prune(self, pair=0):
        n = (self.split[1] + self.split[2] - 1) // self.split[2]
        ub = (ctypes.c_float * n)()
        best = ctypes.c_int(-1)
        _check(lib().asx_plan_debug_prune(self._h, int(pair), ub, ctypes.byref(best), n), "asx_plan_debug_prune failed")
        return np.frombuffer(ub, dtype=np.float32).copy(), int(best.value)

    def debug_peak(self, pair=0):
        cap = self.peak_capacity
        b2, cn, rn, pm = ctypes.c_float(), ctypes.c_uint32(), ctypes.c_uint32(), ctypes.c_uint64()
        vals, idxs = np.zeros(cap, dtype=np.float64), np.zeros(cap, dtype=np.uint32)
        _check(lib().asx_plan_debug_peak(self._h, int(pair), ctypes.byref(b2), ctypes.byref(cn), ctypes.byref(rn), ctypes.byref(pm),
                                         vals.ctypes.data, idxs.ctypes.data, cap), "asx_plan_debug_peak failed")
        key = index = None
        if pm.value:
            hi = pm.value >> 32
            hi = (hi & 0x7FFFFFFF) if hi & 0x80000000 else (~hi & 0xFFFFFFFF)
            key = float(np.array([hi], dtype=np.uint32).view(np.float32)[0])
            index = 0xFFFFFFFF - (pm.value & 0xFFFFFFFF)
        n = min(int(rn.value), cap)
        return {"bound2": float(b2.value), "cand_n": int(cn.value), "refine_n": int(rn.value), "key": key, "index": index,
                "refine_idx": idxs[:n].astype(np.int64), "refine_val": vals[:n].copy()}

    def debug_spectral(self, pair=0):
        ntiles = (self.split[1] + self.split[2] - 1) // self.split[2]
        f = lib().asx_plan_debug_spectral
        dims, hdr, seg, pick = (ctypes.c_int * 4)(), (ctypes.c_double * 4)(), (ctypes.c_longlong * 6)(), (ctypes.c_double * 8)()
        _check(f(self._h, int(pair), dims, None, 0, hdr, seg, pick),
               "asx_plan_debug_spectral failed (a real-column plan that has run a group?)")
        assert dims[0] == ntiles, (dims[0], ntiles)
        band = np.zeros((2, dims[0], dims[1], 2), dtype=np.float32)
        _check(f(self._h, int(pair), dims, band.ctypes.data, band.size, hdr, seg, pick), "asx_plan_debug_spectral failed")
        return {"band": band, "nbands": dims[1], "band_rows": dims[2], "prep_blocks": dims[3],
                "r": hdr[0], "rb": hdr[1], "direct": hdr[2] != 0.0, "mode": int(hdr[3]),
                "seg": dict(zip(("lag", "src_off", "smp_off", "len", "peak", "flags"), (int(v) for v in seg))),
                "pick": dict(zip(("mode", "n", "Sx", "Sxx", "Sy", "Syy", "r", "bound"),
                                 (int(pick[0]),) + tuple(float(v) for v in pick[1:])))}

    def debug_kernels(self):
        f = lib().asx_plan_debug_kernels
        return _kernel_choice(lambda *a: f(self._h, *a))

    def debug_bank(self):
        return _counters(lib().asx_plan_debug_bank, self._h, 3, "asx_plan_debug_bank failed")

    def debug_over_list(self):
        d, h = ctypes.c_uint32(0), ctypes.c_uint32(0)
        _check(lib().asx_plan_debug_over_list(self._h, ctypes.byref(d), ctypes.byref(h)), "asx_plan_debug_over_list failed")
        return d.value, h.value

    def debug_stamps(self, cap):
        buf = np.zeros(int(cap), dtype=np.uint64)
        got = lib().asx_plan_debug_stamps(self._h, buf.ctypes.data, buf.size)
        if got < 0:
# ... 94 lines not shown
```

Before: 59160 cross-correlations/s.

## Store only predicted-peak tiles of row-FFT output, redo pairs on misprediction

Splits the row pass into a first batch of rows that computes tile energies, a prediction kernel that picks the few high-energy tiles per pair, and a second batch that writes only those predicted tiles of the spectrum to global memory. The aim is to cut the large write traffic of the intermediate row output when pruning leaves only a few tiles. If pruning later needs a tile that was not stored, the pair is flagged and recomputed in full on the host overflow path. This adds an extra launch and a host round-trip for mispredicted pairs.

```diff
diff --git a/include/audiosync/xcorr_hip.h b/include/audiosync/xcorr_hip.h
--- a/include/audiosync/xcorr_hip.h
+++ b/include/audiosync/xcorr_hip.h
@@ -35,6 +35,9 @@
 
 int asx_plan_set_prune(asx_plan *plan, int on);
 int asx_plan_prune_stats(asx_plan *plan, uint64_t *tiles_transformed, uint64_t *tiles_total);
+
+int asx_plan_set_qstore(asx_plan *plan, int mode);
+int asx_plan_qstore_stats(asx_plan *plan, uint64_t out[4]);
 
 size_t asx_plan_sample_len(const asx_plan *plan);
 size_t asx_plan_fft_len(const asx_plan *plan);
diff --git a/old-audiosync_amd/csrc/asx_api.hip b/old-audiosync_amd/csrc/asx_api.hip
--- a/old-audiosync_amd/csrc/asx_api.hip
+++ b/old-audiosync_amd/csrc/asx_api.hip
@@ -147,6 +147,9 @@
     bool prunable = false;
     bool prune = false;
     unsigned long long *prune_stats = nullptr;
+    int qstore = 1;
+    unsigned long long *qstore_stats = nullptr;
+    uint64_t qstore_redone = 0;
     bool tune_placement = false, placement_done = false;
     double placement_ms[2] = { 0.0, 0.0 };
     int placement_kept = -1;
@@ -273,8 +276,15 @@
             }
             if (dev_alloc(m, &ln.prune.eng, g * ((size_t)h.M1 + 1) * (size_t)h.ntiles) || dev_alloc(m, &ln.prune.ub, g * (size_t)h.ntiles) ||
                 dev_alloc(m, &ln.prune.best, g) || dev_alloc(m, &ln.prune.skip, g * (size_t)h.ntiles) ||
-                dev_alloc(m, &ln.prune.part, g * 1024) || dev_alloc(m, &ln.prune.ticket, g))
+                dev_alloc(m, &ln.prune.part, g * 1024) || dev_alloc(m, &ln.prune.ticket, g) || dev_alloc(m, &ln.prune.list, g) ||
+                dev_alloc(m, &ln.prune.redo, g))
                 return -1;
+            if (!p->qstore_stats) {
+                if (dev_alloc(m, &p->qstore_stats, 4)) return -1;
+                HIP_TRY(hipMemset(p->qstore_stats, 0, 4 * sizeof(unsigned long long)));
+            }
+            HIP_TRY(hipMemset(ln.prune.redo, 0, g));
+            ln.prune.qstats = p->qstore_stats;
             HIP_TRY(hipMemset(ln.prune.part, 0, g * 1024 * sizeof(double)));
             HIP_TRY(hipMemset(ln.prune.ticket, 0, g * sizeof(unsigned)));
             ln.prune.stats = p->prune_stats;
@@ -304,6 +314,7 @@
     if (const char *e = getenv("ASX_PEARSON")) p->spectral = p->spectral && strcmp(e, "direct") != 0;
     p->prune = p->prunable;
     if (const char *e = getenv("ASX_PRUNE")) p->prune = p->prune && atoi(e) != 0;
+    if (const char *e = getenv("ASX_QSTORE")) p->qstore = std::min(2, std::max(0, atoi(e)));
     if (const char *e = getenv("ASX_EXACT")) p->exact = atoi(e) != 0;
     p->win_lo = -(int64_t)p->host.N;
     p->win_hi = (int64_t)p->host.N - 1;
@@ -530,6 +541,29 @@
     return 0;
 }
 
+extern "C" int asx_plan_set_qstore(asx_plan *p, int mode)
+{
+    if (!p) return fail("asx_plan_set_qstore: null argument");
+    if (mode < 0 || mode > 2) return fail("asx_plan_set_qstore: mode %d (0 off, 1 auto, 2 always)", mode);
+    std::lock_guard<std::mutex> guard(p->lock);
+    p->qstore = mode;
+    return 0;
+}
+
+extern "C" int asx_plan_qstore_stats(asx_plan *p, uint64_t out[4])
+{
+    if (!p || !out) return fail("asx_plan_qstore_stats: null argument");
+    PlanCall c(p);
+    if (!c.dg.ok) return fail("cannot select device %d", p->device);
+    out[0] = out[1] = out[2] = out[3] = 0;
+    if (!p->qstore_stats) return 0;
+    HIP_TRY(hipDeviceSynchronize());
+    unsigned long long v[4];
+    HIP_TRY(hipMemcpy(v, p->qstore_stats, sizeof v, hipMemcpyDeviceToHost));
+    out[0] = v[0]; out[1] = v[1]; out[2] = p->qstore_redone; out[3] = v[3];
+    return 0;
+}
+
 extern "C" int asx_plan_peak_repairs(asx_plan *p, uint64_t *count)
 {
     if (!p || !count) return fail("asx_plan_peak_repairs: null argument");
@@ -762,6 +796,7 @@
     Topk topk{};
     AsxWeight weight = ASX_W_NONE;
     AsxBand fband{};
+    bool qstore = true;
 };
 
 template <typename TIn>
@@ -782,8 +817,13 @@
     const bool prune = p->prune && !phat && f32_entry && !x.pool && x.bc == 0 && !o.r_out && !o.pk && o.topk.k == 1 && call.kind == AsxSearch::ALL;
     const AsxPoolPair *pl = x.pool ? W.pool : nullptr;
     const AsxSpectra &from = pl ? p->bank.c : p->bslot;
+    AsxPrune U = W.prune;
+    U.q_rows = (prune && o.listed && o.qstore && fin.over_list) ? asx_qstore_rows(P, (int)g, p->qstore) : 0;
+    U.q_row_a = P.M1 / 3;
+    U.pair_base = o.pair_base;
+    if (!U.q_rows) { U.list = nullptr; U.redo = nullptr; }
     const AsxSpectra C{ (pl || (x.bc & 1)) ? from.cx : W.zxa, (pl || (x.bc & 2)) ? from.cy : W.zya, pk.nrm_part, tk.band, x.bc, pl,
-                        prune ? &W.prune : nullptr, o.weight, o.fband };
+                        prune ? &U : nullptr, o.weight, o.fband };
     if (mark(0)) return -1;
     if (pl) {
         const AsxPoolArgs A{ x.pool->rows, (uint64_t)x.first, (uint64_t)x.pool->nsrc, (uint64_t)x.pool->nsmp, (uint64_t)x.src_step,
@@ -833,6 +873,7 @@
         return 0;
     };
     if (pass(call, true)) return -1;
+    if (U.q_rows && spectral) asx_launch_qstore_takeback(U, W.spec, (int)g, s);
     if (call.kind == AsxSearch::ROWS && K == 1) asx_launch_invalid_rows(call.rows, P.N, y.lag, y.coef, y.ret, (int)g, s);
     if (pl && K == 1) asx_launch_invalid_pairs(pl, y.lag, y.coef, y.ret, (int)g, s);
     for (int j = 0; K > 1 && j < K; j++) {
@@ -881,42 +922,56 @@
 template <typename TIn>
 static int resolve_overflows(asx_plan *p, const Pairs<TIn> &x, const Results &y, hipStream_t s, const Topk &topk = {})
 {
-    HIP_TRY(hipStreamSynchronize(s));
-    if (p->lanes[0].pk.cap >= 2 * p->host.N) return 0;
-    const uint32_t n = *p->h_over_n;
-    if (n == 0) return 0;
-    if (n > p->over_cap) {
-        (void)hipMemsetAsync(p->over_n, 0, sizeof(uint32_t), s);
-        (void)hipStreamSynchronize(s);
+    int total = 0;
+    for (int round = 0; round < 2; round++) {
+        HIP_TRY(hipStreamSynchronize(s));
+        if (p->lanes[0].pk.cap >= 2 * p->host.N) return total;
+        const uint32_t n = *p->h_over_n;
+        if (n == 0) return total;
+        if (n > p->over_cap) {
+            (void)hipMemsetAsync(p->over_n, 0, sizeof(uint32_t), s);
+            (void)hipStreamSynchronize(s);
+            *p->h_over_n = 0;
+            return fail("internal: %u overflowed pairs in a window of %zu", n, p->over_cap);
+        }
+        p->h_over.resize(n);
+        HIP_TRY(hipMemcpyAsync(p->h_over.data(), p->over_list, n * sizeof(uint32_t), hipMemcpyDeviceToHost, s));
+        HIP_TRY(hipMemsetAsync(p->over_n, 0, sizeof(uint32_t), s));
+        std::vector<int32_t> ab;
+        if (x.pool) {
+            ab.resize(2 * (size_t)n);
+            for (uint32_t k = 0; k < n; k++) {
+                const size_t pi = x.first + (p->h_over[k] & ~ASX_QSTORE_REDO);
+                if (x.pool->rows)
+                    HIP_TRY(hipMemcpyAsync(&ab[2 * k], x.pool->rows + 2 * pi, 2 * sizeof(int32_t), hipMemcpyDeviceToHost, s));
+                else { ab[2 * k] = (int32_t)(pi / x.pool->nsmp); ab[2 * k + 1] = (int32_t)(pi % x.pool->nsmp); }
+            }
+        }
+        HIP_TRY(hipStreamSynchronize(s));
         *p->h_over_n = 0;
-        return fail("internal: %u overflowed pairs in a window of %zu", n, p->over_cap);
-    }
-    p->h_over.resize(n);
-    HIP_TRY(hipMemcpyAsync(p->h_over.data(), p->over_list, n * sizeof(uint32_t), hipMemcpyDeviceToHost, s));
-    HIP_TRY(hipMemsetAsync(p->over_n, 0, sizeof(uint32_t), s));
-    std::vector<int32_t> ab;
-    if (x.pool) {
-        ab.resize(2 * (size_t)n);
+        const std::vector<uint32_t> list = p->h_over;
+        uint32_t redone = 0;
         for (uint32_t k = 0; k < n; k++) {
-            const size_t pi = x.first + p->h_over[k];
-            if (x.pool->rows)
-                HIP_TRY(hipMemcpyAsync(&ab[2 * k], x.pool->rows + 2 * pi, 2 * sizeof(int32_t), hipMemcpyDeviceToHost, s));
-            else { ab[2 * k] = (int32_t)(pi / x.pool->nsmp); ab[2 * k + 1] = (int32_t)(pi % x.pool->nsmp); }
+            const uint32_t i = list[k] & ~ASX_QSTORE_REDO;
+            Pairs<TIn> xi = x.at(i);
+            if (list[k] & ASX_QSTORE_REDO) {
+                if (run_group(p, xi, 1, y.at(i), s, { .prof_group = GroupOpts::no_marks, .pair_base = i, .topk = topk, .qstore = false }))
+                    return -1;
+                p->qstore_redone++;
+                redone++;
+                continue;
+            }
+            if (x.pool) {
+                const int64_t a = ab[2 * k], b = ab[2 * k + 1];
+                if (a < 0 || (size_t)a >= x.pool->nsrc || b < 0 || (size_t)b >= x.pool->nsmp) continue;
+                xi = xi.pool_pair((size_t)a, (size_t)b, p->host.N);
+            }
+            if (second_look(p, xi, y.at(i), s, topk)) return -1;
         }
-    }
-    HIP_TRY(hipStreamSynchronize(s));
-    *p->h_over_n = 0;
-    for (uint32_t k = 0; k < n; k++) {
-        const uint32_t i = p->h_over[k];
-        Pairs<TIn> xi = x.at(i);
-        if (x.pool) {
-            const int64_t a = ab[2 * k], b = ab[2 * k + 1];
-            if (a < 0 || (size_t)a >= x.pool->nsrc || b < 0 || (size_t)b >= x.pool->nsmp) continue;
-            xi = xi.pool_pair((size_t)a, (size_t)b, p->host.N);
-        }
-        if (second_look(p, xi, y.at(i), s, topk)) return -1;
-    }
-    return (int)n;
+        total += (int)n;
+        if (!redone) return total;
+    }
+    return total;
 }
 
 template <typename TIn>
diff --git a/old-audiosync_amd/csrc/asx_internal.h b/old-audiosync_amd/csrc/asx_internal.h
--- a/old-audiosync_amd/csrc/asx_internal.h
+++ b/old-audiosync_amd/csrc/asx_internal.h
@@ -17,6 +17,18 @@
 #define ASX_PRUNE_DELTA 6.103515625e-5f
 #define ASX_PRUNE_FLOOR_PER_TERM 3.944304526105059e-31
 #define ASX_PRUNE_T 16
+#define ASX_Q_ALL 0xFFFFFFFFFFFFFFFFull
+#define ASX_QSTORE_C 1.75
+#define ASX_QSTORE_REDO 0x80000000u
+__host__ __device__ inline bool asx_q_stored(unsigned long long w, int tile)
+{
+    const unsigned t = (unsigned)tile;
+    return w == ASX_Q_ALL || (unsigned)(w & 0xFFFFu) == t || (unsigned)((w >> 16) & 0xFFFFu) == t ||
+           (unsigned)((w >> 32) & 0xFFFFu) == t || (unsigned)((w >> 48) & 0xFFFFu) == t;
+}
+struct AsxRowRun {
+    int row_a = 0, count = 0, hop = 0;
+};
 #define ASX_CAND_MAX 16384
 #define ASX_CAND_MIN 2048
 #define ASX_DOT_BLOCKS 128
@@ -259,6 +271,11 @@
     unsigned *ticket;
     unsigned char *skip;
     unsigned long long *stats;
+    unsigned long long *list;
+    unsigned char *redo;
+    unsigned long long *qstats;
+    int q_rows, q_row_a;
+    uint32_t pair_base;
 };
 
 struct AsxSelAll {
@@ -281,6 +298,7 @@
 template <bool FIRST> struct AsxSelPrune {
     const int *__restrict__ best;
     const unsigned char *__restrict__ skip;
+    const unsigned long long *__restrict__ list;
     static constexpr bool masks = false;
     __device__ __forceinline__ AsxWin window_of(size_t, uint32_t) const { return AsxWin{}; }
 };
@@ -290,7 +308,8 @@
 {
     if constexpr (FIRST) {
         const int bt = q.best[blockIdx.x];
-        return blockIdx.y == 0 || bt != 0;
+        if (blockIdx.y == 0) return !q.list || asx_q_stored(q.list[blockIdx.x], bt);
+        return bt != 0;
     } else {
         return grid_tile * T < M2 && !q.skip[(size_t)blockIdx.x * (size_t)(M2 / T) + grid_tile];
     }
@@ -358,6 +377,8 @@
 void asx_launch_fwd_cols_r(const AsxDev &P, const float *src, size_t src_stride, const float *smp, size_t smp_stride, size_t first,
                            int count, const AsxSpectra &dst, bool temporal, hipStream_t s);
 void asx_launch_rows_r(const AsxDev &P, const AsxSpectra &C, float2 *q, const AsxPeakWs &W, int npairs, hipStream_t s);
+int asx_qstore_rows(const AsxDev &P, int npairs, int mode);
+void asx_launch_qstore_takeback(const AsxPrune &U, const AsxSpecWs &S, int npairs, hipStream_t s);
 void asx_launch_inv_cols_r(const AsxDev &P, const float2 *q, const AsxPeakWs &W, float *r_out, int npairs, hipStream_t s,
                            const AsxSearch &search, const AsxPrune *U);
 void asx_launch_phat_finalize(const AsxDev &P, const AsxPeakWs &W, AsxSeg *seg, double *peak, double f, int npairs, hipStream_t s,
diff --git a/old-audiosync_amd/csrc/rlayout.hip b/old-audiosync_amd/csrc/rlayout.hip
--- a/old-audiosync_amd/csrc/rlayout.hip
+++ b/old-audiosync_amd/csrc/rlayout.hip
@@ -127,12 +127,14 @@
     return m == 0.f ? Cx1{ 0.f, 0.f } : Cx1{ a * y, b * y };
 }
 
-template <class S, int NT, bool TWO, int BC, bool ENG = false, bool PHAT = false, bool BAND = false>
+template <class S, int NT, bool TWO, int BC, bool ENG = false, bool PHAT = false, bool BAND = false, bool MSK = false>
 __device__ __forceinline__ void rows_r_body(const RArgs P, const float2 *__restrict__ cx, const float2 *__restrict__ cy,
                                             float2 *__restrict__ qo, int nrows, size_t pitch_x, size_t pitch_y, size_t pitch_q,
                                             AsxPeakWs W, const AsxPoolPair *__restrict__ L = nullptr, float *__restrict__ eng = nullptr,
-                                            const AsxBand band = {})
-{
+                                            const AsxBand band = {}, const AsxRowRun run = {},
+                                            const unsigned long long *__restrict__ list = nullptr)
+{
+    static_assert(!MSK || (ENG && TWO), "partial storing: the two-half form, with the tile energies");
     static_assert(S::nstages == 3, "three-stage row schedules only");
     static_assert(!BAND || PHAT, "a band is a band of the phase transform");
     constexpr int NS = S::n;
@@ -159,8 +161,12 @@
     __shared__ float2 tw_step[WSTEPS];
     __shared__ float2 leg[R0];
 
-    const int pair = task / nrows;
-    const uint32_t k1 = (uint32_t)(task - pair * nrows);
+    const int pair = MSK ? task / run.count : task / nrows;
+    uint32_t k1 = (uint32_t)(task - pair * (MSK ? run.count : nrows));
+    if constexpr (MSK) k1 += (int)k1 >= run.row_a ? (uint32_t)run.hop : 0u;
+    unsigned long long wl = ASX_Q_ALL;
+    if constexpr (MSK) { if (list) wl = list[pair]; }
+    [[maybe_unused]] const bool part = MSK && wl != ASX_Q_ALL;
     const size_t row = (size_t)RWS_PAIR(pair) * pitch_q + (size_t)k1 * M2;
     size_t rowx, rowy;
     if constexpr ((BC & 4) != 0) {
@@ -381,17 +387,30 @@
             const float2 w2 = (ASX_ROWS_EARLY & 2) ? tail_w2 : P.tw2[j];
             const float2 fa = (ASX_ROWS_EARLY & 2) ? cmul(tail_lo, tail_hi) : tw_F(P, k1 * (uint32_t)j);
             const float2 fbh = cmul(fa, wh);
-            static_for<0, R0>([&](auto T) __attribute__((always_inline)) {
-                constexpr int t = decltype(T)::value;
-                const Cx1 A = Cx1{ v[t].re.x, v[t].im.x };
-                const Cx1 Bw = mul_root<2 * R0, t, true>(mulwc(Cx1{ v[t].re.y, v[t].im.y }, w2));
-                const float2 lg = leg[t];
-                const Cx1 y = mulwc(A + Bw, t == 0 ? fa : cmul(fa, lg));
-                const Cx1 z = mulwc(A - Bw, t == 0 ? fbh : cmul(fbh, lg));
-                st_f2(go + j + t * Q0, make_float2(y.re, y.im), ASX_RNT & 8);
-                st_f2(go + NS + j + t * Q0, make_float2(z.re, z.im), ASX_RNT & 8);
-                if constexpr (ENG) { eng_put(ej, t * Q0, y); eng_put(ej, NS + t * Q0, z); }
-            });
+            auto leave = [&](auto PART) __attribute__((always_inline)) {
+                static_for<0, R0>([&](auto T) __attribute__((always_inline)) {
+                    constexpr int t = decltype(T)::value;
+                    const Cx1 A = Cx1{ v[t].re.x, v[t].im.x };
+                    const Cx1 Bw = mul_root<2 * R0, t, true>(mulwc(Cx1{ v[t].re.y, v[t].im.y }, w2));
+                    const float2 lg = leg[t];
+                    const Cx1 y = mulwc(A + Bw, t == 0 ? fa : cmul(fa, lg));
+                    const Cx1 z = mulwc(A - Bw, t == 0 ? fbh : cmul(fbh, lg));
+                    if constexpr (decltype(PART)::value) {
+                        ej[4 * (t * Q0) - 2] = y.re; ej[4 * (t * Q0) - 1] = y.im;
+                        ej[4 * (NS + t * Q0) - 2] = z.re; ej[4 * (NS + t * Q0) - 1] = z.im;
+                    } else {
+                        st_f2(go + j + t * Q0, make_float2(y.re, y.im), ASX_RNT & 8);
+                        st_f2(go + NS + j + t * Q0, make_float2(z.re, z.im), ASX_RNT & 8);
+                    }
+                    if constexpr (ENG) { eng_put(ej, t * Q0, y); eng_put(ej, NS + t * Q0, z); }
+                });
+            };
+            if constexpr (MSK) {
+                if (part) leave(std::true_type{});
+                else leave(std::false_type{});
+            } else {
+                leave(std::false_type{});
+            }
         }
     }
     if constexpr (ENG) {
@@ -410,6 +429,16 @@
                 constexpr int i = decltype(I)::value;
                 if ((i + 1) * NTB <= M2 || tid + i * NTB < M2) eo[(NTB / 16) * i] = v[I];
             });
+        if constexpr (MSK) {
+            if (part && tid < 64) {
+                const unsigned t = (unsigned)(wl >> (16 * (tid >> 4))) & 0xFFFFu;
+                if (t < (unsigned)NTILE) {
+                    const int c = (int)t * ASX_PRUNE_T + (tid & 15);
+                    const float *sl = reinterpret_cast<const float *>(asx_lds_r) + 4 * c;
+                    st_f2(go + c, make_float2(sl[0], sl[1]), ASX_RNT & 8);
+                }
+            }
+        }
     }
     RSTAMP(0, task, 4);
 #ifdef ASX_STAMPS
@@ -432,6 +461,17 @@
                                                                                  float *__restrict__ eng)
 {
     rows_r_body<S, NT, TWO, 0, true>(P, cx, cy, qo, nrows, pair_pitch, pair_pitch, pair_pitch, W, nullptr, eng);
+}
+
+template <class S, int NT, bool TWO>
+__global__ __launch_bounds__(TWO ? 2 * NT : NT, ASX_ROWSR_WAVES) void k_rows_rm(const RArgs P, const float2 *__restrict__ cx,
+                                                                                 const float2 *__restrict__ cy, float2 *__restrict__ qo,
+                                                                                 int nrows, size_t pair_pitch, AsxPeakWs W,
+                                                                                 float *__restrict__ eng, const AsxRowRun run,
+                                                                                 const unsigned long long *__restrict__ list)
+{
+    rows_r_body<S, NT, TWO, 0, true, false, false, true>(P, cx, cy, qo, nrows, pair_pitch, pair_pitch, pair_pitch, W, nullptr, eng, {}, run,
+                                                          list);
 }
 
 template <class S, int NT, bool TWO, int BC>
@@ -952,27 +992,94 @@
 
 __global__ __launch_bounds__(256) void k_prune_select(const float *__restrict__ ub, const int *__restrict__ best,
                                                        unsigned char *__restrict__ skip, AsxPeakWs W, int ntiles,
-                                                       unsigned long long *__restrict__ stats)
-{
-    __shared__ unsigned kept;
+                                                       unsigned long long *__restrict__ stats, const unsigned long long *__restrict__ list,
+                                                       unsigned char *__restrict__ redo, uint32_t pair_base)
+{
+    __shared__ unsigned kept, short_of;
     const size_t pair = blockIdx.x;
-    if (threadIdx.x == 0) kept = 0;
+    if (threadIdx.x == 0) { kept = 0; short_of = 0; }
     __syncthreads();
     const asx_peak_t pm = W.pairmax[pair];
     const float thr = near_max_threshold(peak_key(pm), W.bound2[pair]);
     const int bt = best[pair];
-    unsigned n = 0;
+    const unsigned long long w = list ? list[pair] : ASX_Q_ALL;
+    unsigned n = 0, miss = asx_q_stored(w, bt) ? 0u : 1u;
     for (int t = threadIdx.x; t < ntiles; t += 256) {
         const bool sk = t == bt || t == 0 || (pm != 0 && ub[pair * ntiles + t] < thr);
         skip[pair * ntiles + t] = sk ? 1 : 0;
         n += sk ? 0u : 1u;
+        miss |= (!sk && !asx_q_stored(w, t)) ? 1u : 0u;
     }
     if (n) atomicAdd(&kept, n);
-    __syncthreads();
+    if (miss) atomicOr(&short_of, 1u);
+    __syncthreads();
+    const bool again = short_of != 0;
+    if (again)
+        for (int t = threadIdx.x; t < ntiles; t += 256) skip[pair * ntiles + t] = 1;
     if (threadIdx.x == 0) {
-        atomicAdd(&stats[0], (unsigned long long)(kept + (bt == 0 ? 1u : 2u)));
+        const unsigned first = 1u + ((bt != 0 && asx_q_stored(w, bt)) ? 1u : 0u);
+        atomicAdd(&stats[0], (unsigned long long)((again ? 0u : kept) + first));
         atomicAdd(&stats[1], (unsigned long long)ntiles);
-    }
+        if (list) redo[pair] = again ? 1 : 0;
+        if (again) {
+            W.pairmax[pair] = 0;
+            W.cand_n[pair] = 0;
+            if (W.over_list) {
+                const uint32_t slot = atomicAdd(W.over_n, 1u);
+                if (slot < W.over_cap) W.over_list[slot] = (pair_base + (uint32_t)pair) | ASX_QSTORE_REDO;
+                if (W.over_host) (void)__hip_atomic_fetch_add(W.over_host, 1u, __ATOMIC_RELAXED, __HIP_MEMORY_SCOPE_SYSTEM);
+            }
+        }
+    }
+}
+
+__global__ __launch_bounds__(256) void k_q_predict(const float *__restrict__ eng, int nrows, int ntiles, int row_a, int r0, double c,
+                                                    unsigned long long *__restrict__ list, unsigned long long *__restrict__ qstats)
+{
+    __shared__ double p[256];
+    __shared__ double med;
+    __shared__ unsigned pick[3];
+    const size_t pair = blockIdx.x;
+    const int t = threadIdx.x;
+    double mine = 0.0;
+    if (t < ntiles) {
+        const float *e = eng + (pair * (size_t)nrows + (size_t)row_a) * ntiles + t;
+        for (int i = 0; i < r0; i++) mine += (double)e[(size_t)i * ntiles];
+        p[t] = mine;
+    }
+    if (t == 0) med = (double)NAN;
+    if (t < 3) pick[t] = 0xFFFFu;
+    __syncthreads();
+    int below = 0, above = 0;
+    if (t < ntiles)
+        for (int o = 0; o < ntiles; o++) {
+            const double v = p[o];
+            below += (v < mine || (v == mine && o < t)) ? 1 : 0;
+            above += (o != 0 && (v > mine || (v == mine && o < t))) ? 1 : 0;
+        }
+    if (t < ntiles && below == ntiles / 2) med = mine;
+    __syncthreads();
+    if (t > 0 && t < ntiles && above < 3 && mine > c * med) pick[above] = (unsigned)t;
+    __syncthreads();
+    if (t != 0) return;
+    unsigned long long w = ASX_Q_ALL;
+    unsigned stored = (unsigned)ntiles;
+    if (pick[0] != 0xFFFFu || mine > c * med) {
+        w = 0ull | ((unsigned long long)pick[0] << 16) | ((unsigned long long)pick[1] << 32) | ((unsigned long long)pick[2] << 48);
+        stored = 1u + (pick[0] != 0xFFFFu ? 1u : 0u) + (pick[1] != 0xFFFFu ? 1u : 0u) + (pick[2] != 0xFFFFu ? 1u : 0u);
+    }
+    list[pair] = w;
+    atomicAdd(&qstats[w == ASX_Q_ALL ? 1 : 0], 1ull);
+    atomicAdd(&qstats[3], (unsigned long long)stored);
+}
+
+__global__ __launch_bounds__(256) void k_qstore_takeback(const unsigned char *__restrict__ redo, const double *__restrict__ hdr,
+                                                          unsigned long long *__restrict__ mode_count, int npairs)
+{
+    const int pair = blockIdx.x * 256 + threadIdx.x;
+    if (pair >= npairs || !redo[pair]) return;
+    const int mode = (int)hdr[(size_t)pair * ASX_SPEC_HDR + 3];
+    if (mode >= 0 && mode < ASX_PM_NMODES) atomicAdd(&mode_count[mode], ~0ull);
 }
 
 template <class Sel>
@@ -1023,6 +1130,21 @@
             case 2: launch_rows_r(k_rows_rp<S, NT, TWO, 2>, P, nt, C, q, W, npairs, s); break;
             default: launch_rows_r(k_rows_rp<S, NT, TWO, 3>, P, nt, C, q, W, npairs, s); break;
             }
+        else if (C.prune && C.prune->list) {
+            if constexpr (TWO) {
+                const AsxPrune &U = *C.prune;
+                const int nrows = P.M1 + 1, r0 = U.q_rows, a = U.q_row_a;
+                auto rows = [&](AsxRowRun run, const unsigned long long *list) {
+                    hipLaunchKernelGGL((k_rows_rm<S, NT, TWO>), dim3((unsigned)run.count * (unsigned)npairs), dim3(nt),
+                                       (size_t)P.M2 * sizeof(float4), s, rargs_of(P), (const float2 *)C.cx, (const float2 *)C.cy, q, nrows,
+                                       (size_t)nrows * (size_t)P.M2, W, U.eng, run, list);
+                };
+                rows(AsxRowRun{ 0, r0, a }, nullptr);
+                hipLaunchKernelGGL(k_q_predict, dim3(npairs), dim3(256), 0, s, U.eng, nrows, P.ntiles, a, r0, (double)ASX_QSTORE_C, U.list,
+                                   U.qstats);
+                rows(AsxRowRun{ a, nrows - r0, r0 }, U.list);
+            }
+        }
         else if (C.prune) launch_rows_r(k_rows_re<S, NT, TWO>, P, nt, C, q, W, npairs, s, C.prune->eng);
         else if (C.pl) launch_rows_r(k_rows_rl<S, NT, TWO>, P, nt, C, q, W, npairs, s, C.pl);
         else
@@ -1061,6 +1183,29 @@
         n = (unsigned)per_cu * (unsigned)cus;
     known[{ fn, dev }] = n;
     return n;
+}
+
+constexpr int ASX_QSTORE_MIN_GENS = 8;
+int asx_qstore_rows(const AsxDev &P, int npairs, int mode)
+{
+    int r0 = 0;
+    if (mode <= 0 || npairs <= 0 || P.ntiles > 256 || P.M1 + 1 < 64) return 0;
+    asx_with_entry(AsxRRows{}, P.krows, [&](auto e) {
+        using S = typename decltype(e)::sched;
+        constexpr int NT = e.nt;
+        if constexpr (e.two) {
+            if (mode >= 2) { r0 = 8; return; }
+            const unsigned res = resident_blocks((const void *)k_rows_rm<S, NT, true>, 2 * NT, (size_t)P.M2 * sizeof(float4));
+            if ((size_t)(P.M1 + 1) * (size_t)npairs < (size_t)ASX_QSTORE_MIN_GENS * res) return;
+            r0 = std::min(32, std::max(8, (int)(res / (unsigned)npairs)));
+        }
+    });
+    return r0;
+}
+
+void asx_launch_qstore_takeback(const AsxPrune &U, const AsxSpecWs &S, int npairs, hipStream_t s)
+{
+    hipLaunchKernelGGL(k_qstore_takeback, dim3((unsigned)(npairs + 255) / 256), dim3(256), 0, s, U.redo, S.hdr, S.mode_count, npairs);
 }
 
 void asx_launch_fwd_cols_r(const AsxDev &P, const float *src, size_t src_stride, const float *smp, size_t smp_stride, size_t first,
@@ -1125,10 +1270,10 @@
     hipLaunchKernelGGL(k_tile_bounds, dim3(npairs, 1024 / tp), dim3((tp + 63) & ~63), 0, s, U.eng, U.ub, U.best, U.part, U.ticket, P.M1 + 1, P.ntiles,
                        4.0 * (double)P.M1, ASX_PRUNE_FLOOR_PER_TERM * (double)ASX_PRUNE_T * (double)(P.M1 + 1));
     hipLaunchKernelGGL(k1, dim3(npairs, 2), dim3(NT), lds, s, rargs_of(P), q, pitch, W, resident_blocks((const void *)k1, NT, lds),
-                       AsxSelPrune<true>{ U.best, U.skip });
-    hipLaunchKernelGGL(k_prune_select, dim3(npairs), dim3(256), 0, s, U.ub, U.best, U.skip, W, P.ntiles, U.stats);
+                       AsxSelPrune<true>{ U.best, U.skip, U.list });
+    hipLaunchKernelGGL(k_prune_select, dim3(npairs), dim3(256), 0, s, U.ub, U.best, U.skip, W, P.ntiles, U.stats, U.list, U.redo, U.pair_base);
     hipLaunchKernelGGL(k2, dim3(npairs, rcol_grid_x(P.ntiles, asx_ilog2(TC))), dim3(NT), lds, s, rargs_of(P), q, pitch, W,
-                       resident_blocks((const void *)k2, NT, lds), AsxSelPrune<false>{ U.best, U.skip });
+                       resident_blocks((const void *)k2, NT, lds), AsxSelPrune<false>{ U.best, U.skip, U.list });
 }
 
 void asx_launch_inv_cols_r(const AsxDev &P, const float2 *q, const AsxPeakWs &W, float *r_out, int npairs, hipStream_t s,
diff --git a/old-audiosync_amd/hipxcorr.py b/old-audiosync_amd/hipxcorr.py
--- a/old-audiosync_amd/hipxcorr.py
+++ b/old-audiosync_amd/hipxcorr.py
@@ -47,6 +47,8 @@
     "asx_plan_pearson_modes": (_int, [_vp, _u64p]),
     "asx_plan_set_prune": (_int, [_vp, _int]),
     "asx_plan_prune_stats": (_int, [_vp, _u64p, _u64p]),
+    "asx_plan_set_qstore": (_int, [_vp, _int]),
+    "asx_plan_qstore_stats": (_int, [_vp, _u64p]),
     "asx_plan_set_profiling": (_int, [_vp, _int]),
     "asx_plan_last_timings_ms": (_int, [_vp, c_f32p]),
     "asx_plan_timings_ms": (_int, [_vp, _int, c_f32p]),
@@ -585,6 +587,14 @@
     def prune_stats(self):
         return _counters(lib().asx_plan_prune_stats, self._h, 2)
 
+    def set_qstore(self, mode=1):
+        _check(lib().asx_plan_set_qstore(self._h, int(mode)))
+
+    def qstore_stats(self):
+        c = (ctypes.c_uint64 * 4)()
+        _check(lib().asx_plan_qstore_stats(self._h, c))
+        return tuple(int(v) for v in c)
+
     def narrowed_calls(self):
         return _counters(lib().asx_plan_narrowed_calls, self._h, 1)[0]
 
```

New measurement: 61460 cross-correlations/s, median of 6. 3.9% higher.
